# wangkenpu/rsrgan

Hardware: AMD Instinct MI355X
Metric: GAN train frames/sec (G+D step), 257-dim LPS->40-dim MFCC (higher is better)
Workload: dtype f32

## Files before the change

### rsrgan_amd/csrc/capi.cpp

```cpp
#include <cstring>
#include <exception>
#include <new>
#include <vector>

#include "model.h"
#include "segan.h"

using namespace rsr;

struct rsrgan_handle_s { Model m; };

#define CHECK_H(h)                                                    \
  if (!(h)) { set_error("null handle"); return RSRGAN_ERR_INVALID; }

#define REFUSE_INFER(h, what, rc)                                                                                   \
  if ((h)->m.infer()) { set_error("%s: the handle is inference-only (RSRGAN_FLAG_INFER)", what); return rc; }

template <class F>
static int guard(const char* what, F&& body) {
  try {
    return body();
  } catch (const std::bad_alloc&) {
    set_error("%s: out of host memory", what);
  } catch (const std::exception& e) {
// ... 372 lines not shown
  h->m.prof_on = true; h->m.prof_n = 0; h->m.prof_flops = 0.0; h->m.prof_gp_n = 0; h->m.prof_gp_flops = 0.0; h->m.prof_gb_n = 0; h->m.prof_gb_flops = 0.0; h->m.prof_fdt_n = 0;
  for (int& c : h->m.prof_cnt) c = 0;
  g_chain_launches = 0;
  return RSRGAN_OK;
}
int rsrgan_set_dropout(rsrgan_handle h, float keep_prob, uint64_t seed) {
  CHECK_H(h);
  REFUSE_INFER(h, "rsrgan_set_dropout", RSRGAN_ERR_STATE);
  if (!(keep_prob > 0.f && keep_prob <= 1.f)) { set_error("keep_prob=%g outside (0, 1]", (double)keep_prob); return RSRGAN_ERR_INVALID; }
  Model& m = h->m;
  if (keep_prob < 1.f && m.g_bnl()) { set_error("g_type bnlstm: DropoutWrapper (keep_prob < 1) is not built"); return RSRGAN_ERR_INVALID; }
  if (keep_prob < 1.f && !m.g_dnn()) {
    for (const LstmLayer& L : m.gl)
      if (!L.has_proj) { set_error("DropoutWrapper is built for generator layers with a projection (num_proj) only"); return RSRGAN_ERR_INVALID; }
  }
  if (hipDeviceSynchronize() != hipSuccess) { set_error("hipDeviceSynchronize failed"); return RSRGAN_ERR_HIP; }
  m.keep_prob = keep_prob; m.drop_seed = seed; m.drop_run = 0;
  if (m.drop_ctr && hipMemset(m.drop_ctr, 0, 16) != hipSuccess) { set_error("hipMemset failed"); return RSRGAN_ERR_HIP; }
  m.drop_graphs();
  m.g_fwd_valid = false;
  return RSRGAN_OK;
}

int rsrgan_device_status(rsrgan_handle h, int32_t* code) {
  CHECK_H(h);
  if (!code) { set_error("null output pointer"); return RSRGAN_ERR_INVALID; }
  Model& m = h->m;
  *code = 0;
  if (m.ev_last_set && hipEventSynchronize(m.ev_last) != hipSuccess) { set_error("hipEventSynchronize failed"); return RSRGAN_ERR_HIP; }
  for (hipStream_t q : {m.main_s, m.side})
    if (q && hipStreamSynchronize(q) != hipSuccess) { set_error("hipStreamSynchronize failed"); return RSRGAN_ERR_HIP; }
  if (!m.dp_ctl && !m.gp_ctl) return RSRGAN_OK;
  unsigned* blocks[3] = {m.dp_ctl, m.gp_ctl, m.dp_ctl2};
  for (int k_ = 0; k_ < 3; ++k_) {
    const int k = k_ == 2 ? 0 : k_;
    if (!blocks[k_]) continue;
    unsigned ctl[DP_CTL_WORDS];
    if (hipMemcpy(ctl, blocks[k_], sizeof(ctl), hipMemcpyDeviceToHost) != hipSuccess) { set_error("hipMemcpy failed"); return RSRGAN_ERR_HIP; }
    if (*code == 0 && ctl[DP_CTL_ERR] != 0) *code = (int32_t)(ctl[DP_CTL_ERR] + (k ? 0x10000u : 0u));
    if (ctl[DP_CTL_ERR] != 0 || ctl[DP_CTL_DONE] != 0) {
      const unsigned z[2] = {0u, 0u};
      if (hipMemcpy(blocks[k_] + DP_CTL_DONE, z, sizeof(z), hipMemcpyHostToDevice) != hipSuccess) { set_error("hipMemcpy failed"); return RSRGAN_ERR_HIP; }
      if (k == 1) m.gpersist_rearm();
      if (ctl[DP_CTL_ERR] != 0) m.persist_disable(k);
    }
  }
  return RSRGAN_OK;
}
int rsrgan_device_bytes(rsrgan_handle h, int64_t* bytes) {
  CHECK_H(h);
  if (!bytes) { set_error("null output pointer"); return RSRGAN_ERR_INVALID; }
  *bytes = (int64_t)h->m.alloc_bytes;
  return RSRGAN_OK;
}
int rsrgan_profile_launches(rsrgan_handle h, int64_t* n) {
  CHECK_H(h);
  if (!n) { set_error("null output pointer"); return RSRGAN_ERR_INVALID; }
  *n = g_chain_launches;
  return RSRGAN_OK;
}
int rsrgan_profile_read(rsrgan_handle h, int32_t* launches, double* total_us, double* alg_flops) {
  CHECK_H(h);
  Model& m = h->m;
  if (!launches || !total_us || !alg_flops) { set_error("null output pointer"); return RSRGAN_ERR_INVALID; }
  m.prof_on = false;
  double us = 0.0;
  for (int i = 0; i < m.prof_n; ++i) {
    if (hipEventSynchronize(m.prof_ev[2 * i + 1]) != hipSuccess) { set_error("hipEventSynchronize failed"); return RSRGAN_ERR_HIP; }
    float ms = 0.f;
    if (hipEventElapsedTime(&ms, m.prof_ev[2 * i], m.prof_ev[2 * i + 1]) != hipSuccess) { set_error("hipEventElapsedTime failed"); return RSRGAN_ERR_HIP; }
    us += 1e3 * ms;
  }
  *launches = m.prof_n; *total_us = us; *alg_flops = m.prof_flops;
  return RSRGAN_OK;
}
int rsrgan_profile_read_kind(rsrgan_handle h, int32_t kind, int32_t* launches, double* total_us, double* alg_flops) {
  CHECK_H(h);
  if (kind == 0) return rsrgan_profile_read(h, launches, total_us, alg_flops);
  Model& m = h->m;
  if (kind == 3 && launches && total_us && alg_flops) {
    *launches = m.prof_fdt_n; *total_us = 0.0; *alg_flops = 0.0;
    return RSRGAN_OK;
  }
  if (kind >= 4 && kind <= 8 && launches && total_us && alg_flops) {
    *launches = m.prof_cnt[kind]; *total_us = 0.0; *alg_flops = 0.0;
    return RSRGAN_OK;
  }
  if ((kind != 1 && kind != 2) || !launches || !total_us || !alg_flops) { set_error("profile_read_kind: bad argument"); return RSRGAN_ERR_INVALID; }
  std::vector<hipEvent_t>& ev = kind == 1 ? m.prof_gp_ev : m.prof_gb_ev;
  const int n = kind == 1 ? m.prof_gp_n : m.prof_gb_n;
  double us = 0.0;
  for (int i = 0; i < n; ++i) {
    if (hipEventSynchronize(ev[2 * i + 1]) != hipSuccess) { set_error("hipEventSynchronize failed"); return RSRGAN_ERR_HIP; }
    float ms = 0.f;
    if (hipEventElapsedTime(&ms, ev[2 * i], ev[2 * i + 1]) != hipSuccess) { set_error("hipEventElapsedTime failed"); return RSRGAN_ERR_HIP; }
    us += 1e3 * ms;
  }
  *launches = n; *total_us = us; *alg_flops = kind == 1 ? m.prof_gp_flops : m.prof_gb_flops;
  return RSRGAN_OK;
}

int rsrgan_op_launch_floor(int32_t n, int32_t mode, double* us_per_launch, void* stream) {
  if (n <= 0 || !us_per_launch) { set_error("op_launch_floor: bad argument"); return RSRGAN_ERR_INVALID; }
  static float* buf = nullptr;
  if (!buf && hipMalloc((void**)&buf, 2 * 65536 * 4 * sizeof(float)) != hipSuccess) { set_error("hipMalloc failed"); return RSRGAN_ERR_HIP; }
  hipStream_t s = nullptr;
  hipGraph_t g = nullptr; hipGraphExec_t ge = nullptr;
  hipEvent_t e0 = nullptr, e1 = nullptr;
  int rc = RSRGAN_ERR_HIP;
  do {
    if (hipStreamCreateWithFlags(&s, hipStreamNonBlocking) != hipSuccess) break;
    if (hipMemsetAsync(buf, 0, 2 * 65536 * 4 * sizeof(float), s) != hipSuccess) break;
    if (hipStreamBeginCapture(s, hipStreamCaptureModeThreadLocal) != hipSuccess) break;
    launch_floor_chain(buf, buf + 65536 * 4, n, mode, s);
    if (hipStreamEndCapture(s, &g) != hipSuccess) break;
    if (hipGraphInstantiate(&ge, g, nullptr, nullptr, 0) != hipSuccess) break;
    if (hipEventCreate(&e0) != hipSuccess || hipEventCreate(&e1) != hipSuccess) break;
    if (hipGraphLaunch(ge, s) != hipSuccess) break;
    if (hipEventRecord(e0, s) != hipSuccess || hipGraphLaunch(ge, s) != hipSuccess || hipEventRecord(e1, s) != hipSuccess) break;
    if (hipEventSynchronize(e1) != hipSuccess) break;
    float ms = 0.f;
    if (hipEventElapsedTime(&ms, e0, e1) != hipSuccess) break;
    *us_per_launch = 1e3 * ms / n;
    rc = RSRGAN_OK;
  } while (0);
  if (rc != RSRGAN_OK) set_error("op_launch_floor: HIP call failed");
  if (e0) (void)hipEventDestroy(e0);
  if (e1) (void)hipEventDestroy(e1);
  if (ge) (void)hipGraphExecDestroy(ge);
  if (g) (void)hipGraphDestroy(g);
  if (s) (void)hipStreamDestroy(s);
  (void)stream;
  return rc;
}

static const size_t g_op_ws_floats = (size_t)32 << 20;
static const size_t g_op_scratch_floats = (size_t)2 << 20;
static float* op_ws() {
  static float* ws = nullptr;
  if (!ws && hipMalloc((void**)&ws, g_op_ws_floats * sizeof(float)) != hipSuccess) ws = nullptr;
  return ws;
}
static float* op_scratch() {
  static float* sc = nullptr;
  if (!sc && hipMalloc((void**)&sc, g_op_scratch_floats * sizeof(float)) != hipSuccess) sc = nullptr;
  return sc;
}
#define OP_REFUSE(cond, ...) do { if (cond) { set_error(__VA_ARGS__); return RSRGAN_ERR_INVALID; } } while (0)
struct WorkersScope {
  int saved;
  explicit WorkersScope(int w) : saved(g_gemm_workers) { if (w > 0) g_gemm_workers = w; }
  ~WorkersScope() { g_gemm_workers = saved; }
};

int rsrgan_op_gemm(const float* A, int32_t lda, int32_t a_kc, const float* B, int32_t ldb, int32_t b_kc, float* C, int32_t ldc,
                   int32_t M, int32_t N, int32_t K, const float* bias, int32_t act, float alpha, int32_t accumulate, void* stream) {
  if (!A || !B || !C || (lda & 3) || (ldb & 3)) { set_error("op_gemm: null pointer or leading dimension not a multiple of 4"); return RSRGAN_ERR_INVALID; }
  float* ws = op_ws();
  launch_gemm(A, lda, a_kc != 0, B, ldb, b_kc != 0, C, ldc, M, N, K, bias, act, alpha, accumulate != 0, (hipStream_t)stream,
              ws, ws ? g_op_ws_floats : 0);
  if (hipGetLastError() != hipSuccess) { set_error("op_gemm launch failed"); return RSRGAN_ERR_HIP; }
  return RSRGAN_OK;
}

int rsrgan_op_gemm2(const float* A, int32_t lda, int32_t a_kc, const float* A2, int32_t lda2, int32_t M1, const float* B, int32_t ldb,
                    int32_t b_kc, float* C, int32_t ldc, int32_t M, int32_t N, int32_t K, const float* bias, int32_t act, float alpha,
                    int32_t accumulate, int32_t map_rows_per, int64_t map_outer, int64_t map_inner, int32_t workers, int32_t force_cfg,
// ... 900 lines not shown
```

### rsrgan_amd/csrc/dpersist.hip

```cpp
#include "kernels.h"

namespace rsr {

#include "dpersist_dev.h"

#ifdef DP_TRACE
__device__ unsigned g_dp_trace[64][128][12];
#define DPT(i) do { if (threadIdx.x == 0 && t < 128) dp_tr[t][i] = (unsigned)__builtin_amdgcn_s_memtime(); } while (0)
#define DPG(i) do { if (threadIdx.x == 256 && t < 128) dp_tr[t][8 + (i)] = (unsigned)__builtin_amdgcn_s_memtime(); } while (0)
#define DPT_DECL __shared__ unsigned dp_tr[128][12];
#define DPT_FLUSH() do { if (threadIdx.x == 0 && blockIdx.x < 64) for (int t_ = 0; t_ < 128; ++t_) for (int i_ = 0; i_ < 12; ++i_) g_dp_trace[blockIdx.x][t_][i_] = dp_tr[t_][i_]; } while (0)
#else
#define DPT(i) do { } while (0)
#define DPG(i) do { } while (0)
#define DPT_DECL
#define DPT_FLUSH() do { } while (0)
#endif

__device__ __forceinline__ void dp_fwd_body(const DPersistArgs& a, const unsigned gen) {
  __shared__ __attribute__((aligned(16))) float part_m[DP_NQ][DP_KB][64][4];
  __shared__ __attribute__((aligned(16))) float part_x[2][DP_NQ][DP_KB][64][4];
  __shared__ __attribute__((aligned(16))) float stage[6][16 * DP_HS];
  __shared__ __attribute__((aligned(16))) float kx_lds[4][4][DP_KB][64][4];
  __shared__ __attribute__((aligned(16))) float wp_lds[4][4][64][4];
  __shared__ int dead;
  DPT_DECL
  const int RTn = a.N >> 4, ncl = a.nl * RTn;
  const int cl = blockIdx.x % ncl, cq = blockIdx.x / ncl;
  const int l = cl / RTn, r = cl - l * RTn;
  const DPersistLayer L = a.L[l];
  const int tid = threadIdx.x, lane = tid & 63, lr = lane & 15, q = lane >> 4;
  const int w = __builtin_amdgcn_readfirstlane(tid >> 6);
  const int H = a.H, H4 = 4 * H, T = a.T, P = L.P, ldP = L.ldP, I = L.I;
  const int r0 = r * 16;
  const int Ns = a.Ns ? a.Ns : a.N, rb = a.row0 + r0;
  gu32* err = (gu32*)a.ctl + DP_CTL_ERR;
  if (tid == 0) dead = 0;
  const size_t slot_stride_t = (size_t)DP_NQ * DP_SLOT;
  __syncthreads();

  if (w >= 4) {
    __builtin_amdgcn_s_setprio(3);
    const int j = w - 4;
    const gu64* gm = (const gu64*)a.gran + ((size_t)(l * RTn + r) * T) * slot_stride_t + (size_t)j * DP_SLOT;
    const gu64* gx = (const gu64*)a.gran + ((size_t)(max(l - 1, 0) * RTn + r) * T) * slot_stride_t + (size_t)j * DP_SLOT;
    gu64* gout = (gu64*)a.gran + ((size_t)(l * RTn + r) * T) * slot_stride_t + (size_t)cq * DP_SLOT;
    float vm[DP_KB * 4], vx[DP_KB * 4];
    auto put = [&](float (*part)[DP_KB][64][4], const float (&v)[DP_KB * 4]) {
#pragma unroll
      for (int kb = 0; kb < DP_KB; ++kb)
        *reinterpret_cast<float4*>(&part[j][kb][lane][0]) = make_float4(v[kb * 4], v[kb * 4 + 1], v[kb * 4 + 2], v[kb * 4 + 3]);
    };
    auto fail = [&]() { if (lane == 0) { dead = 1; __hip_atomic_store(err, 1u + (unsigned)blockIdx.x, __ATOMIC_RELAXED, __HIP_MEMORY_SCOPE_AGENT); } };
    if (l > 0) {
      if (!dp_sweep2(nullptr, gen, vm, gx, gen, vx, lane, err)) fail();
      put(part_x[0], vx);
    }
    __syncthreads();
    if (dead) return;
    const int t_end = cq == 0 ? T + 1 : T;
    for (int t = 0; t < t_end; ++t) {
      const bool wm = t > 0, wx = l > 0 && t + 1 < T;
      DPG(0);
      if (wm || wx) {
        if (!dp_sweep2(wm ? gm + (size_t)(t - 1) * slot_stride_t : nullptr, gen, vm,
                       wx ? gx + (size_t)(t + 1) * slot_stride_t : nullptr, gen, vx, lane, err)) fail();
        if (wm) put(part_m, vm);
        if (wx) put(part_x[(t + 1) & 1], vx);
      }
      DPG(1);
      __syncthreads();
      if (dead) return;
      if (t < T) {
        __syncthreads();
        DPG(2);
        if (j < 3) {
          f32x4 pm = f32x4{0.f, 0.f, 0.f, 0.f};
#pragma unroll
          for (int kb = 0; kb < 4; ++kb) {
            const float4 af = *reinterpret_cast<const float4*>(&stage[5][lr * DP_HS + 16 * kb + 4 * q]);
            const float4 bf = *reinterpret_cast<const float4*>(&wp_lds[j][kb][lane][0]);
            pm = __builtin_amdgcn_mfma_f32_16x16x4f32(bf.x, af.x, pm, 0, 0, 0);
            pm = __builtin_amdgcn_mfma_f32_16x16x4f32(bf.y, af.y, pm, 0, 0, 0);
            pm = __builtin_amdgcn_mfma_f32_16x16x4f32(bf.z, af.z, pm, 0, 0, 0);
            pm = __builtin_amdgcn_mfma_f32_16x16x4f32(bf.w, af.w, pm, 0, 0, 0);
          }
          gu64* go_ = gout + (size_t)t * slot_stride_t + ((size_t)j * 64 + lane) * 4;
          dp_store2(go_, gen, pm[0], pm[1]);
          dp_store2(go_ + 2, gen, pm[2], pm[3]);
        }
        else {
          const int c4 = (lane & 15) * 4, rr = lane >> 4;
#pragma unroll
          for (int rg = 0; rg < 4; ++rg) {
            const int row = 4 * rg + rr;
            const size_t grow = (size_t)t * Ns + rb + row;
#pragma unroll
            for (int g = 0; g < 4; ++g)
              *reinterpret_cast<float4*>(L.gates + grow * H4 + g * H + cq * 64 + c4) = *reinterpret_cast<const float4*>(&stage[g][row * DP_HS + c4]);
            *reinterpret_cast<float4*>(L.c + (grow + Ns) * H + cq * 64 + c4) = *reinterpret_cast<const float4*>(&stage[4][row * DP_HS + c4]);
            *reinterpret_cast<float4*>(L.h + grow * L.ldH + cq * 64 + c4) = *reinterpret_cast<const float4*>(&stage[5][row * DP_HS + c4]);
          }
        }
        DPG(3);
      }
    }
    return;
  }

  const int cell = cq * 64 + 16 * w + lr;
  float4 kh[4][DP_KB];
#pragma unroll
  for (int g = 0; g < 4; ++g)
#pragma unroll
    for (int kb = 0; kb < DP_KB; ++kb) {
      float vh[4], vx[4];
#pragma unroll
      for (int u = 0; u < 4; ++u) {
        const int k = 16 * kb + 4 * q + u;
        vh[u] = L.K[(size_t)(I + min(k, P - 1)) * H4 + g * H + cell];
        vx[u] = L.K[(size_t)min(k, I - 1) * H4 + g * H + cell];
      }
      asm volatile("" : "+v"(vh[0]), "+v"(vh[1]), "+v"(vh[2]), "+v"(vh[3]), "+v"(vx[0]), "+v"(vx[1]), "+v"(vx[2]), "+v"(vx[3]));
#pragma unroll
      for (int u = 0; u < 4; ++u) {
        const int k = 16 * kb + 4 * q + u;
        vh[u] = k < P ? vh[u] : 0.f;
        vx[u] = k < I ? vx[u] : 0.f;
      }
      kh[g][kb] = make_float4(vh[0], vh[1], vh[2], vh[3]);
      *reinterpret_cast<float4*>(&kx_lds[w][g][kb][lane][0]) = make_float4(vx[0], vx[1], vx[2], vx[3]);
    }
  {
    const int col = 16 * w + lr;
#pragma unroll
    for (int kb = 0; kb < 4; ++kb) {
      float v[4];
#pragma unroll
      for (int u = 0; u < 4; ++u) v[u] = L.Wp[(size_t)(cq * 64 + 16 * kb + 4 * q + u) * ldP + min(col, P - 1)];
      asm volatile("" : "+v"(v[0]), "+v"(v[1]), "+v"(v[2]), "+v"(v[3]));
#pragma unroll
      for (int u = 0; u < 4; ++u) v[u] = col < P ? v[u] : 0.f;
      *reinterpret_cast<float4*>(&wp_lds[w][kb][lane][0]) = make_float4(v[0], v[1], v[2], v[3]);
    }
  }
  const int cb = cq * 64 + 16 * w + 4 * q;
  const float4 pwi = *reinterpret_cast<const float4*>(L.wi + cb), pwf = *reinterpret_cast<const float4*>(L.wf + cb);
  const float4 pwo = *reinterpret_cast<const float4*>(L.wo + cb);
  f32x4 bs[4];
#pragma unroll
  for (int g = 0; g < 4; ++g) bs[g] = *reinterpret_cast<const f32x4*>(L.bias + g * H + cb);
  const int lenF = a.len[r0 + lr];
  float cp[4] = {0.f, 0.f, 0.f, 0.f};
  float4 mf[DP_KB];
#pragma unroll
  for (int kb = 0; kb < DP_KB; ++kb) mf[kb] = make_float4(0.f, 0.f, 0.f, 0.f);
  *reinterpret_cast<float4*>(L.c + (size_t)(rb + lr) * H + cb) = make_float4(0.f, 0.f, 0.f, 0.f);
  if (cq == 0 && w == 0) {
#pragma unroll
    for (int kb = 0; kb < DP_KB; ++kb)
      if (16 * kb + 4 * q < P) *reinterpret_cast<float4*>(L.mst + (size_t)(rb + lr) * ldP + 16 * kb + 4 * q) = make_float4(0.f, 0.f, 0.f, 0.f);
  }

  f32x4 accn[4];
  float4 xn[DP_KB];
  auto load_x = [&](int t) {
    const float* xr = L.in + ((size_t)t * Ns + rb + lr) * L.ldI;
#pragma unroll
    for (int kb = 0; kb < DP_KB; ++kb) xn[kb] = *reinterpret_cast<const float4*>(xr + min(16 * kb + 4 * q, I - 4));
  };
  auto sum_parts = [&](float (*part)[DP_KB][64][4], int width, float4 (&s)[DP_KB]) {
#pragma unroll
    for (int kb = 0; kb < DP_KB; ++kb) {
      const float4 p0 = *reinterpret_cast<const float4*>(&part[0][kb][lane][0]), p1 = *reinterpret_cast<const float4*>(&part[1][kb][lane][0]);
      const float4 p2 = *reinterpret_cast<const float4*>(&part[2][kb][lane][0]), p3 = *reinterpret_cast<const float4*>(&part[3][kb][lane][0]);
      s[kb] = dp_sel(16 * kb + 4 * q < width,
                     make_float4(((p0.x + p1.x) + p2.x) + p3.x, ((p0.y + p1.y) + p2.y) + p3.y, ((p0.z + p1.z) + p2.z) + p3.z,
                                 ((p0.w + p1.w) + p2.w) + p3.w), make_float4(0.f, 0.f, 0.f, 0.f));
    }
  };
  auto mma_part = [&](f32x4 (&acc)[4], const float4 (&af)[DP_KB], const float4 (&bf)[4][DP_KB]) {
#pragma unroll
    for (int kb = 0; kb < DP_KB; ++kb) {
#pragma unroll
      for (int g = 0; g < 4; ++g) acc[g] = __builtin_amdgcn_mfma_f32_16x16x4f32(bf[g][kb].x, af[kb].x, acc[g], 0, 0, 0);
#pragma unroll
      for (int g = 0; g < 4; ++g) acc[g] = __builtin_amdgcn_mfma_f32_16x16x4f32(bf[g][kb].y, af[kb].y, acc[g], 0, 0, 0);
#pragma unroll
      for (int g = 0; g < 4; ++g) acc[g] = __builtin_amdgcn_mfma_f32_16x16x4f32(bf[g][kb].z, af[kb].z, acc[g], 0, 0, 0);
#pragma unroll
      for (int g = 0; g < 4; ++g) acc[g] = __builtin_amdgcn_mfma_f32_16x16x4f32(bf[g][kb].w, af[kb].w, acc[g], 0, 0, 0);
    }
  };
  auto next_x = [&](int t) {
#pragma unroll
    for (int g = 0; g < 4; ++g) accn[g] = bs[g];
    float4 xs[DP_KB];
    if (l > 0) {
      sum_parts(part_x[t & 1], I, xs);
      const bool live = t < lenF;
#pragma unroll
      for (int kb = 0; kb < DP_KB; ++kb) xs[kb] = dp_sel(live, xs[kb], make_float4(0.f, 0.f, 0.f, 0.f));
    } else {
#pragma unroll
      for (int kb = 0; kb < DP_KB; ++kb) xs[kb] = dp_sel(16 * kb + 4 * q < I, xn[kb], make_float4(0.f, 0.f, 0.f, 0.f));
    }
#pragma unroll
    for (int kb = 0; kb < DP_KB; ++kb) {
      float4 bf[4];
#pragma unroll
      for (int g = 0; g < 4; ++g) bf[g] = *reinterpret_cast<const float4*>(&kx_lds[w][g][kb][lane][0]);
#pragma unroll
      for (int g = 0; g < 4; ++g) accn[g] = __builtin_amdgcn_mfma_f32_16x16x4f32(bf[g].x, xs[kb].x, accn[g], 0, 0, 0);
#pragma unroll
      for (int g = 0; g < 4; ++g) accn[g] = __builtin_amdgcn_mfma_f32_16x16x4f32(bf[g].y, xs[kb].y, accn[g], 0, 0, 0);
#pragma unroll
      for (int g = 0; g < 4; ++g) accn[g] = __builtin_amdgcn_mfma_f32_16x16x4f32(bf[g].z, xs[kb].z, accn[g], 0, 0, 0);
#pragma unroll
      for (int g = 0; g < 4; ++g) accn[g] = __builtin_amdgcn_mfma_f32_16x16x4f32(bf[g].w, xs[kb].w, accn[g], 0, 0, 0);
    }
  };
  auto store_m = [&](int t, const float4 (&mnew)[DP_KB], bool live_prev) {
    if (cq != 0 || w != 0) return;
#pragma unroll
    for (int kb = 0; kb < DP_KB; ++kb)
      if (16 * kb + 4 * q < P) {
        *reinterpret_cast<float4*>(L.mst + ((size_t)t * Ns + rb + lr) * ldP + 16 * kb + 4 * q) = mf[kb];
        *reinterpret_cast<float4*>(L.out + ((size_t)(t - 1) * Ns + rb + lr) * ldP + 16 * kb + 4 * q) =
            dp_sel(live_prev, mnew[kb], make_float4(0.f, 0.f, 0.f, 0.f));
      }
  };

  if (l == 0) load_x(0);
  __syncthreads();
  if (dead) return;
  next_x(0);
  if (l == 0) load_x(min(1, T - 1));

  float hv[4] = {0.f, 0.f, 0.f, 0.f}, sg[4][4] = {};
  for (int t = 0; t < T; ++t) {
    f32x4 acc[4];
    DPT(0);
    __syncthreads();
    if (dead) return;
    DPT(1);
#pragma unroll
    for (int g = 0; g < 4; ++g) acc[g] = accn[g];
    if (t > 0) {
      float4 ms[DP_KB];
      sum_parts(part_m, P, ms);
      const bool live_prev = (t - 1) < lenF;
#pragma unroll
      for (int kb = 0; kb < DP_KB; ++kb) mf[kb] = dp_sel(live_prev, ms[kb], mf[kb]);
      store_m(t, ms, live_prev);
    }
    mma_part(acc, mf, kh);
    DPT(2);
    const bool live = t < lenF;
    const float pi_[4] = {pwi.x, pwi.y, pwi.z, pwi.w}, pf_[4] = {pwf.x, pwf.y, pwf.z, pwf.w}, po_[4] = {pwo.x, pwo.y, pwo.z, pwo.w};
#pragma unroll
    for (int i = 0; i < 4; ++i) {
      const float cpv = cp[i];
      const float gi = dp_sigmoid(acc[0][i] + pi_[i] * cpv);
      const float gf = dp_sigmoid(acc[2][i] + a.forget_bias + pf_[i] * cpv);
      const float gj = dp_tanh(acc[1][i]);
      const float cn = gf * cpv + gi * gj;
      const float go = dp_sigmoid(acc[3][i] + po_[i] * cn);
      const float hh = go * dp_tanh(cn);
      hv[i] = live ? hh : 0.f;
      sg[0][i] = live ? gi : 0.f; sg[1][i] = live ? gj : 0.f; sg[2][i] = live ? gf : 0.f; sg[3][i] = live ? go : 0.f;
      cp[i] = live ? cn : cpv;
    }
    {
      const int so = lr * DP_HS + 16 * w + 4 * q;
#pragma unroll
      for (int g = 0; g < 4; ++g) *reinterpret_cast<float4*>(&stage[g][so]) = make_float4(sg[g][0], sg[g][1], sg[g][2], sg[g][3]);
      *reinterpret_cast<float4*>(&stage[4][so]) = make_float4(cp[0], cp[1], cp[2], cp[3]);
      *reinterpret_cast<float4*>(&stage[5][so]) = make_float4(hv[0], hv[1], hv[2], hv[3]);
    }
    DPT(3);
    __syncthreads();
    DPT(4);
    DPT(7);
    __builtin_amdgcn_s_sleep(12);
    if (t + 1 < T) next_x(t + 1);
    if (l == 0) load_x(min(t + 2, T - 1));
    DPT(5);
    DPT(6);
  }
  DPT_FLUSH();
  if (cq == 0) {
    __syncthreads();
    if (dead) return;
    float4 ms[DP_KB];
    sum_parts(part_m, P, ms);
    const bool live_prev = (T - 1) < lenF;
#pragma unroll
    for (int kb = 0; kb < DP_KB; ++kb) mf[kb] = dp_sel(live_prev, ms[kb], mf[kb]);
    store_m(T, ms, live_prev);
  }
}

__global__ __launch_bounds__(512, 1) void k_dlstm_fwd(const DPersistArgs a) {
  gu32* ctl = (gu32*)a.ctl;
  const unsigned gen = __hip_atomic_load(ctl + DP_CTL_GEN, __ATOMIC_RELAXED, __HIP_MEMORY_SCOPE_AGENT);
  dp_fwd_body(a, gen);
  if (threadIdx.x == 0) persist_last_out(ctl, gen, [] { return gridDim.x; }, [&] { return a.L[a.nl - 1].out; }, 0u, [] {});
}

__device__ __forceinline__ void dp_bwd_body(const DPersistArgs& a, const unsigned gen) {
  __shared__ __attribute__((aligned(16))) float part_m[DP_NQ][DP_KB][64][4];
  __shared__ __attribute__((aligned(16))) float part_x[2][DP_NQ][DP_KB][64][4];
  __shared__ __attribute__((aligned(16))) float stage[4][16 * DP_HS];
  __shared__ __attribute__((aligned(16))) float psum[4][DP_KB][64][4];
  __shared__ __attribute__((aligned(16))) float psum_x[2][4][DP_KB][64][4];
  __shared__ __attribute__((aligned(16))) float kx_lds[4][DP_KB][4][64][4];
  __shared__ int dead;
  DPT_DECL
  const int RTn = a.N >> 4, ncl = a.nl * RTn;
  const int cl = blockIdx.x % ncl, cq = blockIdx.x / ncl;
  const int l = cl / RTn, r = cl - l * RTn;
  const DPersistLayer L = a.L[l];
  const int tid = threadIdx.x, lane = tid & 63, lr = lane & 15, q = lane >> 4;
  const int w = __builtin_amdgcn_readfirstlane(tid >> 6);
  const int H = a.H, H4 = 4 * H, T = a.T, N = a.N, P = L.P, ldP = L.ldP, I = L.I;
  const int r0 = r * 16;
  const bool top = l == a.nl - 1;
  gu32* err = (gu32*)a.ctl + DP_CTL_ERR;
  if (tid == 0) dead = 0;
  const size_t slot_stride_t = (size_t)DP_NQ * DP_SLOT;
  auto edge = [&](int layer, int e) -> gu64* {
    return (gu64*)a.gran + ((size_t)((layer * 2 + e) * RTn + r) * T) * slot_stride_t;
  };
  __syncthreads();

  if (w >= 4) {
    __builtin_amdgcn_s_setprio(3);
    const int j = w - 4;
    const gu64* gm = edge(l, 0) + (size_t)j * DP_SLOT;
    const gu64* gx = edge(min(l + 1, a.nl - 1), 1) + (size_t)j * DP_SLOT;
    gu64* gout_m = edge(l, 0) + (size_t)cq * DP_SLOT;
    gu64* gout_x = edge(l, 1) + (size_t)cq * DP_SLOT;
    gu32* dwf = a.dw_ws ? (gu32*)a.dw_flag + ((size_t)(l * RTn + r) * (T + 1)) * 4 + cq : nullptr;
    float vm[DP_KB * 4], vx[DP_KB * 4];
    auto put = [&](float (*part)[DP_KB][64][4], const float (&v)[DP_KB * 4]) {
#pragma unroll
      for (int kb = 0; kb < DP_KB; ++kb)
        *reinterpret_cast<float4*>(&part[j][kb][lane][0]) = make_float4(v[kb * 4], v[kb * 4 + 1], v[kb * 4 + 2], v[kb * 4 + 3]);
    };
    auto fail = [&]() { if (lane == 0) { dead = 1; __hip_atomic_store(err, 1u + (unsigned)blockIdx.x, __ATOMIC_RELAXED, __HIP_MEMORY_SCOPE_AGENT); } };
    auto publish = [&](float (*ps)[DP_KB][64][4], gu64* dst) {
      const float4 p0 = *reinterpret_cast<const float4*>(&ps[0][j][lane][0]), p1 = *reinterpret_cast<const float4*>(&ps[1][j][lane][0]);
      const float4 p2 = *reinterpret_cast<const float4*>(&ps[2][j][lane][0]), p3 = *reinterpret_cast<const float4*>(&ps[3][j][lane][0]);
      gu64* go_ = dst + ((size_t)j * 64 + lane) * 4;
      dp_store2(go_, gen, ((p0.x + p1.x) + p2.x) + p3.x, ((p0.y + p1.y) + p2.y) + p3.y);
      dp_store2(go_ + 2, gen, ((p0.z + p1.z) + p2.z) + p3.z, ((p0.w + p1.w) + p2.w) + p3.w);
    };
    if (!top) {
      if (!dp_sweep2(nullptr, gen, vm, gx + (size_t)(T - 1) * slot_stride_t, gen, vx, lane, err)) fail();
      put(part_x[(T - 1) & 1], vx);
    }
    __syncthreads();
    if (dead) return;
    for (int t = T - 1; t >= 0; --t) {
      const bool wm = t < T - 1, wx = !top && t > 0;
      DPG(0);
      if (wm || wx) {
        if (!dp_sweep2(wm ? gm + (size_t)(t + 1) * slot_stride_t : nullptr, gen, vm,
                       wx ? gx + (size_t)(t - 1) * slot_stride_t : nullptr, gen, vx, lane, err)) fail();
        if (wm) put(part_m, vm);
        if (wx) put(part_x[(t - 1) & 1], vx);
      }
      DPG(1);
      __syncthreads();
      if (dead) return;
      if (j < 3 && l > 0 && t < T - 1) publish(psum_x[(t + 1) & 1], gout_x + (size_t)(t + 1) * slot_stride_t);
      __syncthreads();
      DPG(2);
      if (j < 3) {
        publish(psum, gout_m + (size_t)t * slot_stride_t);
      } else {
        const int c4 = (lane & 15) * 4, rr = lane >> 4;
        if (dwf) {
          if (lane == 0) __hip_atomic_store(dwf + (size_t)t * 4, gen, __ATOMIC_RELAXED, __HIP_MEMORY_SCOPE_AGENT);
#pragma unroll
          for (int rg = 0; rg < 4; ++rg) {
            const int row = 4 * rg + rr;
            const size_t grow = (size_t)t * N + r0 + row;
#pragma unroll
            for (int g = 0; g < 4; ++g)
              dp_store4_wt(L.gates + grow * H4 + g * H + cq * 64 + c4, *reinterpret_cast<const float4*>(&stage[g][row * DP_HS + c4]));
          }
        } else {
#pragma unroll
          for (int rg = 0; rg < 4; ++rg) {
            const int row = 4 * rg + rr;
            const size_t grow = (size_t)t * N + r0 + row;
#pragma unroll
            for (int g = 0; g < 4; ++g)
              *reinterpret_cast<float4*>(L.gates + grow * H4 + g * H + cq * 64 + c4) = *reinterpret_cast<const float4*>(&stage[g][row * DP_HS + c4]);
          }
        }
      }
      DPG(3);
    }
    if (l > 0) {
      __syncthreads();
      if (j < 3) publish(psum_x[0], gout_x);
    }
    return;
  }

  const int cb = cq * 64 + 16 * w + 4 * q;
  float4 wpA[DP_KB], khA[DP_KB][4];
  {
    const float* wrow = L.Wp + (size_t)(cq * 64 + 16 * w + lr) * ldP;
#pragma unroll
    for (int kb = 0; kb < DP_KB; ++kb) {
      const int k = 16 * kb + 4 * q;
      const float4 v = *reinterpret_cast<const float4*>(wrow + min(k, P - 4));
      wpA[kb] = dp_sel(k < P, v, make_float4(0.f, 0.f, 0.f, 0.f));
    }
#pragma unroll
    for (int pt = 0; pt < DP_KB; ++pt) {
      const int p = 16 * pt + lr;
#pragma unroll
      for (int g = 0; g < 4; ++g) {
        const float4 vh = *reinterpret_cast<const float4*>(L.K + (size_t)(I + min(p, P - 1)) * H4 + g * H + cb);
        const float4 vx = *reinterpret_cast<const float4*>(L.K + (size_t)min(p, I - 1) * H4 + g * H + cb);
        khA[pt][g] = dp_sel(p < P, vh, make_float4(0.f, 0.f, 0.f, 0.f));
        *reinterpret_cast<float4*>(&kx_lds[w][pt][g][lane][0]) = dp_sel(l > 0 && p < I, vx, make_float4(0.f, 0.f, 0.f, 0.f));
      }
    }
  }
  const float4 pwi = *reinterpret_cast<const float4*>(L.wi + cb), pwf = *reinterpret_cast<const float4*>(L.wf + cb);
  const float4 pwo = *reinterpret_cast<const float4*>(L.wo + cb);
  const float pi_[4] = {pwi.x, pwi.y, pwi.z, pwi.w}, pf_[4] = {pwf.x, pwf.y, pwf.z, pwf.w}, po_[4] = {pwo.x, pwo.y, pwo.z, pwo.w};
  const int lenF = a.len[r0 + lr];

  float dc[4] = {0.f, 0.f, 0.f, 0.f};
  float4 mf[DP_KB];
#pragma unroll
  for (int kb = 0; kb < DP_KB; ++kb) mf[kb] = make_float4(0.f, 0.f, 0.f, 0.f);
  f32x4 gn[4], cpn;
  float4 don[DP_KB];
  f32x4 ccur;
  auto prefetch = [&](int t) {
    const size_t row = (size_t)t * N + r0 + lr;
#pragma unroll
    for (int g = 0; g < 4; ++g) gn[g] = *reinterpret_cast<const f32x4*>(L.gates + row * H4 + g * H + cb);
    cpn = *reinterpret_cast<const f32x4*>(L.c + row * H + cb);
    if (top) {
#pragma unroll
      for (int kb = 0; kb < DP_KB; ++kb)
        don[kb] = *reinterpret_cast<const float4*>(a.dout_top + row * a.ld_dout + min(16 * kb + 4 * q, P - 4));
    }
  };
  auto sum_parts = [&](float (*part)[DP_KB][64][4], int width, float4 (&s)[DP_KB]) {
#pragma unroll
    for (int kb = 0; kb < DP_KB; ++kb) {
      const float4 p0 = *reinterpret_cast<const float4*>(&part[0][kb][lane][0]), p1 = *reinterpret_cast<const float4*>(&part[1][kb][lane][0]);
      const float4 p2 = *reinterpret_cast<const float4*>(&part[2][kb][lane][0]), p3 = *reinterpret_cast<const float4*>(&part[3][kb][lane][0]);
      s[kb] = dp_sel(16 * kb + 4 * q < width,
                     make_float4(((p0.x + p1.x) + p2.x) + p3.x, ((p0.y + p1.y) + p2.y) + p3.y, ((p0.z + p1.z) + p2.z) + p3.z,
                                 ((p0.w + p1.w) + p2.w) + p3.w), make_float4(0.f, 0.f, 0.f, 0.f));
    }
  };
  ccur = *reinterpret_cast<const f32x4*>(L.c + ((size_t)T * N + r0 + lr) * H + cb);
  prefetch(T - 1);
  __syncthreads();
  if (dead) return;

  for (int t = T - 1; t >= 0; --t) {
    DPT(0);
    __syncthreads();
    if (dead) return;
    DPT(1);
    const bool live = t < lenF;
    f32x4 gt[4];
#pragma unroll
    for (int g = 0; g < 4; ++g) gt[g] = gn[g];
    const f32x4 cprev = cpn;
    float4 dout[DP_KB];
    if (top) {
#pragma unroll
      for (int kb = 0; kb < DP_KB; ++kb) dout[kb] = dp_sel(16 * kb + 4 * q < P, don[kb], make_float4(0.f, 0.f, 0.f, 0.f));
    } else {
      sum_parts(part_x[t & 1], P, dout);
    }
    prefetch(max(t - 1, 0));
    if (t < T - 1) {
      float4 ms[DP_KB];
      sum_parts(part_m, P, ms);
      const bool live_next = (t + 1) < lenF;
#pragma unroll
      for (int kb = 0; kb < DP_KB; ++kb) mf[kb] = dp_sel(live_next, ms[kb], mf[kb]);
    }
    float4 dm[DP_KB];
#pragma unroll
    for (int kb = 0; kb < DP_KB; ++kb)
      dm[kb] = dp_sel(live, make_float4(dout[kb].x + mf[kb].x, dout[kb].y + mf[kb].y, dout[kb].z + mf[kb].z, dout[kb].w + mf[kb].w),
                      make_float4(0.f, 0.f, 0.f, 0.f));
    if (cq == 0 && w == 0) {
      if (a.dw_ws) {
#pragma unroll
        for (int kb = 0; kb < DP_KB; ++kb)
          if (16 * kb + 4 * q < P) dp_store4_wt(L.dmt + ((size_t)t * N + r0 + lr) * ldP + 16 * kb + 4 * q, dm[kb]);
      } else {
#pragma unroll
        for (int kb = 0; kb < DP_KB; ++kb)
          if (16 * kb + 4 * q < P) *reinterpret_cast<float4*>(L.dmt + ((size_t)t * N + r0 + lr) * ldP + 16 * kb + 4 * q) = dm[kb];
      }
    }
    f32x4 dh = f32x4{0.f, 0.f, 0.f, 0.f};
#pragma unroll
    for (int kb = 0; kb < DP_KB; ++kb) {
      dh = __builtin_amdgcn_mfma_f32_16x16x4f32(wpA[kb].x, dm[kb].x, dh, 0, 0, 0);
      dh = __builtin_amdgcn_mfma_f32_16x16x4f32(wpA[kb].y, dm[kb].y, dh, 0, 0, 0);
      dh = __builtin_amdgcn_mfma_f32_16x16x4f32(wpA[kb].z, dm[kb].z, dh, 0, 0, 0);
      dh = __builtin_amdgcn_mfma_f32_16x16x4f32(wpA[kb].w, dm[kb].w, dh, 0, 0, 0);
    }
    DPT(2);
    float dz[4][4];
#pragma unroll
    for (int i = 0; i < 4; ++i) {
      const float gi = gt[0][i], gj = gt[1][i], gf = gt[2][i], go = gt[3][i];
      const float tc = dp_tanh(ccur[i]);
      const float dao = dh[i] * tc * go * (1.f - go);
      const float dcn = dc[i] + dh[i] * go * (1.f - tc * tc) + dao * po_[i];
      const float daf = dcn * cprev[i] * gf * (1.f - gf);
      const float dai = dcn * gj * gi * (1.f - gi);
      const float dj = dcn * gi * (1.f - gj * gj);
      dz[0][i] = live ? dai : 0.f; dz[1][i] = live ? dj : 0.f; dz[2][i] = live ? daf : 0.f; dz[3][i] = live ? dao : 0.f;
      dc[i] = live ? dcn * gf + dai * pi_[i] + daf * pf_[i] : dc[i];
    }
    ccur = cprev;
    {
      const int so = lr * DP_HS + 16 * w + 4 * q;
#pragma unroll
      for (int g = 0; g < 4; ++g) *reinterpret_cast<float4*>(&stage[g][so]) = make_float4(dz[g][0], dz[g][1], dz[g][2], dz[g][3]);
    }
    DPT(3);
    f32x4 pa[DP_KB];
#pragma unroll
    for (int pt = 0; pt < DP_KB; ++pt) pa[pt] = f32x4{0.f, 0.f, 0.f, 0.f};
#pragma unroll
    for (int g = 0; g < 4; ++g) {
#pragma unroll
      for (int pt = 0; pt < DP_KB; ++pt) pa[pt] = __builtin_amdgcn_mfma_f32_16x16x4f32(khA[pt][g].x, dz[g][0], pa[pt], 0, 0, 0);
#pragma unroll
      for (int pt = 0; pt < DP_KB; ++pt) pa[pt] = __builtin_amdgcn_mfma_f32_16x16x4f32(khA[pt][g].y, dz[g][1], pa[pt], 0, 0, 0);
#pragma unroll
      for (int pt = 0; pt < DP_KB; ++pt) pa[pt] = __builtin_amdgcn_mfma_f32_16x16x4f32(khA[pt][g].z, dz[g][2], pa[pt], 0, 0, 0);
#pragma unroll
      for (int pt = 0; pt < DP_KB; ++pt) pa[pt] = __builtin_amdgcn_mfma_f32_16x16x4f32(khA[pt][g].w, dz[g][3], pa[pt], 0, 0, 0);
    }
#pragma unroll
    for (int pt = 0; pt < DP_KB; ++pt) *reinterpret_cast<f32x4*>(&psum[w][pt][lane][0]) = pa[pt];
    DPT(4);
    __syncthreads();
    DPT(5);
    if (l > 0) {
      __builtin_amdgcn_s_sleep(8);
#pragma unroll
      for (int pt = 0; pt < DP_KB; ++pt) pa[pt] = f32x4{0.f, 0.f, 0.f, 0.f};
#pragma unroll
      for (int g = 0; g < 4; ++g) {
        float4 af[DP_KB];
#pragma unroll
        for (int pt = 0; pt < DP_KB; ++pt) af[pt] = *reinterpret_cast<const float4*>(&kx_lds[w][pt][g][lane][0]);
#pragma unroll
        for (int pt = 0; pt < DP_KB; ++pt) pa[pt] = __builtin_amdgcn_mfma_f32_16x16x4f32(af[pt].x, dz[g][0], pa[pt], 0, 0, 0);
#pragma unroll
        for (int pt = 0; pt < DP_KB; ++pt) pa[pt] = __builtin_amdgcn_mfma_f32_16x16x4f32(af[pt].y, dz[g][1], pa[pt], 0, 0, 0);
#pragma unroll
        for (int pt = 0; pt < DP_KB; ++pt) pa[pt] = __builtin_amdgcn_mfma_f32_16x16x4f32(af[pt].z, dz[g][2], pa[pt], 0, 0, 0);
#pragma unroll
        for (int pt = 0; pt < DP_KB; ++pt) pa[pt] = __builtin_amdgcn_mfma_f32_16x16x4f32(af[pt].w, dz[g][3], pa[pt], 0, 0, 0);
      }
#pragma unroll
      for (int pt = 0; pt < DP_KB; ++pt) *reinterpret_cast<f32x4*>(&psum_x[t & 1][w][pt][lane][0]) = pa[pt];
    }
    DPT(6);
  }
  DPT_FLUSH();
  if (l > 0) __syncthreads();
}

constexpr int DW_MT = 6;
__device__ __forceinline__ float dp_ld_sc1(const float* p) {
  return __uint_as_float(__hip_atomic_load((const unsigned*)p, __ATOMIC_RELAXED, __HIP_MEMORY_SCOPE_AGENT));
}
template <bool proj>
__device__ __forceinline__ void dp_dw_body(const DPersistArgs& a, const unsigned gen, const int bid) {
  const int RTn = a.N >> 4;
  const int g = bid & 3, cl = bid >> 2;
  const int l = cl / RTn, r = cl - l * RTn;
  const DPersistLayer L = a.L[l];
  const int lane = threadIdx.x & 63, lr = lane & 15, q = lane >> 4;
  const int w = __builtin_amdgcn_readfirstlane(threadIdx.x >> 6);
  const int H = a.H, H4 = 4 * H, T = a.T, N = a.N, I = L.I, P = L.P, ldP = L.ldP, ldI = L.ldI;
  const int r0 = r * 16;
  const int c0 = 32 * w, col0 = g * H + c0;
  gu32* err = (gu32*)a.ctl + DP_CTL_ERR;
  const gu32* flags = (const gu32*)a.dw_flag + ((size_t)(l * RTn + r) * (T + 1)) * 4;

  f32x4 acc[DW_MT][2];
#pragma unroll
  for (int mt = 0; mt < DW_MT; ++mt) { acc[mt][0] = f32x4{0.f, 0.f, 0.f, 0.f}; acc[mt][1] = f32x4{0.f, 0.f, 0.f, 0.f}; }
  f32x4 accp[2][DP_KB];
#pragma unroll
  for (int j = 0; j < 2; ++j)
#pragma unroll
    for (int nt = 0; nt < DP_KB; ++nt) accp[j][nt] = f32x4{0.f, 0.f, 0.f, 0.f};
  float pp[2] = {0.f, 0.f};
  const size_t coff = g == 3 ? (size_t)N * H : 0;

  struct Ops { float av[DW_MT][4], bv[2][4], ev[DP_KB][4], fv[2][4]; };
  bool ok = true;
  auto wait_for = [&](int t) {
    const gu32* fp = flags + (size_t)(t >= 2 ? t - 2 : T) * 4;
    const unsigned long long t0 = __builtin_amdgcn_s_memrealtime();
    for (unsigned spins = 0;; ++spins) {
      u32x4 v;
      asm volatile("global_load_dwordx4 %0, %1, off sc1\n\ts_waitcnt vmcnt(0)" : "=&v"(v) : "v"(fp) : "memory");
      if (v.x == gen && v.y == gen && v.z == gen && v.w == gen) return;
      __builtin_amdgcn_s_sleep(32);
      if ((spins & 63) == 63 && (__builtin_amdgcn_s_memrealtime() - t0 > 100000000ull ||
                                 __hip_atomic_load(err, __ATOMIC_RELAXED, __HIP_MEMORY_SCOPE_AGENT) != 0)) { ok = false; return; }
    }
  };
  unsigned off_x[3], off_m[3], off_d[DP_KB];
  float msk_x[3], msk_m[3], one_m[3];
#pragma unroll
  for (int k = 0; k < 3; ++k) {
    const int f = 16 * k + lr;
    off_x[k] = (unsigned)((r0 + q) * ldI + min(f, I - 1)); msk_x[k] = f < I ? 1.f : 0.f;
    off_m[k] = (unsigned)((r0 + q) * ldP + min(f, P - 1)); msk_m[k] = f < P ? 1.f : 0.f; one_m[k] = f == P ? 1.f : 0.f;
    off_d[k] = off_m[k];
  }
  const unsigned off_b = (unsigned)((r0 + q) * H4 + col0 + lr);
  const unsigned off_c = (unsigned)((r0 + q) * (proj ? L.ldH : H) + c0 + lr);
  auto load = [&](Ops& o, int t) {
#pragma unroll
    for (int s = 0; s < 4; ++s) {
      const size_t rw = (size_t)t * N + 4 * s;
      const float* gb = L.gates + rw * H4;
      o.bv[0][s] = dp_ld_sc1(gb + off_b);
      o.bv[1][s] = dp_ld_sc1(gb + off_b + 16);
    }
#pragma unroll
    for (int s = 0; s < 4; ++s) {
      const size_t rw = (size_t)t * N + 4 * s;
      const float* xb = L.in + rw * ldI;
      const float* mb = L.mst + rw * ldP;
#pragma unroll
      for (int k = 0; k < 3; ++k) { o.av[k][s] = xb[off_x[k]]; o.av[3 + k][s] = mb[off_m[k]]; }
    }
    if (proj) {
#pragma unroll
      for (int s = 0; s < 4; ++s) {
        const size_t rw = (size_t)t * N + 4 * s;
        const float* hb = L.h + rw * L.ldH;
        const float* db = L.dmt + rw * ldP;
        o.fv[0][s] = hb[off_c]; o.fv[1][s] = hb[off_c + 16];
#pragma unroll
        for (int nt = 0; nt < DP_KB; ++nt) o.ev[nt][s] = dp_ld_sc1(db + off_d[nt]);
      }
    } else {
#pragma unroll
      for (int s = 0; s < 4; ++s) {
        const float* cb = L.c + coff + ((size_t)t * N + 4 * s) * H;
        o.fv[0][s] = cb[off_c]; o.fv[1][s] = cb[off_c + 16];
      }
    }
    __builtin_amdgcn_sched_barrier(0);
#pragma unroll
    for (int s = 0; s < 4; ++s) {
#pragma unroll
      for (int k = 0; k < 3; ++k) { o.av[k][s] *= msk_x[k]; o.av[3 + k][s] = o.av[3 + k][s] * msk_m[k] + one_m[k]; }
      if (proj) {
#pragma unroll
        for (int nt = 0; nt < DP_KB; ++nt) o.ev[nt][s] *= msk_m[nt];
      }
    }
  };
  auto compute = [&](const Ops& o) {
#pragma unroll
    for (int s = 0; s < 4; ++s) {
#pragma unroll
      for (int mt = 0; mt < DW_MT; ++mt) {
        acc[mt][0] = __builtin_amdgcn_mfma_f32_16x16x4f32(o.av[mt][s], o.bv[0][s], acc[mt][0], 0, 0, 0);
        acc[mt][1] = __builtin_amdgcn_mfma_f32_16x16x4f32(o.av[mt][s], o.bv[1][s], acc[mt][1], 0, 0, 0);
      }
    }
    if (proj) {
#pragma unroll
      for (int s = 0; s < 4; ++s)
#pragma unroll
        for (int j = 0; j < 2; ++j)
#pragma unroll
          for (int nt = 0; nt < DP_KB; ++nt) accp[j][nt] = __builtin_amdgcn_mfma_f32_16x16x4f32(o.fv[j][s], o.ev[nt][s], accp[j][nt], 0, 0, 0);
    } else {
#pragma unroll
      for (int s = 0; s < 4; ++s) { pp[0] += o.bv[0][s] * o.fv[0][s]; pp[1] += o.bv[1][s] * o.fv[1][s]; }
    }
  };
  __shared__ int prog;
  if (threadIdx.x == 0) prog = T;
  __syncthreads();
  Ops o;
  if (w == 0) {
    wait_for(T - 1);
    if (lane == 0) __hip_atomic_store(&prog, ok ? T - 1 : -1, __ATOMIC_RELAXED, __HIP_MEMORY_SCOPE_WORKGROUP);
    for (int t = T - 1; t >= 0 && ok; --t) {
      u32x4 fl = {gen, gen, gen, gen};
      if (t >= 1) {
        const gu32* fp = flags + (size_t)(t >= 3 ? t - 3 : T) * 4;
        asm volatile("global_load_dwordx4 %0, %1, off sc1" : "=&v"(fl) : "v"(fp) : "memory");
      }
      load(o, t);
      compute(o);
      asm volatile("s_waitcnt vmcnt(0)" : "+v"(fl) : : "memory");
      if (t >= 1) {
        if (!(fl.x == gen && fl.y == gen && fl.z == gen && fl.w == gen)) { __builtin_amdgcn_s_sleep(32); wait_for(t - 1); }
        if (lane == 0) __hip_atomic_store(&prog, ok ? t - 1 : -1, __ATOMIC_RELAXED, __HIP_MEMORY_SCOPE_WORKGROUP);
      }
    }
  } else {
    for (int t = T - 1; t >= 0 && ok; --t) {
      for (;;) {
        const int p_ = __hip_atomic_load(&prog, __ATOMIC_RELAXED, __HIP_MEMORY_SCOPE_WORKGROUP);
        if (p_ < 0) { ok = false; break; }
        if (p_ <= t) break;
        __builtin_amdgcn_s_sleep(4);
      }
      if (!ok) break;
      load(o, t);
      compute(o);
    }
  }
  if (!ok) return;
  float* wsb = a.dw_ws + (size_t)(l * RTn + r) * a.dw_stride;
#pragma unroll
  for (int mt = 0; mt < DW_MT; ++mt)
#pragma unroll
    for (int nt = 0; nt < 2; ++nt)
#pragma unroll
      for (int i = 0; i < 4; ++i) {
        const int f = 16 * (mt % 3) + 4 * q + i;
        const bool on = mt < 3 ? f < I : f <= P;
        if (on) wsb[(size_t)(mt < 3 ? f : I + f) * H4 + col0 + 16 * nt + lr] = acc[mt][nt][i];
      }
  if (proj) {
    float* pw = wsb + (size_t)(I + P + 1) * H4 + 3 * H;
#pragma unroll
    for (int j = 0; j < 2; ++j)
#pragma unroll
      for (int nt = 0; nt < DP_KB; ++nt)
#pragma unroll
        for (int i = 0; i < 4; ++i)
          if (16 * nt + lr < P) pw[(size_t)(c0 + 16 * j + 4 * q + i) * ldP + 16 * nt + lr] = accp[j][nt][i];
  } else {
    float* pw = wsb + (size_t)(I + P + 1) * H4 + (g == 0 ? 0 : g == 2 ? 1 : 2) * H + c0;
#pragma unroll
    for (int nt = 0; nt < 2; ++nt) {
      float v = pp[nt];
      v += __shfl_xor(v, 16); v += __shfl_xor(v, 32);
      if (q == 0) pw[16 * nt + lr] = v;
    }
  }
}

__global__ __launch_bounds__(512, 1) void k_dlstm_bwd(const DPersistArgs a) {
  gu32* ctl = (gu32*)a.ctl;
  const unsigned gen = __hip_atomic_load(ctl + DP_CTL_GEN, __ATOMIC_RELAXED, __HIP_MEMORY_SCOPE_AGENT);
  const int nchain = a.nl * (a.N >> 4) * DP_NQ;
  if ((int)blockIdx.x >= nchain) {
    const int bid = (int)blockIdx.x - nchain;
    if ((bid & 3) == 1) dp_dw_body<true>(a, gen, bid); else dp_dw_body<false>(a, gen, bid);
  } else {
    dp_bwd_body(a, gen);
    if (a.dw_ws) {
      asm volatile("s_waitcnt vmcnt(0)" ::: "memory");
      __syncthreads();
      if (threadIdx.x == 0) {
        const int RTn = a.N >> 4, ncl = a.nl * RTn, cl = blockIdx.x % ncl, cq = blockIdx.x / ncl;
        __hip_atomic_store((gu32*)a.dw_flag + ((size_t)cl * (a.T + 1) + a.T) * 4 + cq, gen, __ATOMIC_RELAXED, __HIP_MEMORY_SCOPE_AGENT);
      }
    }
  }
  if (threadIdx.x == 0) persist_last_out(ctl, gen, [] { return gridDim.x; }, [&] { return a.L[0].gates; }, 0u, [] {});
}


size_t dpersist_granule_bytes(int nl, int N, int T) { return (size_t)2 * nl * (N / 16) * T * DP_NQ * DP_SLOT * sizeof(unsigned long long); }

int dpersist_grid(int nl, int N) { return nl * (N / 16) * DP_NQ; }
size_t dpersist_lds_bytes() {
  hipFuncAttributes f{}, b{};
  if (hipFuncGetAttributes(&f, (const void*)k_dlstm_fwd) != hipSuccess || hipFuncGetAttributes(&b, (const void*)k_dlstm_bwd) != hipSuccess) return 0;
  return f.sharedSizeBytes > b.sharedSizeBytes ? f.sharedSizeBytes : b.sharedSizeBytes;
}

bool dpersist_supported(const DPersistArgs& a) {
  if (a.nl < 1 || a.nl > DP_MAXL || a.N % 16 != 0 || a.H != 64 * DP_NQ || a.T < 1) return false;
  if (dpersist_grid(a.nl, a.N) > 128 || dpersist_grid(a.nl, a.N) > device_cu_count()) return false;
  for (int l = 0; l < a.nl; ++l) {
    const DPersistLayer& L = a.L[l];
    if (L.P > 16 * DP_KB || L.P % 4 != 0 || L.ldP % 4 != 0 || L.P < 4) return false;
    if (l > 0 && (L.I != a.L[l - 1].P)) return false;
    if (L.I > 16 * DP_KB || (l == 0 && (L.I < 4 || L.I % 4 != 0 || L.ldI % 4 != 0))) return false;
  }
  return true;
}

void launch_dlstm_bwd(const DPersistArgs& a, hipStream_t s) {
  const int blocks = dpersist_grid(a.nl, a.N) + (a.dw_ws ? dpersist_dw_grid(a.nl, a.N) : 0);
  hipLaunchKernelGGL(k_dlstm_bwd, dim3(blocks), dim3(512), 0, s, a);
  ++g_chain_launches;
}
int dpersist_dw_grid(int nl, int N) { return 4 * nl * (N / 16); }
size_t dpersist_dw_stride(const DPersistArgs& a) { return (size_t)(a.L[0].I + a.L[0].P + 1) * 4 * a.H + 3 * (size_t)a.H + (size_t)a.H * a.L[0].ldP; }
size_t dpersist_dw_flag_bytes(int nl, int N, int T) { return (size_t)nl * (N / 16) * (T + 1) * 4 * sizeof(unsigned); }
bool dpersist_dw_supported(const DPersistArgs& a) {
  for (int l = 0; l < a.nl; ++l) {
    const DPersistLayer& L = a.L[l];
    if (L.I > 48 || L.P > 47 || L.I < 1 || L.I != a.L[0].I || L.P != a.L[0].P || L.ldP != a.L[0].ldP || L.ldI < L.I) return false;
  }
  return a.H == 64 * DP_NQ;
}

__global__ __launch_bounds__(768, 3) void k_dlstm_fwd_t(const DPersistArgs a) {
  __shared__ __attribute__((aligned(16))) DpFwdTLds S;
  gu32* ctl = (gu32*)a.ctl;
  const unsigned gen = __hip_atomic_load(ctl + DP_CTL_GEN, __ATOMIC_RELAXED, __HIP_MEMORY_SCOPE_AGENT);
  if (threadIdx.x == 0) S.dead = 0;
  __syncthreads();
  dp_fwdt_body<false>(a, gen, S, (int)blockIdx.x, false);
  if (threadIdx.x == 0) persist_last_out(ctl, gen, [] { return gridDim.x; }, [&] { return a.L[a.nl - 1].out; }, 0u, [] {});
}
void launch_dlstm_fwd_t(const DPersistArgs& a, hipStream_t s) {
  hipLaunchKernelGGL(k_dlstm_fwd_t, dim3(a.nl * (a.N / 32) * DP_NQ), dim3(768), 0, s, a);
  ++g_chain_launches;
}

size_t dpersist_fwdt_lds_bytes() { return sizeof(DpFwdTLds); }
int dpersist_trail_grid(int nl, int N) { return nl * (N / 32) * DP_NQ + N / 16; }
size_t dpersist_trail_lds_bytes() { return sizeof(DpTrailLds); }
bool dpersist_trail_supported(const DPersistArgs& a) {
  if (!dpersist_supported(a) || a.N % 32 != 0 || !a.dy || !a.fc_w || !a.dtop) return false;
  if (a.ld_dy % 4 != 0 || a.ld_fcw % 4 != 0 || a.ld_dtop % 4 != 0 || a.fc_P < 1 || a.fc_P > a.ld_dtop || a.ld_dtop > 16 * 8 * DP_FCT) return false;
  return a.L[0].I % 4 == 0 && a.L[0].I >= 4 && a.L[0].I <= a.ld_dy && a.L[0].I <= a.ld_fcw;
}
void launch_dlstm_fwd(const DPersistArgs& a, hipStream_t s) {
  const int blocks = dpersist_grid(a.nl, a.N);
  hipLaunchKernelGGL(k_dlstm_fwd, dim3(blocks), dim3(512), 0, s, a);
  ++g_chain_launches;
}

}
```

### rsrgan_amd/csrc/kernels.h

```cpp
#pragma once
#include <hip/hip_runtime.h>
#include <stdint.h>

#include "switches.h"

namespace rsr {

constexpr int MAXJ = 8;

struct Place { int x0, nx, sb, se, nb, w; };
constexpr int JOBMAP_MAX = 768;
struct JobMap { int valid; unsigned char job[JOBMAP_MAX]; };
struct PlanItem { int ncol, nrow; double cost; int mult; };
int plan_places(int n, const PlanItem* items, Place* out);

enum { DYN_G_LR = 0, DYN_D_LR = 1, DYN_LAMBDA = 2, DYN_D_REAL = 3, DYN_D_FAKE = 4, DYN_L2 = 5, DYN_CLIP = 6,
       DYN_B1 = 7, DYN_B2 = 8, DYN_EPS = 9, DYN_EMA = 10, DYN_ADAM_LRT = 11, DYN_ADAM_LRT_D = 12, DYN_COUNT = 16 };

struct FwdGateJob {
  const float* x;
  const float* KxT;
  const float* m;
  const float* KhT;
  const float* Wsw;
// ... 34 lines not shown
  const float* noise;
  int ldh, ldm, ldo, P, t, N;
  int nblk_c;
  Place pl;
  DropSpec drop;
};
struct FwdProjJobs { int n; FwdProjJob j[MAXJ]; JobMap map; };

struct BwdAJob {
  const float* dout;
  const float* dmst;
  const float* Wp;
  const float* Wp_sw;
  float* dmt;
  float* gates;
  const float* c_prev;
  const float* c_cur;
  const float* wf; const float* wi; const float* wo;
  float* dc;
  const int* len;
  int ldm, P, t, N, H;
  int nblk_c;
  Place pl;
  DropSpec drop;
};
struct BwdAJobs { int n; BwdAJob j[MAXJ]; JobMap map; };

struct BwdBJob {
  const float* dz;
  const float* K;
  const float* Ksw;
  float* dx;
  float* dmst;
  const int* len;
  int I, n_begin, n_end, lddx, ldm, t, N, H4;
  int dx_accumulate;
  int nblk_c;
  Place pl;
  float* ws;
  int ldw, KG, kpg, ncg, nrg;
  Place plp, plr;
};
struct BwdBJobs { int n; BwdBJob j[MAXJ]; JobMap map, mapr; };

inline int job_blocks(int nblk_c, int N, int rows = 32) { return ((nblk_c + 7) & ~7) * ((N + rows - 1) / rows); }
int fwd_gates_rows();
void launch_fwd_gates(const FwdGateJobs& jobs, int total_blocks, int kb_max, hipStream_t s);
void launch_fwd_proj(const FwdProjJobs& jobs, int total_blocks, int kb_max, hipStream_t s);
int bwd_a_cells();
void launch_bwd_a(const BwdAJobs& jobs, int total_blocks, int kb_max, hipStream_t s);
void launch_bwd_b(const BwdBJobs& jobs, int total_blocks, int kb_max, hipStream_t s);
size_t bwd_b_plan(BwdBJobs& jobs, float* ws_base);
void launch_bwd_b_splitk(const BwdBJobs& jobs, hipStream_t s);
constexpr int DP_MAXL = 3;
constexpr int DP_CTL_GEN = 0, DP_CTL_DONE = 1, DP_CTL_ERR = 2, DP_CTL_WORDS = 4;
struct DPersistLayer {
  const float *K, *bias, *wi, *wf, *wo, *Wp;
  float *gates, *c, *h, *mst, *out;
  const float* in;
  float* dmt;
  int I, P, ldP, ldH, ldI;
};
struct DPersistArgs {
  DPersistLayer L[DP_MAXL];
  int nl, N, T, H;
  const int* len;
  unsigned long long* gran;
  unsigned* ctl;
  float forget_bias;
  const float* dout_top;
  int ld_dout;
  float* dy;
  const float* fc_w;
  float* dtop;
  int ld_dy, ld_fcw, ld_dtop, fc_P;
  const float* fc_b;
  const float* noise;
  int xd_Ns, xd_row0;
  int Ns, row0;
  int nrt;
  float* dw_ws;
  unsigned* dw_flag;
  size_t dw_stride;
};
int dpersist_dw_grid(int nl, int N);
size_t dpersist_dw_stride(const DPersistArgs& a);
size_t dpersist_dw_flag_bytes(int nl, int N, int T);
bool dpersist_dw_supported(const DPersistArgs& a);
size_t dpersist_granule_bytes(int nl, int N, int T);
int dpersist_trail_grid(int nl, int N);
size_t dpersist_trail_lds_bytes();
bool dpersist_trail_supported(const DPersistArgs& a);
bool dpersist_supported(const DPersistArgs& a);
int dpersist_grid(int nl, int N);
size_t dpersist_lds_bytes();
void launch_dlstm_fwd(const DPersistArgs& a, hipStream_t s);
void launch_dlstm_fwd_t(const DPersistArgs& a, hipStream_t s);
void launch_dlstm_bwd(const DPersistArgs& a, hipStream_t s);
constexpr int GP_MAXL = 4;
constexpr int GP_ROWS = 32;
constexpr int GP_THREADS = 768;
struct GPersistLayer {
  const float *KxT, *KhT;
  const float *bias, *wi, *wf, *wo, *Wp;
  float *gates, *c, *h, *mst, *out;
  const float* in;
  float* dmt;
  int I, P, ldI, ldP, ldH;
  float* res_out;
  const float *ca, *cb;
};
struct GPersistArgs {
  GPersistLayer L[GP_MAXL];
  int nl, N, T, H;
  int NT, NC;
  const int* len;
  unsigned long long *gran1, *gran2;
  unsigned* ctl;
  float forget_bias;
  unsigned long long* gran3;
  const float* dout_top;
  int ld_dout;
  float* din0;
  int ld_din0;
  int res;
  int tags;
  int dout_trail;
  int fwd_trail;
  int ngl, grp0;
  int nrt;
  int sched;
  int carry;
  int lean;
  int cnorm;
};
constexpr int GP_TMAX = 2046;
bool gpersist_plan(GPersistArgs& a);
void gpersist_arm_bytes(void* p, size_t bytes, hipStream_t s);
extern thread_local int g_gemm_workers;
int gpersist_grid(const GPersistArgs& a);
int gpersist_dt_grid(const GPersistArgs& a, const DPersistArgs& d);
void launch_glstm_fwd_dt(const GPersistArgs& a, const DPersistArgs& d, hipStream_t s);
size_t dpersist_fwdt_lds_bytes();
void launch_glstm_bwd_dt(const GPersistArgs& a, const DPersistArgs& d, hipStream_t s);
size_t gpersist_lds_bytes();
int device_cu_count();
bool resident_probe(int grid, int threads, size_t lds_bytes);
size_t gpersist_gran1_bytes(const GPersistArgs& a);
size_t gpersist_gran2_bytes(const GPersistArgs& a);
size_t gpersist_gran3_bytes(const GPersistArgs& a);
void gpersist_arm(const GPersistArgs& a, hipStream_t s);
void launch_glstm_fwd(const GPersistArgs& a, hipStream_t s);
bool gpersist_np_plan(GPersistArgs& a, int nt_force = 0);
size_t gpersist_np_gran2_bytes(const GPersistArgs& a);
size_t gpersist_np_lds_bytes();
void launch_glstm_np_fwd(const GPersistArgs& a, hipStream_t s);
size_t gpersist_np_gran1_bytes(const GPersistArgs& a);
size_t gpersist_np_gran3_bytes(const GPersistArgs& a);
void gpersist_np_arm(const GPersistArgs& a, hipStream_t s);
void launch_glstm_np_bwd(const GPersistArgs& a, hipStream_t s);
void launch_glstm_bwd(const GPersistArgs& a, hipStream_t s);
extern long long g_chain_launches;
void launch_floor_chain(float* a, float* b, int n, int mode, hipStream_t s);

struct GemmRowMap { int rows_per; long long outer; long long inner; };
enum { GEMM_CLS_NONE = 0, GEMM_CLS_GEMM16 = 1, GEMM_CLS_N32 = 2, GEMM_CLS_KGEMM = 3, GEMM_CLS_KGEMM_S = 4, GEMM_CLS_GEMM16_B = 5,
       GEMM_CLS_KGEMM_B = 6, GEMM_CLS_KGEMM_S_B = 7 };
struct GemmPlanRecord { int cls, bm, bn, W, n_dp, fixup, splits, Ur; };
extern thread_local GemmPlanRecord g_gemm_last_plan;
void launch_gemm_mapped(const float* A, int lda, const GemmRowMap& ma, const float* A2, int lda2, int M1, bool a_kc, const float* B, int ldb,
                        bool b_kc, float* C, int ldc, int M, int N, int K, const float* bias, int act, float alpha,
                        bool accumulate, hipStream_t s, float* ws, size_t ws_floats, int force_cfg = -1);
constexpr int GEMM16_MAXB = 4;
struct Gemm16Batch { const float* A[GEMM16_MAXB]; const float* A2[GEMM16_MAXB]; const float* B[GEMM16_MAXB]; float* C[GEMM16_MAXB]; int n; };
void launch_gemm16_batch(const Gemm16Batch& bt, int lda, int lda2, int M1, int ldb, int ldc, int M, int N, int K, bool accumulate,
                         hipStream_t s, float* ws, size_t ws_floats);
void launch_gemm2(const float* A, int lda, const float* A2, int lda2, int M1, bool a_kc, const float* B, int ldb, bool b_kc,
                  float* C, int ldc, int M, int N, int K, const float* bias, int act, float alpha, bool accumulate,
// ... 140 lines not shown
```

### rsrgan_amd/csrc/model.cpp

```cpp
#include "model.h"

#include <cmath>
#include <cstdarg>
#include <cstdio>
#include <cstdlib>
#include <cstring>

namespace rsr {

static thread_local char g_err[512] = "";
void set_error(const char* fmt, ...) {
  va_list ap;
  va_start(ap, fmt);
  vsnprintf(g_err, sizeof(g_err), fmt, ap);
  va_end(ap);
}
const char* get_error() { return g_err; }

static inline uint64_t seg_key(int seg, int T, unsigned bits) { return ((uint64_t)seg << 48) | ((uint64_t)(unsigned)T << 16) | (bits & 0xffffu); }
enum { SEG_D = 1, SEG_G_MAIN = 2, SEG_G_FCIN = 3, SEG_G_LAYER0 = 4 , SEG_G_L2 = 20, SEG_G_TAIL = 21, SEG_APPLY_D = 22, SEG_APPLY_G = 23, SEG_G_BATCH = 24, SEG_BNL = 25 };

template <class F>
void Model::run_seg(uint64_t key, hipStream_t s, F&& body) {
  if (!graphs_on() || s == nullptr) { body(); return; }
// ... 293 lines not shown
    flush_g();
    for (size_t c = 0; c < chains.size(); ++c) {
      Chain& ch = chains[c];
      const int off = offsets ? (*offsets)[c] : 0;
      for (int l = (int)ch.size() - 1; l >= 0; --l) {
        const int t = d - off - l;
        if (t < 0 || t >= T) continue;
        const LayerRun& R = ch[l];
        if (!R.L->has_proj) continue;
        if (pj.n == MAXJ) flush_p();
        FwdProjJob& p = pj.j[pj.n++]; fill_proj(p, R, t); pb += proj_blocks(R.L->P, R.N);
        pk = std::max(pk, kb16(R.L->ldH));
      }
    }
    if (fcs)
      for (auto& F : *fcs) {
        const int t = d - F.offset;
        if (t < 0 || t >= T) continue;
        if (pj.n == MAXJ) flush_p();
        FwdProjJob& p = pj.j[pj.n++]; fill_fc_fwd(p, F, t); pb += proj_blocks(F.D, F.N);
        pk = std::max(pk, kb16(F.ld_in));
      }
    flush_p();
  }
}

void Model::refresh_fold(hipStream_t s) {
  SwizzleList sl{};
  for (size_t l = 0; l < dl.size(); ++l) {
    const LstmLayer& L = dl[l]; const LstmLayer& F = dl_fold[l];
    const int H4 = 4 * L.H;
    const float* K = D.W(L.tK);
    float* Kf = dl_fold_K[l];
    if (l == 0) (void)hipMemcpyAsync(Kf, K, (size_t)L.I * H4 * sizeof(float), hipMemcpyDeviceToDevice, s);
    else gemm(D.W(dl[l - 1].tWp), dl[l - 1].ldP, true, K, H4, false, Kf, H4, dl[l - 1].H, H4, L.I, nullptr, 0, 0.f, false, s);
    gemm(D.W(L.tWp), L.ldP, true, K + (size_t)L.I * H4, H4, false, Kf + (size_t)F.I * H4, H4, L.H, H4, L.P, nullptr, 0, 0.f, false, s);
    const int ncb = (F.H + 15) / 16;
    sl.j[sl.n++] = SwizzleJob{Kf, F.Wg_full, H4, 4, F.H, 0, 0, 0, F.I, F.P, F.ldI, 4 * ncb, (F.ldI + F.ldP + 15) / 16, 0};
    sl.j[sl.n++] = SwizzleJob{Kf, F.Wg_h, H4, 4, F.H, 0, 0, 0, F.I, F.P, 0, 4 * ncb, (F.ldP + 15) / 16, 0};
  }
  launch_swizzle_many(sl, s);
}

bool Model::fold_forward(Chain& ch, int T, hipStream_t s) {
  if (dl_fold.empty() || !wavefront() || ch.size() != dl_fold.size()) return false;
  Chain fch;
  for (size_t l = 0; l < ch.size(); ++l) {
    const LayerRun& R = ch[l];
    if (R.L != &dl[l] || R.S != &d_st[l] || R.res_in || R.res_out || R.zx_batched || R.want_wgrads || R.row0 != 0 || R.Ns != R.N) return false;
    LayerRun Rf = R;
    Rf.L = &dl_fold[l]; Rf.S = &d_fold_st[l];
    if (l > 0) Rf.in = d_st[l - 1].h;
    fch.push_back(Rf);
  }
  refresh_fold(s);
  std::vector<Chain> chains{fch};
  const bool prof_was = prof_on;
  prof_on = false;
  rnn_forward(chains, T, s);
  prof_on = prof_was;
  for (size_t l = 0; l < ch.size(); ++l) {
    const LstmLayer& L = dl[l];
    gemm(d_st[l].h, L.ldH, true, D.W(L.tWp), L.ldP, false, d_st[l].out, L.ldP, T * ch[l].N, L.P, L.H, nullptr, 0, 0.f, false, s);
  }
  return true;
}

bool Model::persist_forward(Chain& ch, int T, hipStream_t s) {
  if (!dp_gran || !(dp_live & 1) || !wavefront() || ch.size() != dl.size()) return false;
  DPersistArgs a{};
  a.nl = (int)ch.size(); a.N = ch[0].N; a.T = T; a.H = dl[0].H; a.len = ch[0].len;
  a.gran = dp_gran; a.ctl = dp_ctl; a.forget_bias = cfg.forget_bias;
  for (size_t l = 0; l < ch.size(); ++l) {
    const LayerRun& R = ch[l]; const LstmLayer& L = dl[l]; const LstmStash& S = d_st[l];
    if (R.L != &L || R.S != &S || R.res_in || R.res_out || R.row0 != 0 || R.Ns != R.N || R.N != a.N || !L.has_proj || L.H != a.H) return false;
    if (l > 0 && R.in != d_st[l - 1].out) return false;
    DPersistLayer& D_ = a.L[l];
    D_.K = D.W(L.tK); D_.bias = D.W(L.tb); D_.wi = D.W(L.twi); D_.wf = D.W(L.twf); D_.wo = D.W(L.two); D_.Wp = D.W(L.tWp);
    D_.gates = S.gates; D_.c = S.c; D_.h = S.h; D_.mst = S.mst; D_.out = S.out;
    D_.I = L.I; D_.P = L.P; D_.ldP = L.ldP; D_.ldH = L.ldH; D_.ldI = L.ldI;
    D_.in = l == 0 ? R.in : nullptr;
  }
  if (!dpersist_supported(a) || dpersist_grid(a.nl, a.N) > dp_max_grid || dpersist_granule_bytes(a.nl, a.N, a.T) > dp_gran_bytes) return false;
  if (switches().dfwd_t && a.N % 32 == 0) launch_dlstm_fwd_t(a, s); else launch_dlstm_fwd(a, s);
  if (prof_on) ++prof_cnt[4];
  return true;
}

int Model::trail_nrt() const {
  const bool on = switches().dp_nrt && switches().gp_nrt;
  return on && B == 32 && Bt <= 16 && (gp_live & 3) == 3 && (dp_live & 3) == 3 ? 1 : 0;
}
bool Model::gpersist_shape(GPersistArgs& a, int T) const {
  const bool res = (cfg.g_type == RSRGAN_G_RES_LSTM_L || g_resi()) && switches().gp_res;
  if (!gp_live || gl.empty() || gl.size() > (size_t)GP_MAXL || (cfg.g_type != RSRGAN_G_LSTM && cfg.g_type != RSRGAN_G_RES_LSTM_BASE && !res && !bnl_infer())) return false;
  a = GPersistArgs{};
  a.nl = (int)gl.size(); a.N = B; a.T = T; a.H = gl[0].H; a.res = res ? (g_resi() ? 2 : 1) : 0;
  bool noproj = !gl[0].has_proj;
  a.tags = switches().gp_tags && !noproj ? 1 : 0;
  if (bnl_infer()) { if (!a.tags) return false; a.cnorm = 1; }
  for (size_t l = 0; l < gl.size(); ++l) {
    const LstmLayer& L = gl[l];
    if (L.has_proj == noproj || L.H != a.H) return false;
    GPersistLayer& G_ = a.L[l];
    G_.I = L.I; G_.P = L.P; G_.ldI = L.ldI; G_.ldP = L.ldP; G_.ldH = L.ldH;
  }
  if (noproj) return switches().gp_noproj && !res && (gp_live & 1) && gpersist_np_plan(a, gp_np_nt);
  if (!gpersist_plan(a)) return false;
  if (switches().gp_nrt && B == 32 && Bt <= 16 && (gp_live & 3) == 3) a.nrt = 1;
  const int sched_env = switches().gp_sched;
  a.sched = sched_env >= 0 ? sched_env : (B >= 64 ? 3 : 0);
  return true;
}
bool Model::gpersist_args(GPersistArgs& a, int T) const {
  if (!gpersist_shape(a, T)) return false;
  a.len = len_dev;
  a.gran1 = gp_gran1; a.gran2 = gp_gran2; a.gran3 = gp_gran3; a.ctl = gp_ctl; a.forget_bias = cfg.forget_bias;
  for (size_t l = 0; l < gl.size(); ++l) {
    const LstmLayer& L = gl[l]; const LstmStash& S = g_st[l];
    GPersistLayer& G_ = a.L[l];
    G_.KxT = L.KxT; G_.KhT = L.KhT; G_.bias = L.bias_f ? L.bias_f : G.W(L.tb); G_.ca = L.ca; G_.cb = L.cb; G_.wi = G.W(L.twi); G_.wf = G.W(L.twf); G_.wo = G.W(L.two); G_.Wp = L.has_proj ? G.W(L.tWp) : nullptr;
    G_.gates = S.gates; G_.c = S.c; G_.h = S.h; G_.mst = S.mst; G_.out = S.out; G_.dmt = S.dmt;
    G_.res_out = a.res ? g_res[l] : nullptr;
  }
  return true;
}

void Model::persist_disable(int which) {
  if (which == 1) gp_live = 0; else dp_live = 0;
  lazy_sw = false;
  trail_fits = false;
  dpipe = false;
  drop_graphs();
  refresh_swizzles(RSRGAN_NET_G, nullptr);
  refresh_swizzles(RSRGAN_NET_D, nullptr);
  (void)hipStreamSynchronize(nullptr);
}

void Model::gpersist_rearm() {
  GPersistArgs a{};
  if (!gp_gran1 || !gpersist_args(a, gp_Tcap)) return;
  if (gp_noproj) {
    if (gp_gran3) { gpersist_np_arm(a, 0); (void)hipDeviceSynchronize(); }
    return;
  }
  gpersist_arm(a, 0);
  (void)hipDeviceSynchronize();
}

static void glstm_fwd_groups(GPersistArgs a, const DPersistArgs* d, hipStream_t s) {
  const int ngr = a.N / GP_ROWS;
  if (!a.ngl) { if (d) launch_glstm_fwd_dt(a, *d, s); else launch_glstm_fwd(a, s); return; }
  for (int g = 0; g < ngr; ++g) {
    a.grp0 = g;
    if (d && g == ngr - 1) launch_glstm_fwd_dt(a, *d, s); else launch_glstm_fwd(a, s);
  }
}
static void glstm_bwd_groups(GPersistArgs a, const DPersistArgs* d, hipStream_t s) {
  const int ngr = a.N / GP_ROWS;
  if (!a.ngl) { if (d) launch_glstm_bwd_dt(a, *d, s); else launch_glstm_bwd(a, s); return; }
  for (int g = 0; g < ngr; ++g) {
    a.grp0 = g;
    if (d && g == 0) { a.dout_trail = 1; launch_glstm_bwd_dt(a, *d, s); } else { a.dout_trail = 0; launch_glstm_bwd(a, s); }
  }
}

bool Model::persist_forward_g(int T, hipStream_t s) {
  if (!gp_fwd_on() || !wavefront() || seq_drop_on()) return false;
  GPersistArgs a{};
  if (!gpersist_args(a, T) || (gp_noproj ? gpersist_np_gran2_bytes(a) : gpersist_gran2_bytes(a)) > gp_gran2_bytes) return false;
  a.L[0].in = g_ins[0];
  a.carry = g_carry ? 1 : 0;
  if (infer()) {
    a.lean = 1; a.len = len_win;
    a.L[0].in = g_ins[0] + (size_t)inf_t0 * B * gl[0].ldI;
    const size_t top = gl.size() - 1;
    for (size_t l = 0; l < gl.size(); ++l) {
      GPersistLayer& G_ = a.L[l];
      G_.gates = G_.h = G_.dmt = nullptr;
      const size_t o = (size_t)inf_t0 * B * gl[l].ldP;
      G_.out = l == top && !a.res ? g_st[l].out + o : nullptr;
      G_.res_out = l == top && a.res ? g_res[l] + o : nullptr;
    }
  }
  if (gp_noproj) {
    for (size_t l = 0; l < gl.size(); ++l) a.L[l].Wp = nullptr;
    launch_glstm_np_fwd(a, s);
    if (prof_on) ++prof_cnt[7];
    return true;
  }
  if (prof_on) {
    if ((size_t)(2 * prof_gp_n + 2) > prof_gp_ev.size()) {
      const size_t old = prof_gp_ev.size();
      prof_gp_ev.resize(old + 8, nullptr);
      for (size_t i = old; i < prof_gp_ev.size(); ++i) (void)hipEventCreate(&prof_gp_ev[i]);
    }
    for (size_t l = 0; l < gl.size(); ++l)
      prof_gp_flops += 2.0 * Bt * T * ((double)(gl[l].I + gl[l].P) * 4.0 * gl[l].H + (double)gl[l].H * gl[l].P);
    (void)hipEventRecord(prof_gp_ev[2 * prof_gp_n], s);
    glstm_fwd_groups(a, nullptr, s);
    (void)hipEventRecord(prof_gp_ev[2 * prof_gp_n + 1], s);
    ++prof_gp_n;
    return true;
  }
  glstm_fwd_groups(a, nullptr, s);
  return true;
}

// ... 63 lines not shown
      if (l > 0 && (R.din_accumulate || ch[l].din != ch[l - 1].dout)) return false;
    }
    if (ch[0].din) return false;
    a.dout_top = ch.back().dout; a.ld_dout = gl.back().ldP;
    if (!a.dout_top) return false;
    if (check_only) return true;
    launch_glstm_np_bwd(a, s);
    if (prof_on) ++prof_cnt[8];
    if (!defer_wgrads) chain_wgrads(ch, T, s, nullptr, pre, post);
    else { if (pre) pre(s); if (post) post(s); }
    return true;
  }
  const bool resi = a.res == 2;
  if (resi) { a.res = 0; if (gp_trail_next) return false; }
  for (size_t l = 0; l < ch.size(); ++l) {
    const LayerRun& R = ch[l];
    if (R.L != &gl[l] || R.S != &g_st[l] || R.row0 != 0 || R.Ns != R.N || R.N != a.N || R.len != a.len) return false;
    if (!a.res) {
      if (resi ? (R.res_in != g_ins[0] || R.res_out != g_res[l]) : (R.res_in || R.res_out)) return false;
      if (l > 0 && (R.din_accumulate || ch[l].din != ch[l - 1].dout)) return false;
    } else {
      if (R.res_in != g_ins[l] || R.res_out != g_res[l] || R.dout != ch.back().dout) return false;
      if (l > 0 ? (!R.din_accumulate || R.din != R.dout) : R.din != nullptr) return false;
    }
  }
  if (!a.res && ch[0].din && ch[0].din_accumulate) return false;
  a.dout_top = ch.back().dout; a.ld_dout = gl.back().ldP;
  if (!a.dout_top) return false;
  if (check_only) return true;
  const bool din_inside = ch[0].din && switches().gp_din0 && (gl[0].I + 15) / 16 <= (gl[0].P + 15) / 16 && gl[0].ldI % 4 == 0;
  if (din_inside) { a.din0 = ch[0].din; a.ld_din0 = gl[0].ldI; }
  a.dout_trail = gp_trail_next ? switch_now_trail_dbg() : 0;
  if (gp_phase == 2) {
  } else if (prof_on) {
    if ((size_t)(2 * prof_gb_n + 2) > prof_gb_ev.size()) {
      const size_t old = prof_gb_ev.size();
      prof_gb_ev.resize(old + 8, nullptr);
      for (size_t i = old; i < prof_gb_ev.size(); ++i) (void)hipEventCreate(&prof_gb_ev[i]);
    }
    for (size_t l = 0; l < gl.size(); ++l)
      prof_gb_flops += 2.0 * Bt * T * ((double)((l || din_inside ? gl[l].I : 0) + gl[l].P) * 4.0 * gl[l].H + (double)gl[l].H * gl[l].P);
    if (gp_trail_next) {
      for (size_t l = 0; l < dl.size(); ++l)
        prof_gb_flops += 2.0 * Bt * T * ((double)(dl[l].I + dl[l].P) * 4.0 * dl[l].H + (double)dl[l].H * dl[l].P);
      prof_gb_flops += 2.0 * Bt * T * (double)Dout * gR;
    }
    (void)hipEventRecord(prof_gb_ev[2 * prof_gb_n], s);
    glstm_bwd_groups(a, gp_trail_next ? &dt_args : nullptr, s);
    (void)hipEventRecord(prof_gb_ev[2 * prof_gb_n + 1], s);
    ++prof_gb_n;
  } else
    glstm_bwd_groups(a, gp_trail_next ? &dt_args : nullptr, s);
  if (gp_phase == 1) return true;
  auto din0 = [&](hipStream_t q) {
    if (ch[0].din && !din_inside) {
      const LayerRun& R = ch[0];
      const int H4 = 4 * R.L->H;
      gemm(R.S->gates, H4, true, R.ps->W(R.L->tK), H4, true, R.din, R.L->ldI, T * R.N, R.L->I, H4, nullptr, 0, 0.f, false, q);
    }
  };
  if (!defer_wgrads) chain_wgrads(ch, T, s, din0, pre, post);
  else { if (pre) pre(s); din0(s); if (post) post(s); }
  return true;
}

bool Model::persist_backward(Chain& ch, int T, hipStream_t s) {
  if (!dp_gran || !(dp_live & 2) || !wavefront() || ch.size() != dl.size() || ch[0].din) return false;
  DPersistArgs a{};
  a.nl = (int)ch.size(); a.N = ch[0].N; a.T = T; a.H = dl[0].H; a.len = ch[0].len;
  a.gran = dp_gran; a.ctl = dp_ctl; a.forget_bias = cfg.forget_bias;
  for (size_t l = 0; l < ch.size(); ++l) {
    const LayerRun& R = ch[l]; const LstmLayer& L = dl[l]; const LstmStash& S = d_st[l];
    if (R.L != &L || R.S != &S || R.res_in || R.res_out || R.row0 != 0 || R.Ns != R.N || R.N != a.N || !L.has_proj || L.H != a.H) return false;
    if (l > 0 && R.in != d_st[l - 1].out) return false;
    DPersistLayer& D_ = a.L[l];
    D_.K = D.W(L.tK); D_.bias = D.W(L.tb); D_.wi = D.W(L.twi); D_.wf = D.W(L.twf); D_.wo = D.W(L.two); D_.Wp = D.W(L.tWp);
    D_.gates = S.gates; D_.c = S.c; D_.h = S.h; D_.mst = S.mst; D_.out = S.out; D_.dmt = S.dmt;
    D_.I = L.I; D_.P = L.P; D_.ldP = L.ldP; D_.ldH = L.ldH; D_.ldI = L.ldI; D_.in = R.in;
  }
  a.dout_top = ch.back().dout; a.ld_dout = dl.back().ldP;
  if (!a.dout_top || !dpersist_supported(a) || dpersist_grid(a.nl, a.N) > dp_max_grid || dpersist_granule_bytes(a.nl, a.N, a.T) > dp_gran_bytes) return false;
  bool dw = dw_ws && !defer_wgrads && a.N == 2 * B && T <= Tmax;
  for (auto& R : ch) dw = dw && R.want_wgrads && R.in && R.ps == &D;
  if (dw) { a.dw_ws = dw_ws; a.dw_flag = dw_flag; a.dw_stride = dw_stride; }
  launch_dlstm_bwd(a, s);
  if (prof_on) { ++prof_cnt[5]; if (dw) ++prof_cnt[6]; }
  if (dw) {
    launch_dw_reduce(dw_ws, dw_stride, a.N / 16, dw_src, D.g, D.ct, D.partial, s);
    d_partial_fresh = true;
    return true;
  }
  if (!defer_wgrads) {
    bool dK_done = false;
    const bool rest = batch_wgrads(ch, T, s, true, &dK_done);
    for (auto& R : ch)
      if (R.want_wgrads) {
        if (!dK_done || !rest) layer_wgrads_gemms(R, 0, T, false, s, !dK_done, !rest);
        if (!rest) layer_wgrads_colsums(R, T, s, (side && s == side) ? scratch2 : scratch);
      }
  }
  return true;
}

bool Model::persist_backward_trail(Chain& ch, int T, hipStream_t s, float* dy, int ld_dy, float* dtop, int ld_dtop, bool check_only) {
  if (!trail_fits || !dp_gran || !(dp_live & 2) || !wavefront() || ch.size() != dl.size() || ch[0].din) return false;
  DPersistArgs a{};
  a.nl = (int)ch.size(); a.N = ch[0].N; a.T = T; a.H = dl[0].H; a.len = ch[0].len;
  a.gran = dp_gran; a.ctl = dp_ctl; a.forget_bias = cfg.forget_bias;
  for (size_t l = 0; l < ch.size(); ++l) {
    const LayerRun& R = ch[l]; const LstmLayer& L = dl[l]; const LstmStash& S = d_st[l];
    if (R.L != &L || R.S != &S || R.res_in || R.res_out || R.row0 != 0 || R.Ns != R.N || R.N != a.N || !L.has_proj || L.H != a.H || R.want_wgrads) return false;
    if (l > 0 && R.in != d_st[l - 1].out) return false;
    DPersistLayer& D_ = a.L[l];
    D_.K = D.W(L.tK); D_.bias = D.W(L.tb); D_.wi = D.W(L.twi); D_.wf = D.W(L.twf); D_.wo = D.W(L.two); D_.Wp = D.W(L.tWp);
    D_.gates = S.gates; D_.c = S.c; D_.h = S.h; D_.mst = S.mst; D_.out = S.out; D_.dmt = S.dmt;
    D_.I = L.I; D_.P = L.P; D_.ldP = L.ldP; D_.ldH = L.ldH; D_.ldI = L.ldI;
  }
  a.dout_top = ch.back().dout; a.ld_dout = dl.back().ldP;
  a.dy = dy; a.ld_dy = ld_dy; a.fc_w = G.W(g_fc_out_w); a.ld_fcw = ldDout; a.fc_P = gR; a.dtop = dtop; a.ld_dtop = ld_dtop;
  if (!a.dout_top || a.N != B || dl[0].I != Dout || !dpersist_trail_supported(a) || dpersist_granule_bytes(a.nl, a.N, a.T) > dp_gran_bytes) return false;
  if (check_only) return true;
  a.nrt = trail_nrt();
  dt_args = a;
  return true;
}

void Model::layer_wgrads_gemms(const LayerRun& R, int t0, int t1, bool accumulate, hipStream_t s, bool do_dK, bool do_dWp) {
  const LstmLayer& L = *R.L; const LstmStash& S = *R.S; const ParamSet& ps = *R.ps;
  const int H = L.H, H4 = 4 * H, Rws = (t1 - t0) * R.N;
  const size_t r0 = (size_t)t0 * R.N;
  float* dK = ps.Gd(L.tK);
  if (!do_dK) {
  } else if (L.I % 4 == 0) {
    launch_gemm2(R.in + r0 * L.ldI, L.ldI, S.mst + r0 * L.ldP, L.ldP, L.I, false, S.gates + r0 * H4, H4, false, dK, H4,
                 L.I + L.P, H4, Rws, nullptr, 0, 0.f, accumulate, s, (side && s == side) ? gemm_ws2 : gemm_ws, gemm_ws_floats);
  } else {
    gemm(R.in + r0 * L.ldI, L.ldI, false, S.gates + r0 * H4, H4, false, dK, H4, L.I, H4, Rws, nullptr, 0, 0.f, accumulate, s);
    gemm(S.mst + r0 * L.ldP, L.ldP, false, S.gates + r0 * H4, H4, false, dK + (size_t)L.I * H4, H4, L.P, H4, Rws, nullptr, 0, 0.f, accumulate, s);
  }
  if (L.has_proj && do_dWp)
    gemm(S.h + r0 * L.ldH, L.ldH, false, S.dmt + r0 * L.ldP, L.ldP, false, ps.Gd(L.tWp), L.ldP, H, L.P, Rws, nullptr, 0, 0.f, accumulate, s);
}

bool Model::batch_wgrads(Chain& ch, int T, hipStream_t s, bool dK_too, bool* dK_done, bool check_only) {
  *dK_done = false;
  std::vector<const LayerRun*> rs;
  for (auto& R : ch) if (R.want_wgrads) rs.push_back(&R);
  if (!switches().wgrad_batch || rs.size() < 2 || rs.size() > (size_t)GEMM16_MAXB) return false;
  const LstmLayer& L0 = *rs[0]->L;
  for (auto* R : rs) {
    const LstmLayer& L = *R->L;
    if (L.I != L0.I || L.P != L0.P || L.H != L0.H || L.ldI != L0.ldI || L.ldP != L0.ldP || L.ldH != L0.ldH || !L.has_proj ||
        R->N != rs[0]->N || R->Ns != R->N || R->row0 != 0)
      return false;
    if (L.I % 4 != 0 && (dK_too || !dk_tmp || R->ps != &G)) return false;
  }
  const int H = L0.H, H4 = 4 * H, Rws = T * rs[0]->N;
  if ((size_t)rs.size() * 64 * 7 * H > scratch_floats) return false;
  float* ws = (side && s == side) ? gemm_ws2 : gemm_ws;
  float* scr = (side && s == side) ? scratch2 : scratch;
  auto small = [&](int M, int N, int K) { const double outs = (double)M * N; return !(K >= 256 && outs >= 4.0e6) && !(K >= 2048 && outs >= 1.5e6); };
  if (check_only) { *dK_done = dK_too && small(L0.I + L0.P, H4, Rws); return small(H, L0.P, Rws); }
  if (dK_too && small(L0.I + L0.P, H4, Rws)) {
    Gemm16Batch bt{}; bt.n = (int)rs.size();
    for (int p = 0; p < bt.n; ++p) { bt.A[p] = rs[p]->in; bt.A2[p] = rs[p]->S->mst; bt.B[p] = rs[p]->S->gates; bt.C[p] = rs[p]->ps->Gd(rs[p]->L->tK); }
    launch_gemm16_batch(bt, L0.ldI, L0.ldP, L0.I, H4, H4, L0.I + L0.P, H4, Rws, false, s, ws, gemm_ws_floats);
    *dK_done = true;
  }
  if (!small(H, L0.P, Rws)) return false;
// ... 945 lines not shown
```

### rsrgan_amd/csrc/model.h

```cpp
#pragma once
#include <hip/hip_runtime.h>
#include <stdint.h>
#include <string>
#include <unordered_map>
#include <functional>
#include <vector>

#include "../../include/rsrgan.h"
#include "kernels.h"

namespace rsr {

inline int pad4(int x) { return (x + 3) & ~3; }

struct TensorDesc {
  std::string name;
  int rows, cols, ld;
  int64_t off;
  int64_t dense_off;
  bool l2;
  bool trainable = true;
  bool is_vector;
  int xavier_fan_out = 0;
  float bias_init = 0.f;
// ... 70 lines not shown
  DropSpec drop{};
};
typedef std::vector<LayerRun> Chain;

struct FcStage {
  int offset = 0;
  int N = 0, K = 0, D = 0;
  const float* in = nullptr; int ld_in = 0;
  const float* WT = nullptr;
  const float* bias = nullptr;
  const float* noise = nullptr;
  float* y = nullptr; int ldy = 0;
  float* out2 = nullptr; int ld2 = 0, Ns2 = 0, row02 = 0;
  bool accumulate = false;
};

struct BnlLayer {
  int B, H, P, ldP, ldH, nst;
  int train;
  float eps, fb;
  const int* len;
  const float *Whh, *Wp, *bias, *wf, *wi, *wo;
  const float *sc_in, *of_in, *sc_s, *of_s, *sc_c, *of_c;
  float *mm_in, *mv_in, *mm_s, *mv_s, *mm_c, *mv_c;
  float *xh_in, *yin, *xh_s, *act, *cnew, *chat, *ccar, *h, *mst, *out;
  float *mu, *var;
  const float* dout;
  float *dz, *dhh, *dyc, *dmn, *dcc, *dmc;
};
struct BnlCell {
  int tWx, tWh, tin[4], tst[4], tb, twf, twi, two, tce[4], tWp;
  float *zx = nullptr, *xh_in = nullptr, *yin = nullptr, *xh_s = nullptr, *act = nullptr, *cnew = nullptr, *chat = nullptr;
  float *ccar = nullptr, *h = nullptr, *mst = nullptr, *out = nullptr, *mu = nullptr, *var = nullptr;
  float *dz = nullptr, *dyc = nullptr, *dmn = nullptr, *dcc = nullptr, *dmc = nullptr;
};
bool bnl_supported(int B);
void launch_bnl_bn_in(const BnlLayer& a, const float* zx, int T, hipStream_t s);
void launch_bnl_cell_fwd(const BnlLayer& a, int t, hipStream_t s);
void launch_bnl_proj(const BnlLayer& a, int t, hipStream_t s);
void launch_bnl_ema(const BnlLayer& a, int T, float decay, hipStream_t s);
void launch_bnl_cell_bwd(const BnlLayer& a, int t, hipStream_t s);
void launch_bnl_dm(const BnlLayer& a, int t, hipStream_t s);
void launch_bnl_bn_in_bwd(const BnlLayer& a, float* dzx, int T, hipStream_t s);
struct BnlFold {
  const float *Wx, *Wh;
  const float* bn[12];
  const float* bias;
  int P, H, ldI, ldP;
  float eps;
  float *KxT, *KhT, *bias_f, *ca, *cb;
};
void launch_bnl_fold(const BnlFold& a, hipStream_t s);

struct Model {
  rsrgan_cfg cfg{};
  const HandleSwitches sw;
  int B = 0, Tmax = 0, Din = 0, Dout = 0, ldDin = 0, ldDout = 0;
  int Bt = 0;
  int pad_Bp() const { return Bt != B ? B : 0; }
  int gR = 0, dR = 0;
  ParamSet G, D;
  std::vector<LstmLayer> gl, dl;
  int g_fc_in_w = -1, g_fc_in_b = -1, g_fc_out_w = -1, g_fc_out_b = -1, d_fc_w = -1, d_fc_b = -1;

  float *x_tm = nullptr, *lab_tm = nullptr, *g_h0 = nullptr, *y_tm = nullptr;
  std::vector<float*> g_ins;
  std::vector<float*> g_res;
  std::vector<LstmStash> g_st;
  float *g_dA = nullptr, *g_dB = nullptr, *g_dC = nullptr;
  float *xd = nullptr, *logits = nullptr, *dlogits = nullptr;
  std::vector<LstmStash> d_st;
  float *d_dA = nullptr, *d_dB = nullptr, *last_dx0 = nullptr;
  int *len_dev = nullptr;
  float *zeros = nullptr;
  std::vector<LstmLayer> dl_fold;
  std::vector<float*> dl_fold_K;
  std::vector<LstmStash> d_fold_st;
  bool fold_forward(Chain& ch, int T, hipStream_t s);
  void refresh_fold(hipStream_t s);
  unsigned long long* dp_gran = nullptr;
  unsigned* dp_ctl = nullptr;
  size_t dp_gran_bytes = 0;
  int dp_live = sw.dpersist;
  bool persist_forward(Chain& ch, int T, hipStream_t s);
  bool persist_backward(Chain& ch, int T, hipStream_t s);
  bool persist_backward_trail(Chain& ch, int T, hipStream_t s, float* dy, int ld_dy, float* dtop, int ld_dtop, bool check_only = false);
  bool persist_forward_g_trail(Chain& ch, int T, hipStream_t s, const float* nf, bool check_only = false);
  bool dpipe = false;
  bool dfree_inside = false;
  bool dfree_current = false;
  int gp_phase = 0;
  hipEvent_t ev_dfree = nullptr, ev_real = nullptr;
  unsigned long long* dp_gran2 = nullptr;
  unsigned* dp_ctl2 = nullptr;
  bool persist_forward_real(int T, hipStream_t q, bool check_only = false);
  bool trail_fits = false;
  bool gp_trail_next = false;
  DPersistArgs dt_args{};
  unsigned long long *gp_gran1 = nullptr, *gp_gran2 = nullptr, *gp_gran3 = nullptr;
  unsigned* gp_ctl = nullptr;
  size_t gp_gran2_bytes = 0;
  int gp_live = sw.gpersist;
  int gp_Tcap = 0;
  float* dw_ws = nullptr; unsigned* dw_flag = nullptr; long long* dw_src = nullptr; size_t dw_stride = 0;
  bool d_partial_fresh = false;
  int dp_max_grid = 0;
  void persist_disable(int which);
  bool gp_fwd_on() const { return gp_gran1 && (gp_live & 1); }
  bool gpersist_shape(GPersistArgs& a, int T) const;
  int gp_np_nt = 0;
  bool gp_noproj = false;
  bool gpersist_args(GPersistArgs& a, int T) const;
  void gpersist_rearm();
  bool persist_forward_g(int T, hipStream_t s);
  float* g_state = nullptr;
  int g_state_sf = 0;
  bool g_carry = false;
  void gstate_xfer(int dir, int T, int rows, const int* mask, hipStream_t s);
  typedef std::function<void(hipStream_t)> StreamFn;
  bool persist_backward_g(Chain& ch, int T, hipStream_t s, bool check_only = false, const StreamFn& pre = nullptr, const StreamFn& post = nullptr);
  std::vector<FcLayer> gfc, dfc;
  std::vector<float*> g_act, d_act;
  float *fc_dA = nullptr, *fc_dB = nullptr, *joint = nullptr, *dy_buf = nullptr;
  int ldJ = 0;
  int *adam_t_dev_d = nullptr;
  bool g_dnn() const { return cfg.g_type == RSRGAN_G_DNN || cfg.g_type == RSRGAN_G_RCED; }
  bool g_rced() const { return cfg.g_type == RSRGAN_G_RCED; }
  bool g_resi() const { return cfg.g_type == RSRGAN_G_RES_LSTM_I; }
  std::vector<BnlCell> bnl;
  bool g_bnl() const { return cfg.g_type == RSRGAN_G_BNLSTM; }
  int bnl_check(const rsrgan_cfg& c) const;
  void bnl_params();
  void bnl_alloc();
  void bnl_init(std::vector<float>& host, uint64_t seed) const;
  BnlLayer bnl_args(int l, bool train) const;
  void bnl_forward(int T, bool train, hipStream_t s);
  void bnl_backward(int T, float* dy, hipStream_t s);
  int bnl_step(const float* x, const float* labels, const int32_t* lengths, int T, float* out_losses, bool want_grads, hipStream_t s);
  bool bnl_infer() const { return g_bnl() && infer(); }
  void bnl_infer_layers();
  void bnl_refresh_fold(hipStream_t s);
  std::vector<ConvLayer> gconv;
  FcLayer rc_fc{};
  std::vector<float*> rc_act;
  float *rc_col = nullptr, *rc_dcol = nullptr, *rc_dA = nullptr, *rc_dB = nullptr;
  std::vector<float*> rc_cols;
  std::vector<float*> rc_ft_fwd, rc_ft_bwd;
  std::vector<char> rc_wgrad_implicit;
  float* rc_wg_ws = nullptr;
  float* rc_x4 = nullptr;
  bool rc_keep_cols = false;
  size_t scratch_floats = 0;
  int rcS = 0, rcW = 0;
  void g_frame_forward(int rows, hipStream_t s);
  void g_frame_backward(int rows, float* dy, hipStream_t s);
  void rced_forward(int rows, hipStream_t s);
  void rced_backward(int rows, float* dy, hipStream_t s);
  bool d_dnn() const { return cfg.d_type == RSRGAN_D_DNN && !(cfg.flags & RSRGAN_FLAG_INFER); }
  bool d_adam() const { return g_dnn(); }
  void fc_forward(const ParamSet& ps, const std::vector<FcLayer>& L, const std::vector<float*>& act, int rows, hipStream_t s, int calls = 1,
                  int call0 = 0);
  float keep_prob = 1.f;
  uint64_t drop_seed = 0, drop_run = 0;
  bool drop_training() const {
    return g_dnn() && keep_prob < 1.f && !cfg.cross_validation && !bn_eval_call && scal[RSRGAN_L2_SCALE] > 0.0;
  }
// ... 35 lines not shown
  float *tmp3 = nullptr;
  float *scratch = nullptr;
  double scal[RSRGAN_SCALAR_COUNT_] = {0};
  bool g_fwd_valid = false;
  int cur_T = 0;
  bool d_grads_ready = false, g_grads_ready = false;
  std::vector<void*> allocs;
  size_t alloc_bytes = 0;

  int init(const rsrgan_cfg& c, uint64_t seed);
  int check_cfg() const;
  void build_tables();
  void plan_rows();
  int alloc_params();
  int alloc_generator();
  void alloc_rced();
  int alloc_discriminator();
  int alloc_shared();
  int plan_persistent();
  int plan_dpersist();
  int plan_gpersist();
  int init_values(uint64_t seed);
  size_t frame_rows() const { return (size_t)Tmax * B; }
  int g_ldP() const { return g_dnn() ? 4 : pad4(gR); }
  int d_ldP() const { return d_dnn() ? 4 : pad4(dR); }
  bool res_sums() const { return cfg.g_type == RSRGAN_G_RES_LSTM_L || cfg.g_type == RSRGAN_G_RES_LSTM_I; }
  bool ema_on() const { return cfg.ema_decay > 0.f && !infer(); }
  template <typename T> T* alloc(size_t n);
  template <typename T> T* alloc_opt(size_t n);
  void* alloc_raw(size_t bytes, bool required);
  int alloc_status(const char* stage) const;
  bool alloc_fail = false;
  size_t alloc_fail_bytes = 0;
  void destroy();

  int prepare_batch(const float* x, const float* labels, const int32_t* lengths, int T, hipStream_t s, const float** nr = nullptr,
                    const float** nf = nullptr, hipStream_t early = nullptr);
  void g_forward(int T, hipStream_t s, Chain* extra = nullptr);
  void g_forward_head(int T, hipStream_t s);
  void g_forward_tail(int T, hipStream_t s);
  void d_logits(int N, int T, hipStream_t s);
  void d_backward_pass(int N, int T, bool want_wgrads, bool need_dx0, const float* dlog, hipStream_t s, bool head_done = false);
  bool d_head(int N, int T, int n_real, const float* t_real, const float* t_fake, float* loss3, bool want_grads, bool want_wgrads, hipStream_t s);
  void g_backward_pass(int T, float* dy, hipStream_t s);
  int d_backward(const float* x, const float* labels, const int32_t* lengths, int T, const float* nr, const float* nf,
                 float* out_losses, bool want_grads, hipStream_t s);
  int g_backward(const float* x, const float* labels, const int32_t* lengths, int T, const float* nf,
                 float* out_losses, bool want_grads, bool reuse, hipStream_t s);
  int apply(int net, hipStream_t s);
  void apply_body(int net, hipStream_t s);
  int apply_inlined = 0;
  void refresh_transposes(int net, hipStream_t s);
  void refresh_swizzles(int net, hipStream_t s);
  bool lazy_sw = false;

  void rnn_forward(std::vector<Chain>& chains, int T, hipStream_t s, const std::vector<int>* offsets = nullptr,
                   const std::vector<FcStage>* fcs = nullptr);
  void rnn_backward(std::vector<Chain>& chains, int T, hipStream_t s, const std::vector<int>* offsets = nullptr,
                    const std::vector<FcStage>* fcs = nullptr);
  void layer_wgrads(const LayerRun& R, int T, hipStream_t s);
  void chain_wgrads(Chain& ch, int T, hipStream_t s, const StreamFn& between, const StreamFn& pre = nullptr, const StreamFn& post = nullptr);
  void layer_wgrads_gemms(const LayerRun& R, int t0, int t1, bool accumulate, hipStream_t s, bool do_dK = true, bool do_dWp = true);
  int trail_nrt() const;
  bool batch_wgrads(Chain& ch, int T, hipStream_t s, bool dK_too, bool* dK_done, bool check_only = false);
  void layer_wgrads_colsums(const LayerRun& R, int T, hipStream_t s, float* scr);
  hipStream_t side = nullptr;
  struct GradBucket { int64_t off = 0, count = 0; hipEvent_t ev = nullptr; bool marked = false; };
  std::vector<GradBucket> gbk[2];
  bool fused_apply = false;
  bool defer_wgrads = false;
  int build_buckets();
  void mark_bucket(int net, int i, hipStream_t s);
  void finish_buckets(int net, hipStream_t s);
  bool prof_on = false;
  std::vector<hipEvent_t> prof_ev;
  int prof_n = 0;
  double prof_flops = 0.0;
  std::vector<hipEvent_t> prof_gp_ev;
  int prof_gp_n = 0;
  double prof_gp_flops = 0.0;
  std::vector<hipEvent_t> prof_gb_ev;
  int prof_gb_n = 0;
  int prof_fdt_n = 0;
  int prof_cnt[9] = {};
  double prof_gb_flops = 0.0;
  void gates_launch(const FwdGateJobs& gj, int blocks, int kb, hipStream_t s);
  int gates_blocks(int H, int N) const;
  int proj_blocks(int P, int N) const;
  int bwd_a_blocks(int H, int N) const;
  void run_bwd_b_splitk(BwdBJobs& bj, hipStream_t s);
  hipEvent_t ev_pool[16] = {};
  int ev_next = 0;
  float* gemm_ws2 = nullptr;
  float* dk_tmp = nullptr;
  size_t dk_tmp_per = 0;
  float* scratch2 = nullptr;
  bool overlap() const { return side != nullptr && (cfg.flags & RSRGAN_FLAG_OVERLAP) != 0; }
  Chain g_chain(int T);
  Chain d_chain(int N, int Ns, int row0);
  void gemm(const float* A, int lda, bool a_kc, const float* B, int ldb, bool b_kc, float* C, int ldc, int M, int N,
            int K, const float* bias, int act, float alpha, bool accumulate, hipStream_t s);
  bool supervised() const { return (cfg.flags & RSRGAN_FLAG_SUPERVISED) != 0; }
  bool infer() const { return (cfg.flags & RSRGAN_FLAG_INFER) != 0; }
  static constexpr int INFER_WINDOW = 64;
  int inf_W = 0;
  int* len_win = nullptr;
  int inf_t0 = 0, inf_slot = 0;
  bool inf_failed = false;
  bool infer_fallback_stash();
  void infer_forward(int T, hipStream_t s);
  void infer_window_launches(int t0, int Tw, hipStream_t s);
  void infer_state_to_slot0(hipStream_t s);
  bool wavefront() const { return (cfg.flags & RSRGAN_FLAG_WAVEFRONT) != 0; }
  float* g_fc_out_wT = nullptr;
  float* bwdb_ws = nullptr;
  size_t bwdb_ws_floats = 0;
  bool bwd_b_splitk_ok(const BwdBJobs& jobs) const;
  float* gemm_ws = nullptr;
  size_t gemm_ws_floats = 0;

  struct GraphSlot { int uses = 0; hipGraphExec_t exec = nullptr; };
  std::unordered_map<uint64_t, GraphSlot> graphs;
  hipStream_t main_s = nullptr;
  hipEvent_t ev_in = nullptr, ev_out = nullptr;
  hipEvent_t ev_last = nullptr; bool ev_last_set = false;
  float *noise_r_buf = nullptr, *noise_f_buf = nullptr;
  bool graphs_on() const { return (cfg.flags & RSRGAN_FLAG_GRAPH) != 0 && wavefront() && !overlap() && !prof_on && !g_dnn() && sw.graphs; }
  template <class F> void run_seg(uint64_t key, hipStream_t s, F&& body);
  void drop_graphs();
  hipStream_t enter(hipStream_t caller);
  void leave(hipStream_t caller, hipStream_t work);
  const float* stage_noise(const float* src, float* buf, hipStream_t s);
};

void set_error(const char* fmt, ...);
const char* get_error();

#define HIPC(expr)                                                                   \
  do {                                                                               \
    hipError_t e_ = (expr);                                                          \
    if (e_ != hipSuccess) {                                                          \
      rsr::set_error("%s failed: %s (%s:%d)", #expr, hipGetErrorString(e_), __FILE__, __LINE__); \
      return RSRGAN_ERR_HIP;                                                         \
    }                                                                                \
  } while (0)

}
```

### rsrgan_amd/csrc/model_init.cpp

```cpp
#include "model.h"

#include <algorithm>
#include <cmath>
#include <random>

namespace rsr {

int ParamSet::add(const std::string& name, int rows, int cols, bool is_vector) {
  TensorDesc d;
  d.name = name;
  d.rows = rows; d.cols = cols; d.ld = pad4(cols);
  d.off = padded; d.dense_off = dense;
  d.l2 = name.find("bias") == std::string::npos;
  d.is_vector = is_vector;
  padded += ((int64_t)rows * d.ld + 63) / 64 * 64;
  dense += (int64_t)rows * cols;
  t.push_back(d);
  return (int)t.size() - 1;
}

void* Model::alloc_raw(size_t bytes, bool required) {
  void* p = nullptr;
  if (hipMalloc(&p, bytes) != hipSuccess) {
    if (required && !alloc_fail) { alloc_fail = true; alloc_fail_bytes = bytes; }
// ... 459 lines not shown
int Model::alloc_shared() {
  const rsrgan_cfg& c = cfg;
  const bool inf = infer();
  drop_ctr = (unsigned long long*)alloc<float>(4);
  len_dev = alloc<int>(2 * B);
  if (inf) len_win = alloc<int>(B);
  zeros = alloc<float>(64);
  if (!inf) { noise_r_buf = alloc<float>((size_t)B * Dout); noise_f_buf = alloc<float>((size_t)B * Dout); }
  if (hipStreamCreateWithFlags(&main_s, hipStreamNonBlocking) != hipSuccess) main_s = nullptr;
  if (main_s && (hipEventCreateWithFlags(&ev_in, hipEventDisableTiming) != hipSuccess ||
                 hipEventCreateWithFlags(&ev_out, hipEventDisableTiming) != hipSuccess)) { (void)hipStreamDestroy(main_s); main_s = nullptr; }
  dyn = alloc<float>(DYN_COUNT); adam_t_dev = alloc<int>(1);
  losses = alloc<float>(8); tmp3 = alloc<float>(4);
  size_t maxcols = 7 * (size_t)std::max(c.g_cells, c.d_cells);
  maxcols = std::max(maxcols, (size_t)Din + 4);
  maxcols = std::max(maxcols, (size_t)std::max(g_ldP(), ldDin));
  scratch_floats = std::max<size_t>(4 * 64 * maxcols, 16384);
  if (!inf) {
    scratch = alloc<float>(scratch_floats);
    scratch2 = alloc<float>(std::max<size_t>(4 * 64 * maxcols, 1024));
    g_fc_out_wT = g_dnn() ? nullptr : alloc<float>((size_t)Dout * g_ldP());
  }
  if (inf || hipStreamCreateWithFlags(&side, hipStreamNonBlocking) != hipSuccess) side = nullptr;
  if (hipEventCreateWithFlags(&ev_last, hipEventDisableTiming) != hipSuccess) ev_last = nullptr;
  if (side) {
    for (auto& e : ev_pool)
      if (hipEventCreateWithFlags(&e, hipEventDisableTiming) != hipSuccess) { side = nullptr; break; }
  }
  gemm_ws_floats = (size_t)32 << 20;
  gemm_ws = alloc_opt<float>(gemm_ws_floats);
  if (!gemm_ws) gemm_ws_floats = 0;
  bwdb_ws_floats = inf ? 0 : (size_t)8 << 20;
  if (!inf) {
    bwdb_ws = alloc_opt<float>(bwdb_ws_floats);
    gemm_ws2 = alloc_opt<float>(gemm_ws_floats ? gemm_ws_floats : 1);
  }
  if (!inf && switches().dk_pad && !gl.empty() && gl[0].has_proj && gl[0].I % 4 != 0 && gl[0].ldI % 4 == 0 && gl.size() <= (size_t)GEMM_MAXB) {
    dk_tmp_per = (size_t)(gl[0].ldI + gl[0].P) * 4 * gl[0].H;
    dk_tmp = alloc_opt<float>(dk_tmp_per * gl.size());
    if (!dk_tmp) dk_tmp_per = 0;
  }
  if (!gemm_ws2) side = nullptr;
  if (int rc = alloc_status("shared work space")) return rc;
  HIPC(hipMemset(drop_ctr, 0, 16));
  return RSRGAN_OK;
}

int Model::plan_persistent() {
  if (int rc = plan_dpersist()) return rc;
  if (int rc = plan_gpersist()) return rc;
  if (bnl_infer() && !gp_fwd_on()) {
    set_error("g_type bnlstm with RSRGAN_FLAG_INFER: no persistent forward plan for this configuration (batch_size=%d padded to %d rows, %d x %d / p%d; "
              "gpersist_plan's shapes, every workgroup of a row group resident at once, RSRGAN_GPERSIST / RSRGAN_PAD_ROWS not switched off), "
              "and a launch-per-phase forward of the folded cell is not built", Bt, B, cfg.g_layers, cfg.g_cells, cfg.g_proj);
    return RSRGAN_ERR_INVALID;
  }
  GPersistArgs ga{};
  if (sw.trail && dp_gran && (dp_live & 2) && gp_gran1 && gp_gran3 && !gp_noproj && (gp_live & 2) && B % 32 == 0 && gpersist_args(ga, gp_Tcap))
    trail_fits = resident_probe(gpersist_grid(ga) + ((dpersist_trail_grid((int)dl.size(), B) + 7) & ~7), GP_THREADS,
                                std::max(gpersist_lds_bytes(), dpersist_trail_lds_bytes()));
  lazy_sw = switches().lazy_swizzle && wavefront() && gp_gran1 && gp_gran3 && (gp_live & 3) == 3 && dp_gran && (dp_live & 3) == 3;
  if (sw.dpipe > 0 && trail_fits && side && !d_dnn() && dp_max_grid >= dpersist_grid((int)dl.size(), B)) {
    const size_t gb = dpersist_granule_bytes((int)dl.size(), B, Tmax) / 2;
    dp_gran2 = (unsigned long long*)alloc_opt<float>(gb / sizeof(float));
    dp_ctl2 = (unsigned*)alloc_opt<float>(16);
    if (dp_gran2 && dp_ctl2 && hipEventCreateWithFlags(&ev_dfree, hipEventDisableTiming) == hipSuccess &&
        hipEventCreateWithFlags(&ev_real, hipEventDisableTiming) == hipSuccess) {
      HIPC(ctl_reset(dp_ctl2));
      dpipe = true;
    }
  }
  return RSRGAN_OK;
}

int Model::plan_dpersist() {
  if (dp_live && !dl.empty() && dl.size() <= (size_t)DP_MAXL && B % 16 == 0) {
    const int nl_ = (int)dl.size();
    for (int rows : {2 * B, B}) {
      const int g_ = dpersist_grid(nl_, rows);
      if (g_ <= 128 && resident_probe(g_, 512, dpersist_lds_bytes())) { dp_max_grid = g_; break; }
    }
  }
  if (dp_max_grid <= 0) return RSRGAN_OK;
  dp_gran_bytes = dpersist_granule_bytes((int)dl.size(), 2 * B, Tmax);
  dp_gran = (unsigned long long*)alloc<float>(dp_gran_bytes / sizeof(float));
  dp_ctl = (unsigned*)alloc<float>(16);
  if (int rc = alloc_status("persistent discriminator rings")) return rc;
  HIPC(ctl_reset(dp_ctl));
  DPersistArgs pa{};
  pa.nl = (int)dl.size(); pa.N = 2 * B; pa.H = dl[0].H;
  for (size_t l = 0; l < dl.size(); ++l) { pa.L[l].I = dl[l].I; pa.L[l].P = dl[l].P; pa.L[l].ldP = dl[l].ldP; pa.L[l].ldI = dl[l].ldI; }
  bool shapes = switches().dw_inkernel && (dp_live & 2) && dpersist_dw_supported(pa) && !d_adam();
  for (auto& L : dl) shapes = shapes && L.has_proj && L.H == dl[0].H && L.ldH == dl[0].ldH;
  if (shapes && dpersist_grid(pa.nl, pa.N) == dp_max_grid) {
    const int nt = pa.N / 16;
    dw_stride = dpersist_dw_stride(pa);
    dw_ws = alloc_opt<float>((size_t)pa.nl * nt * dw_stride);
    dw_flag = (unsigned*)alloc_opt<float>(dpersist_dw_flag_bytes(pa.nl, pa.N, Tmax) / sizeof(float));
    std::vector<long long> src(D.t.size(), -1);
    const int IP = dl[0].I + dl[0].P, H4 = 4 * dl[0].H, H_ = dl[0].H;
    for (size_t l = 0; l < dl.size(); ++l) {
      const long long base = (long long)l * nt * (long long)dw_stride;
      src[dl[l].tK] = base; src[dl[l].tb] = base + (long long)IP * H4;
      const long long pp = base + (long long)(IP + 1) * H4;
      src[dl[l].twi] = pp; src[dl[l].twf] = pp + H_; src[dl[l].two] = pp + 2 * H_; src[dl[l].tWp] = pp + 3 * H_;
    }
    dw_src = (long long*)alloc_opt<float>(src.size() * 2);
    if (dw_ws && dw_flag && dw_src) HIPC(hipMemcpy(dw_src, src.data(), src.size() * sizeof(long long), hipMemcpyHostToDevice));
    else dw_ws = nullptr;
  }
  return RSRGAN_OK;
}

int Model::plan_gpersist() {
  const bool inf = infer();
  if (!gp_live || g_dnn() || (g_bnl() && !inf)) return RSRGAN_OK;
  auto ring = [&](size_t bytes) { return (unsigned long long*)alloc_opt<float>(bytes / sizeof(float)); };
  GPersistArgs ga{};
  gp_Tcap = std::min(Tmax, (int)GP_TMAX);
  gp_noproj = !gl.empty() && !gl[0].has_proj;
  if (gp_noproj) {
    bool fits = false;
    for (int nt : {2, 4}) {
      gp_np_nt = nt;
      if (gpersist_shape(ga, gp_Tcap) && resident_probe(gpersist_grid(ga), GP_THREADS, gpersist_np_lds_bytes())) { fits = true; break; }
    }
    if (!fits) { gp_np_nt = 0; return RSRGAN_OK; }
    gp_gran2_bytes = gpersist_np_gran2_bytes(ga);
    gp_gran2 = ring(gp_gran2_bytes);
    gp_ctl = (unsigned*)alloc_opt<float>(16);
    if (gp_np_nt == 2 && (gp_live & 2) && switches().gp_np_bwd && !inf) {
      gp_gran1 = ring(gpersist_np_gran1_bytes(ga));
      gp_gran3 = ring(gpersist_np_gran3_bytes(ga));
      if (!gp_gran1 || !gp_gran3) { gp_gran1 = gp_gran3 = nullptr; }
    }
    if (!gp_gran1) gp_gran1 = gp_gran2;
    if (gp_gran2 && gp_ctl) {
      HIPC(ctl_reset(gp_ctl));
      gpersist_rearm();
    } else { gp_gran1 = gp_gran2 = gp_gran3 = nullptr; gp_ctl = nullptr; }
  } else if (gpersist_args(ga, gp_Tcap) && resident_probe(gpersist_grid(ga), GP_THREADS, gpersist_lds_bytes())) {
    gp_gran1 = ring(gpersist_gran1_bytes(ga));
    gp_gran2_bytes = gpersist_gran2_bytes(ga);
    gp_gran2 = ring(gp_gran2_bytes);
    gp_ctl = (unsigned*)alloc_opt<float>(16);
    bool bwd_ok = (gp_live & 2) != 0 && !inf;
    for (auto& L : gl) bwd_ok = bwd_ok && L.P > 16;
    if (bwd_ok) gp_gran3 = ring(gpersist_gran3_bytes(ga));
    if (gp_gran1 && gp_gran2 && gp_ctl) {
      HIPC(ctl_reset(gp_ctl));
      gpersist_rearm();
    } else { gp_gran1 = gp_gran2 = nullptr; gp_ctl = nullptr; }
  }
  return RSRGAN_OK;
}

int Model::init_values(uint64_t seed) {
  const rsrgan_cfg& c = cfg;
  const bool inf = infer();
  std::mt19937_64 rng(seed);
  for (ParamSet* ps : {&G, &D}) {
    if (ps == &D && inf) continue;
    std::vector<float> host((size_t)ps->padded, 0.f);
    if (ps == &G && g_bnl()) bnl_init(host, seed);
    else for (auto& t : ps->t) {
      if (!t.l2 || t.const_init) {
        if (t.bias_init != 0.f)
          for (int cc = 0; cc < t.cols; ++cc) host[(size_t)t.off + cc] = t.bias_init;
        continue;
      }
      const double fan_in = t.is_vector ? t.cols : t.rows, fan_out = t.xavier_fan_out > 0 ? t.xavier_fan_out : t.cols;
      const double lim = std::sqrt(6.0 / (fan_in + fan_out));
      std::uniform_real_distribution<double> u(-lim, lim);
      for (int r = 0; r < t.rows; ++r)
        for (int cc = 0; cc < t.cols; ++cc) host[(size_t)t.off + (size_t)r * t.ld + cc] = (float)u(rng);
    }
    HIPC(hipMemcpy(ps->w, host.data(), host.size() * sizeof(float), hipMemcpyHostToDevice));
    if (ps->ema) HIPC(hipMemcpy(ps->ema, host.data(), host.size() * sizeof(float), hipMemcpyHostToDevice));
  }
  scal[RSRGAN_G_LEARNING_RATE] = 8e-5; scal[RSRGAN_D_LEARNING_RATE] = 1e-3; scal[RSRGAN_MSE_LAMBDA] = 10.0;
  scal[RSRGAN_D_REAL] = 1.0; scal[RSRGAN_D_FAKE] = 0.0; scal[RSRGAN_L2_SCALE] = c.l2_scale;
// ... 81 lines not shown
```

### rsrgan_amd/csrc/switches.h

```cpp
#pragma once
#include <cstdlib>

namespace rsr {

#define RSRGAN_SWITCHES(X) \
  X(GPERSIST,       gpersist,       INT,  3,    ANY,  handle,  "persistent generator recurrences (gpersist.hip): bit 0 the forward launch, bit 1 the BPTT; 0 = the launch-per-phase wavefront") \
  X(DPERSIST,       dpersist,       INT,  3,    ANY,  handle,  "persistent discriminator recurrences (dpersist.hip): bit 0 the forward launch, bit 1 the backward launch") \
  X(DFOLD,          dfold,          BOOL, 1,    ANY,  handle,  "folded small-cell recurrence of the discriminator (one launch per step); 0 = gates + projection") \
  X(TRAIL,          trail,          INT,  1,    ANY,  handle,  "the discriminator's BPTT trailing the generator's inside one launch (k_glstm_bwd_dt); 0 = two launches") \
  X(GRAPHS,         graphs,         BOOL, 1,    ANY,  handle,  "0 = RSRGAN_FLAG_GRAPH is ignored: every segment runs eagerly") \
  X(RCED_IMPLICIT,  rced_implicit,  BOOL, 1,    ANY,  handle,  "implicit-GEMM convolution for every R-CED layer it covers; 0 = patch-matrix GEMMs everywhere") \
  X(DPIPE,          dpipe,          INT,  0,    ANY,  handle,  "D(real) of the D-run ahead on the side stream: > 0 covers labels and lengths, >= 2 a noise_real tensor too (include/rsrgan.h)") \
  X(PAD_ROWS,       pad_rows,       BOOL, 1,    ANY,  process, "pad the batch to a multiple of 32 rows so that the persistent generator recurrences apply; 0 = the caller's row count") \
  X(DW_INKERNEL,    dw_inkernel,    BOOL, 1,    ANY,  process, "the discriminator's weight gradients inside its stand-alone BPTT launch; 0 = GEMM / column-sum launches behind it") \
  X(GP_NP_BWD,      gp_np_bwd,      BOOL, 1,    ANY,  process, "persistent BPTT of an unprojected generator (8 cells per workgroup); 0 = its BPTT takes the launch path") \
  X(GP_NP_NT,       gp_np_nt,       INT,  0,    ANY,  process, "gate tiles per workgroup of the unprojected generator's launches: 2 or 4; 0 = what the resident probe admits") \
  X(GP_NOPROJ,      gp_noproj,      BOOL, 1,    ANY,  process, "persistent forward recurrence for num_proj=None generators (the single-hop form); 0 = launch path") \
  X(GP_RES,         gp_res,         BOOL, 1,    ANY,  process, "res_lstm_l and res_lstm_i inside the persistent launches (the residual sums ride the hand-offs); 0 = launch path") \
  X(GP_TAGS,        gp_tags,        BOOL, 1,    ANY,  process, "ring slots tagged with the parity of the ring pass; 0 = slots re-armed with sentinels") \
  X(GP_NRT,         gp_nrt,         BOOL, 1,    ANY,  process, "a padded generator whose real rows fit one 16-row tile skips the padding tile; 0 = both tiles run") \
  X(DP_NRT,         dp_nrt,         BOOL, 1,    ANY,  process, "the same for the discriminator's halves of the fused launches (only together with GP_NRT); 0 = the padding tile runs") \
  X(GP_SCHED,       gp_sched,       INT,  -1,   ANY,  process, "GPersistArgs::sched 0..3: off-chain work of the forward launch behind the lane's publication; -1 = 3 from 64 rows on, else 0") \
  X(GP_DIN0,        gp_din0,        BOOL, 0,    ANY,  process, "layer 0's input gradient inside k_glstm_bwd (built, bit-stable, measured slower)") \
  X(TRAIL_FWD,      trail_fwd,      BOOL, 1,    ANY,  process, "D(G(x)) trailing the generator's forward recurrence in one launch (k_glstm_fwd_dt); 0 = separate launches") \
  X(DFWD_T,         dfwd_t,         BOOL, 0,    ANY,  process, "the discriminator's forward launch in its two-tile form (launch_dlstm_fwd_t) where rows % 32 == 0") \
  X(DHEAD,          dhead,          BOOL, 1,    ANY,  process, "fused discriminator head (logits, LSGAN loss and their gradients in k_dhead); 0 = d_logits + launch_lsgan + GEMMs") \
  X(WGRAD_BATCH,    wgrad_batch,    BOOL, 1,    ANY,  process, "the layers' weight-gradient products as batched launches; 0 = per layer") \
  X(WGRAD_STREAMS,  wgrad_streams,  INT,  2,    ANY,  process, "streams the weight gradients run on: >= 2 puts dWp and the column sums on the side stream (and allows FC_SIDE)") \
  X(FC_SIDE,        fc_side,        BOOL, 1,    ANY,  process, "the FCs' parameter gradients of the G-run on the side stream beside the dK GEMMs (needs WGRAD_STREAMS >= 2)") \
  X(DIN0_SIDE,      din0_side,      BOOL, 0,    ANY,  process, "layer 0's input gradient and what hangs on it on the side stream as well") \
  X(LAZY_SWIZZLE,   lazy_swizzle,   BOOL, 1,    ANY,  process, "fragment-tiled weight copies rebuilt where they are read, not after every update (when every recurrence runs persistent); 0 = after every update") \
  X(FUSED_SEG,      fused_seg,      BOOL, 1,    ANY,  process, "rsrgan_d_step / rsrgan_g_step: the update closes the backward pass's graph segment; 0 = a segment of its own") \
  X(DK_PAD,         dk_pad,         BOOL, 1,    ANY,  process, "kernel gradients of layers whose input width is no multiple of 4 as one stacked product into a padded temporary; 0 = separate products") \
  X(DPIPE_W,        dpipe_w,        INT,  224,  W8,   process, "GEMM workers of the G-run's weight-gradient launches under DPIPE (the rest of the CUs are left to D(real))") \
  X(XCD_GROUPS,     xcd_groups,     BOOL, 1,    ANY,  process, "heavy jobs of a step launch own a group of XCD slots; 0 = every job spans all 8 (the contiguous layout)") \
  X(BP_GROUPS,      bp_groups,      BOOL, 1,    ANY,  process, "the same for the backward step launches' K slices; 0 = no groups") \
  X(GEMM_SELF,      gemm_self,      BOOL, 1,    ANY,  process, "the 256 x 256 / 128 x 256 / 256 x 128 tiles of k_gemm_s among the plans; 0 = leaves them out") \
  X(GEMM_BATCH,     gemm_batch,     INT,  1,    ANY,  process, "batched GEMM launches: 0 = off (one by one), 1 = 192 x 256 tiles of k_gemm_s, 2 = the 128 x 128 form") \
  X(GEMM_BATCH_W,   gemm_batch_w,   INT,  0,    W8,   process, "workers of the 192 x 256 batched launch, leaving the other CUs to the side stream; 0 = all") \
  X(CONV4,          conv4,          INT,  1,    ANY,  process, "4x4x1-MFMA convolution kernels: 0 = never (both directions), 1 = widths that waste 16-wide columns, 2 = every multiple of 4") \
  X(CONV4_KS,       conv4_ks,       INT,  2,    ANY,  process, "their k' split for 512-position workgroups: 4 = two group sets x k' quarters (measured slower), else four x halves") \
  X(WGRAD4,         wgrad4,         INT,  -1,   ANY,  process, "4x4x1-MFMA weight gradient: 0 = never, 1 = widths that are no multiple of 16, 2 = all; -1 = from CONV4 (0 -> 0, else 2)") \
  X(CONV_ROWS,      conv_rows,      BOOL, 1,    ANY,  process, "row-aligned 64-column strips for wide frames, the remaining columns in a second launch; 0 = equal strips") \
  X(WGRAD_DH,       wgrad_dh,       INT,  6,    ANY,  process, "most filter rows per workgroup of k_conv_wgrad for multi-strip frames (3 = the earlier form)") \
  X(BN_NARROW,      bn_narrow,      INT,  4096, MIN0, process, "least row count that takes the narrow batch-norm form (0 = never)") \
  X(BN_SMALL_ROWS,  bn_small_rows,  INT,  384,  ANY,  process, "most rows that take the single-workgroup-per-column-block batch-norm path") \
  X(COLRED_VEC,     colred_vec,     INT,  11,   ANY,  process, "bit m: column-reduction mode m of segan.hip loads 16 bytes per lane (mode 2 stays scalar for parity)") \
  X(RESIDENT_PROBE, resident_probe, BOOL, 1,    ANY,  process, "ask the device whether a persistent launch is resident at once; 0 = trust the CU count") \
  X(RESIDENT_CAP,   resident_cap,   INT,  0,    ANY,  process, "n > 0: the probe's verdict of a device that can hold n workgroups (what a CU mask would make it find)") \
  X(GRAPH_DEBUG,    graph_debug,    BOOL, 0,    ANY,  call,    "report on stderr when the capture of a graph segment fails") \
  X(TRAIL_DBG,      trail_dbg,      INT,  1,    ANY,  call,    "GPersistArgs::dout_trail of a trailing BPTT launch (debugging the hand-off)")

enum SwKind { SW_BOOL, SW_INT };
enum SwClamp { SW_ANY, SW_MIN0, SW_W8 };

inline int switch_read(const char* name, SwKind kind, int def, SwClamp clamp) {
  const char* e = getenv(name);
  if (!e) return def;
  const int v = atoi(e);
  if (kind == SW_BOOL) return v != 0;
  if (clamp == SW_MIN0) return v > 0 ? v : 0;
  if (clamp == SW_W8) return v >= 64 && v <= 256 ? (v & ~7) : def;
  return v;
}

#define SW_READ(NAME, kind, def, clamp) switch_read("RSRGAN_" #NAME, SW_##kind, def, SW_##clamp)
#define SW_IN_handle_handle(x) x
#define SW_IN_handle_process(x)
#define SW_IN_handle_call(x)
#define SW_IN_process_handle(x)
#define SW_IN_process_process(x) x
#define SW_IN_process_call(x)
#define SW_IN_call_handle(x)
#define SW_IN_call_process(x)
#define SW_IN_call_call(x) x

#define X(NAME, field, kind, def, clamp, scope, doc) SW_IN_handle_##scope(const int field = SW_READ(NAME, kind, def, clamp);)
struct HandleSwitches { RSRGAN_SWITCHES(X) };
#undef X
#define X(NAME, field, kind, def, clamp, scope, doc) SW_IN_process_##scope(const int field = SW_READ(NAME, kind, def, clamp);)
struct ProcessSwitches { RSRGAN_SWITCHES(X) };
#undef X
inline const ProcessSwitches& switches() { static const ProcessSwitches s; return s; }
#define X(NAME, field, kind, def, clamp, scope, doc) SW_IN_call_##scope(inline int switch_now_##field() { return SW_READ(NAME, kind, def, clamp); })
RSRGAN_SWITCHES(X)
#undef X

}
```

Measured before the change: 1.330 million.

## Split discriminator persistent recurrence across eight workgroups per row tile

Templates the persistent discriminator forward and backward kernels on the number of workgroups per row tile (4 or 8). In the eighth form each workgroup owns fewer cells and gate tiles, so the per-step recurrence work spreads over more CUs. The default DPERSIST value is raised to 7, which turns the eight-way forward on, and a residency probe at init decides whether the larger grid fits. The cost is more cross-workgroup ring traffic and partial-sum reduction per step, plus an added s_sleep before the ring sweeps.

```diff
diff --git a/rsrgan_amd/csrc/capi.cpp b/rsrgan_amd/csrc/capi.cpp
--- a/rsrgan_amd/csrc/capi.cpp
+++ b/rsrgan_amd/csrc/capi.cpp
@@ -478,7 +478,7 @@
     *launches = m.prof_fdt_n; *total_us = 0.0; *alg_flops = 0.0;
     return RSRGAN_OK;
   }
-  if (kind >= 4 && kind <= 8 && launches && total_us && alg_flops) {
+  if (kind >= 4 && kind <= 10 && launches && total_us && alg_flops) {
     *launches = m.prof_cnt[kind]; *total_us = 0.0; *alg_flops = 0.0;
     return RSRGAN_OK;
   }
diff --git a/rsrgan_amd/csrc/dpersist.hip b/rsrgan_amd/csrc/dpersist.hip
--- a/rsrgan_amd/csrc/dpersist.hip
+++ b/rsrgan_amd/csrc/dpersist.hip
@@ -17,12 +17,54 @@
 #define DPT_FLUSH() do { } while (0)
 #endif
 
+template <int NQ>
+struct DpForm {
+  static_assert(NQ == 4 || NQ == 8, "cell quarters or eighths");
+  static constexpr int CW = 256 / NQ;
+  static constexpr int CPW = CW / 4;
+  static constexpr int CPL = CPW / 4;
+  static constexpr int NT = CPW / 4;
+  static constexpr int KBP = CW / 16;
+  static constexpr int THREADS = 64 * (4 + NQ);
+  __device__ static __forceinline__ int col(int tl, int m, int c0, int H) {
+    if constexpr (NQ == 4) return tl * H + c0 + m; else return (m & 3) * H + c0 + 2 * (m >> 2) + tl;
+  }
+};
+#ifndef DP_NQ8_WAIT
+#define DP_NQ8_WAIT 16
+#endif
+template <int N> struct DpVec;
+template <> struct DpVec<4> { typedef float4 type; };
+template <> struct DpVec<2> { typedef float2 type; };
+template <int N> __device__ __forceinline__ void dp_ldn(const float* p, float (&v)[N]) {
+  const typename DpVec<N>::type x = *reinterpret_cast<const typename DpVec<N>::type*>(p);
+  v[0] = x.x; v[1] = x.y;
+  if constexpr (N == 4) { v[2] = x.z; v[3] = x.w; }
+}
+template <int N> __device__ __forceinline__ void dp_stn(float* p, const float (&v)[N]) {
+  if constexpr (N == 4) *reinterpret_cast<float4*>(p) = make_float4(v[0], v[1], v[2], v[3]);
+  else *reinterpret_cast<float2*>(p) = make_float2(v[0], v[1]);
+}
+template <int NQ>
+__device__ __forceinline__ float4 dp_sum_nq(const float (*part)[DP_KB][64][4], int kb, int lane) {
+  float4 s = *reinterpret_cast<const float4*>(&part[0][kb][lane][0]);
+#pragma unroll
+  for (int e = 1; e < NQ; ++e) {
+    const float4 p = *reinterpret_cast<const float4*>(&part[e][kb][lane][0]);
+    s = make_float4(s.x + p.x, s.y + p.y, s.z + p.z, s.w + p.w);
+  }
+  return s;
+}
+
+template <int NQ>
 __device__ __forceinline__ void dp_fwd_body(const DPersistArgs& a, const unsigned gen) {
-  __shared__ __attribute__((aligned(16))) float part_m[DP_NQ][DP_KB][64][4];
-  __shared__ __attribute__((aligned(16))) float part_x[2][DP_NQ][DP_KB][64][4];
+  typedef DpForm<NQ> F;
+  constexpr int CW = F::CW, CPW = F::CPW, CPL = F::CPL, NT = F::NT, KBP = F::KBP;
+  __shared__ __attribute__((aligned(16))) float part_m[NQ][DP_KB][64][4];
+  __shared__ __attribute__((aligned(16))) float part_x[2][NQ][DP_KB][64][4];
   __shared__ __attribute__((aligned(16))) float stage[6][16 * DP_HS];
-  __shared__ __attribute__((aligned(16))) float kx_lds[4][4][DP_KB][64][4];
-  __shared__ __attribute__((aligned(16))) float wp_lds[4][4][64][4];
+  __shared__ __attribute__((aligned(16))) float kx_lds[4][NT][DP_KB][64][4];
+  __shared__ __attribute__((aligned(16))) float wp_lds[4][KBP][64][4];
   __shared__ int dead;
   DPT_DECL
   const int RTn = a.N >> 4, ncl = a.nl * RTn;
@@ -36,7 +78,7 @@
   const int Ns = a.Ns ? a.Ns : a.N, rb = a.row0 + r0;
   gu32* err = (gu32*)a.ctl + DP_CTL_ERR;
   if (tid == 0) dead = 0;
-  const size_t slot_stride_t = (size_t)DP_NQ * DP_SLOT;
+  const size_t slot_stride_t = (size_t)NQ * DP_SLOT;
   __syncthreads();
 
   if (w >= 4) {
@@ -63,6 +105,7 @@
       const bool wm = t > 0, wx = l > 0 && t + 1 < T;
       DPG(0);
       if (wm || wx) {
+        if constexpr (NQ == 8 && DP_NQ8_WAIT > 0) __builtin_amdgcn_s_sleep(DP_NQ8_WAIT);
         if (!dp_sweep2(wm ? gm + (size_t)(t - 1) * slot_stride_t : nullptr, gen, vm,
                        wx ? gx + (size_t)(t + 1) * slot_stride_t : nullptr, gen, vx, lane, err)) fail();
         if (wm) put(part_m, vm);
@@ -77,7 +120,7 @@
         if (j < 3) {
           f32x4 pm = f32x4{0.f, 0.f, 0.f, 0.f};
 #pragma unroll
-          for (int kb = 0; kb < 4; ++kb) {
+          for (int kb = 0; kb < KBP; ++kb) {
             const float4 af = *reinterpret_cast<const float4*>(&stage[5][lr * DP_HS + 16 * kb + 4 * q]);
             const float4 bf = *reinterpret_cast<const float4*>(&wp_lds[j][kb][lane][0]);
             pm = __builtin_amdgcn_mfma_f32_16x16x4f32(bf.x, af.x, pm, 0, 0, 0);
@@ -89,17 +132,18 @@
           dp_store2(go_, gen, pm[0], pm[1]);
           dp_store2(go_ + 2, gen, pm[2], pm[3]);
         }
-        else {
-          const int c4 = (lane & 15) * 4, rr = lane >> 4;
-#pragma unroll
-          for (int rg = 0; rg < 4; ++rg) {
-            const int row = 4 * rg + rr;
+        else if (NQ == 4 || j == 3) {
+          constexpr int LPR = CW / 4, RPP = 64 / LPR;
+          const int c4 = (lane % LPR) * 4, rr = lane / LPR;
+#pragma unroll
+          for (int rg = 0; rg < 16 / RPP; ++rg) {
+            const int row = RPP * rg + rr;
             const size_t grow = (size_t)t * Ns + rb + row;
 #pragma unroll
             for (int g = 0; g < 4; ++g)
-              *reinterpret_cast<float4*>(L.gates + grow * H4 + g * H + cq * 64 + c4) = *reinterpret_cast<const float4*>(&stage[g][row * DP_HS + c4]);
-            *reinterpret_cast<float4*>(L.c + (grow + Ns) * H + cq * 64 + c4) = *reinterpret_cast<const float4*>(&stage[4][row * DP_HS + c4]);
-            *reinterpret_cast<float4*>(L.h + grow * L.ldH + cq * 64 + c4) = *reinterpret_cast<const float4*>(&stage[5][row * DP_HS + c4]);
+              *reinterpret_cast<float4*>(L.gates + grow * H4 + g * H + cq * CW + c4) = *reinterpret_cast<const float4*>(&stage[g][row * DP_HS + c4]);
+            *reinterpret_cast<float4*>(L.c + (grow + Ns) * H + cq * CW + c4) = *reinterpret_cast<const float4*>(&stage[4][row * DP_HS + c4]);
+            *reinterpret_cast<float4*>(L.h + grow * L.ldH + cq * CW + c4) = *reinterpret_cast<const float4*>(&stage[5][row * DP_HS + c4]);
           }
         }
         DPG(3);
@@ -108,18 +152,18 @@
     return;
   }
 
-  const int cell = cq * 64 + 16 * w + lr;
-  float4 kh[4][DP_KB];
-#pragma unroll
-  for (int g = 0; g < 4; ++g)
+  float4 kh[NT][DP_KB];
+#pragma unroll
+  for (int g = 0; g < NT; ++g)
 #pragma unroll
     for (int kb = 0; kb < DP_KB; ++kb) {
+      const int gcol = F::col(g, lr, cq * CW + CPW * w, H);
       float vh[4], vx[4];
 #pragma unroll
       for (int u = 0; u < 4; ++u) {
         const int k = 16 * kb + 4 * q + u;
-        vh[u] = L.K[(size_t)(I + min(k, P - 1)) * H4 + g * H + cell];
-        vx[u] = L.K[(size_t)min(k, I - 1) * H4 + g * H + cell];
+        vh[u] = L.K[(size_t)(I + min(k, P - 1)) * H4 + gcol];
+        vx[u] = L.K[(size_t)min(k, I - 1) * H4 + gcol];
       }
       asm volatile("" : "+v"(vh[0]), "+v"(vh[1]), "+v"(vh[2]), "+v"(vh[3]), "+v"(vx[0]), "+v"(vx[1]), "+v"(vx[2]), "+v"(vx[3]));
 #pragma unroll
@@ -134,35 +178,43 @@
   {
     const int col = 16 * w + lr;
 #pragma unroll
-    for (int kb = 0; kb < 4; ++kb) {
+    for (int kb = 0; kb < KBP; ++kb) {
       float v[4];
 #pragma unroll
-      for (int u = 0; u < 4; ++u) v[u] = L.Wp[(size_t)(cq * 64 + 16 * kb + 4 * q + u) * ldP + min(col, P - 1)];
+      for (int u = 0; u < 4; ++u) v[u] = L.Wp[(size_t)(cq * CW + 16 * kb + 4 * q + u) * ldP + min(col, P - 1)];
       asm volatile("" : "+v"(v[0]), "+v"(v[1]), "+v"(v[2]), "+v"(v[3]));
 #pragma unroll
       for (int u = 0; u < 4; ++u) v[u] = col < P ? v[u] : 0.f;
       *reinterpret_cast<float4*>(&wp_lds[w][kb][lane][0]) = make_float4(v[0], v[1], v[2], v[3]);
     }
   }
-  const int cb = cq * 64 + 16 * w + 4 * q;
-  const float4 pwi = *reinterpret_cast<const float4*>(L.wi + cb), pwf = *reinterpret_cast<const float4*>(L.wf + cb);
-  const float4 pwo = *reinterpret_cast<const float4*>(L.wo + cb);
-  f32x4 bs[4];
-#pragma unroll
-  for (int g = 0; g < 4; ++g) bs[g] = *reinterpret_cast<const f32x4*>(L.bias + g * H + cb);
+  const int cb = cq * CW + CPW * w + CPL * q;
+  float pi_[CPL], pf_[CPL], po_[CPL];
+  dp_ldn<CPL>(L.wi + cb, pi_); dp_ldn<CPL>(L.wf + cb, pf_); dp_ldn<CPL>(L.wo + cb, po_);
+  f32x4 bs[NT];
+  if constexpr (NQ == 4) {
+#pragma unroll
+    for (int g = 0; g < 4; ++g) bs[g] = *reinterpret_cast<const f32x4*>(L.bias + g * H + cb);
+  } else {
+#pragma unroll
+    for (int g = 0; g < 4; ++g) {
+      const float2 b2 = *reinterpret_cast<const float2*>(L.bias + g * H + cb);
+      bs[0][g] = b2.x; bs[1][g] = b2.y;
+    }
+  }
   const int lenF = a.len[r0 + lr];
-  float cp[4] = {0.f, 0.f, 0.f, 0.f};
+  float cp[CPL] = {};
   float4 mf[DP_KB];
 #pragma unroll
   for (int kb = 0; kb < DP_KB; ++kb) mf[kb] = make_float4(0.f, 0.f, 0.f, 0.f);
-  *reinterpret_cast<float4*>(L.c + (size_t)(rb + lr) * H + cb) = make_float4(0.f, 0.f, 0.f, 0.f);
+  dp_stn<CPL>(L.c + (size_t)(rb + lr) * H + cb, cp);
   if (cq == 0 && w == 0) {
 #pragma unroll
     for (int kb = 0; kb < DP_KB; ++kb)
       if (16 * kb + 4 * q < P) *reinterpret_cast<float4*>(L.mst + (size_t)(rb + lr) * ldP + 16 * kb + 4 * q) = make_float4(0.f, 0.f, 0.f, 0.f);
   }
 
-  f32x4 accn[4];
+  f32x4 accn[NT];
   float4 xn[DP_KB];
   auto load_x = [&](int t) {
     const float* xr = L.in + ((size_t)t * Ns + rb + lr) * L.ldI;
@@ -172,29 +224,26 @@
   auto sum_parts = [&](float (*part)[DP_KB][64][4], int width, float4 (&s)[DP_KB]) {
 #pragma unroll
     for (int kb = 0; kb < DP_KB; ++kb) {
-      const float4 p0 = *reinterpret_cast<const float4*>(&part[0][kb][lane][0]), p1 = *reinterpret_cast<const float4*>(&part[1][kb][lane][0]);
-      const float4 p2 = *reinterpret_cast<const float4*>(&part[2][kb][lane][0]), p3 = *reinterpret_cast<const float4*>(&part[3][kb][lane][0]);
-      s[kb] = dp_sel(16 * kb + 4 * q < width,
-                     make_float4(((p0.x + p1.x) + p2.x) + p3.x, ((p0.y + p1.y) + p2.y) + p3.y, ((p0.z + p1.z) + p2.z) + p3.z,
-                                 ((p0.w + p1.w) + p2.w) + p3.w), make_float4(0.f, 0.f, 0.f, 0.f));
-    }
-  };
-  auto mma_part = [&](f32x4 (&acc)[4], const float4 (&af)[DP_KB], const float4 (&bf)[4][DP_KB]) {
+      s[kb] = dp_sel(16 * kb + 4 * q < width, dp_sum_nq<NQ>(part, kb, lane), make_float4(0.f, 0.f, 0.f, 0.f));
+      if constexpr (NQ == 8) __builtin_amdgcn_sched_barrier(0);
+    }
+  };
+  auto mma_part = [&](f32x4 (&acc)[NT], const float4 (&af)[DP_KB], const float4 (&bf)[NT][DP_KB]) {
 #pragma unroll
     for (int kb = 0; kb < DP_KB; ++kb) {
 #pragma unroll
-      for (int g = 0; g < 4; ++g) acc[g] = __builtin_amdgcn_mfma_f32_16x16x4f32(bf[g][kb].x, af[kb].x, acc[g], 0, 0, 0);
-#pragma unroll
-      for (int g = 0; g < 4; ++g) acc[g] = __builtin_amdgcn_mfma_f32_16x16x4f32(bf[g][kb].y, af[kb].y, acc[g], 0, 0, 0);
-#pragma unroll
-      for (int g = 0; g < 4; ++g) acc[g] = __builtin_amdgcn_mfma_f32_16x16x4f32(bf[g][kb].z, af[kb].z, acc[g], 0, 0, 0);
-#pragma unroll
-      for (int g = 0; g < 4; ++g) acc[g] = __builtin_amdgcn_mfma_f32_16x16x4f32(bf[g][kb].w, af[kb].w, acc[g], 0, 0, 0);
+      for (int g = 0; g < NT; ++g) acc[g] = __builtin_amdgcn_mfma_f32_16x16x4f32(bf[g][kb].x, af[kb].x, acc[g], 0, 0, 0);
+#pragma unroll
+      for (int g = 0; g < NT; ++g) acc[g] = __builtin_amdgcn_mfma_f32_16x16x4f32(bf[g][kb].y, af[kb].y, acc[g], 0, 0, 0);
+#pragma unroll
+      for (int g = 0; g < NT; ++g) acc[g] = __builtin_amdgcn_mfma_f32_16x16x4f32(bf[g][kb].z, af[kb].z, acc[g], 0, 0, 0);
+#pragma unroll
+      for (int g = 0; g < NT; ++g) acc[g] = __builtin_amdgcn_mfma_f32_16x16x4f32(bf[g][kb].w, af[kb].w, acc[g], 0, 0, 0);
     }
   };
   auto next_x = [&](int t) {
 #pragma unroll
-    for (int g = 0; g < 4; ++g) accn[g] = bs[g];
+    for (int g = 0; g < NT; ++g) accn[g] = bs[g];
     float4 xs[DP_KB];
     if (l > 0) {
       sum_parts(part_x[t & 1], I, xs);
@@ -207,17 +256,17 @@
     }
 #pragma unroll
     for (int kb = 0; kb < DP_KB; ++kb) {
-      float4 bf[4];
-#pragma unroll
-      for (int g = 0; g < 4; ++g) bf[g] = *reinterpret_cast<const float4*>(&kx_lds[w][g][kb][lane][0]);
-#pragma unroll
-      for (int g = 0; g < 4; ++g) accn[g] = __builtin_amdgcn_mfma_f32_16x16x4f32(bf[g].x, xs[kb].x, accn[g], 0, 0, 0);
-#pragma unroll
-      for (int g = 0; g < 4; ++g) accn[g] = __builtin_amdgcn_mfma_f32_16x16x4f32(bf[g].y, xs[kb].y, accn[g], 0, 0, 0);
-#pragma unroll
-      for (int g = 0; g < 4; ++g) accn[g] = __builtin_amdgcn_mfma_f32_16x16x4f32(bf[g].z, xs[kb].z, accn[g], 0, 0, 0);
-#pragma unroll
-      for (int g = 0; g < 4; ++g) accn[g] = __builtin_amdgcn_mfma_f32_16x16x4f32(bf[g].w, xs[kb].w, accn[g], 0, 0, 0);
+      float4 bf[NT];
+#pragma unroll
+      for (int g = 0; g < NT; ++g) bf[g] = *reinterpret_cast<const float4*>(&kx_lds[w][g][kb][lane][0]);
+#pragma unroll
+      for (int g = 0; g < NT; ++g) accn[g] = __builtin_amdgcn_mfma_f32_16x16x4f32(bf[g].x, xs[kb].x, accn[g], 0, 0, 0);
+#pragma unroll
+      for (int g = 0; g < NT; ++g) accn[g] = __builtin_amdgcn_mfma_f32_16x16x4f32(bf[g].y, xs[kb].y, accn[g], 0, 0, 0);
+#pragma unroll
+      for (int g = 0; g < NT; ++g) accn[g] = __builtin_amdgcn_mfma_f32_16x16x4f32(bf[g].z, xs[kb].z, accn[g], 0, 0, 0);
+#pragma unroll
+      for (int g = 0; g < NT; ++g) accn[g] = __builtin_amdgcn_mfma_f32_16x16x4f32(bf[g].w, xs[kb].w, accn[g], 0, 0, 0);
     }
   };
   auto store_m = [&](int t, const float4 (&mnew)[DP_KB], bool live_prev) {
@@ -237,15 +286,15 @@
   next_x(0);
   if (l == 0) load_x(min(1, T - 1));
 
-  float hv[4] = {0.f, 0.f, 0.f, 0.f}, sg[4][4] = {};
+  float hv[CPL] = {}, sg[4][CPL] = {};
   for (int t = 0; t < T; ++t) {
-    f32x4 acc[4];
+    f32x4 acc[NT];
     DPT(0);
     __syncthreads();
     if (dead) return;
     DPT(1);
 #pragma unroll
-    for (int g = 0; g < 4; ++g) acc[g] = accn[g];
+    for (int g = 0; g < NT; ++g) acc[g] = accn[g];
     if (t > 0) {
       float4 ms[DP_KB];
       sum_parts(part_m, P, ms);
@@ -257,26 +306,26 @@
     mma_part(acc, mf, kh);
     DPT(2);
     const bool live = t < lenF;
-    const float pi_[4] = {pwi.x, pwi.y, pwi.z, pwi.w}, pf_[4] = {pwf.x, pwf.y, pwf.z, pwf.w}, po_[4] = {pwo.x, pwo.y, pwo.z, pwo.w};
-#pragma unroll
-    for (int i = 0; i < 4; ++i) {
+    auto z = [&](int g, int i) { if constexpr (NQ == 4) return acc[g][i]; else return acc[i][g]; };
+#pragma unroll
+    for (int i = 0; i < CPL; ++i) {
       const float cpv = cp[i];
-      const float gi = dp_sigmoid(acc[0][i] + pi_[i] * cpv);
-      const float gf = dp_sigmoid(acc[2][i] + a.forget_bias + pf_[i] * cpv);
-      const float gj = dp_tanh(acc[1][i]);
+      const float gi = dp_sigmoid(z(0, i) + pi_[i] * cpv);
+      const float gf = dp_sigmoid(z(2, i) + a.forget_bias + pf_[i] * cpv);
+      const float gj = dp_tanh(z(1, i));
       const float cn = gf * cpv + gi * gj;
-      const float go = dp_sigmoid(acc[3][i] + po_[i] * cn);
+      const float go = dp_sigmoid(z(3, i) + po_[i] * cn);
       const float hh = go * dp_tanh(cn);
       hv[i] = live ? hh : 0.f;
       sg[0][i] = live ? gi : 0.f; sg[1][i] = live ? gj : 0.f; sg[2][i] = live ? gf : 0.f; sg[3][i] = live ? go : 0.f;
       cp[i] = live ? cn : cpv;
     }
     {
-      const int so = lr * DP_HS + 16 * w + 4 * q;
-#pragma unroll
-      for (int g = 0; g < 4; ++g) *reinterpret_cast<float4*>(&stage[g][so]) = make_float4(sg[g][0], sg[g][1], sg[g][2], sg[g][3]);
-      *reinterpret_cast<float4*>(&stage[4][so]) = make_float4(cp[0], cp[1], cp[2], cp[3]);
-      *reinterpret_cast<float4*>(&stage[5][so]) = make_float4(hv[0], hv[1], hv[2], hv[3]);
+      const int so = lr * DP_HS + CPW * w + CPL * q;
+#pragma unroll
+      for (int g = 0; g < 4; ++g) dp_stn<CPL>(&stage[g][so], sg[g]);
+      dp_stn<CPL>(&stage[4][so], cp);
+      dp_stn<CPL>(&stage[5][so], hv);
     }
     DPT(3);
     __syncthreads();
@@ -304,17 +353,27 @@
 __global__ __launch_bounds__(512, 1) void k_dlstm_fwd(const DPersistArgs a) {
   gu32* ctl = (gu32*)a.ctl;
   const unsigned gen = __hip_atomic_load(ctl + DP_CTL_GEN, __ATOMIC_RELAXED, __HIP_MEMORY_SCOPE_AGENT);
-  dp_fwd_body(a, gen);
+  dp_fwd_body<4>(a, gen);
   if (threadIdx.x == 0) persist_last_out(ctl, gen, [] { return gridDim.x; }, [&] { return a.L[a.nl - 1].out; }, 0u, [] {});
 }
-
+__global__ __launch_bounds__(768, 1) void k_dlstm_fwd8(const DPersistArgs a) {
+  gu32* ctl = (gu32*)a.ctl;
+  const unsigned gen = __hip_atomic_load(ctl + DP_CTL_GEN, __ATOMIC_RELAXED, __HIP_MEMORY_SCOPE_AGENT);
+  dp_fwd_body<8>(a, gen);
+  if (threadIdx.x == 0) persist_last_out(ctl, gen, [] { return gridDim.x; }, [&] { return a.L[a.nl - 1].out; }, 0u, [] {});
+}
+
+template <int NQ>
 __device__ __forceinline__ void dp_bwd_body(const DPersistArgs& a, const unsigned gen) {
-  __shared__ __attribute__((aligned(16))) float part_m[DP_NQ][DP_KB][64][4];
-  __shared__ __attribute__((aligned(16))) float part_x[2][DP_NQ][DP_KB][64][4];
+  typedef DpForm<NQ> F;
+  constexpr int CW = F::CW, CPW = F::CPW, CPL = F::CPL;
+  constexpr int NKB = CPW / 4;
+  __shared__ __attribute__((aligned(16))) float part_m[NQ][DP_KB][64][4];
+  __shared__ __attribute__((aligned(16))) float part_x[2][NQ][DP_KB][64][4];
   __shared__ __attribute__((aligned(16))) float stage[4][16 * DP_HS];
   __shared__ __attribute__((aligned(16))) float psum[4][DP_KB][64][4];
   __shared__ __attribute__((aligned(16))) float psum_x[2][4][DP_KB][64][4];
-  __shared__ __attribute__((aligned(16))) float kx_lds[4][DP_KB][4][64][4];
+  __shared__ __attribute__((aligned(16))) float kx_lds[4][DP_KB][NKB][64][4];
   __shared__ int dead;
   DPT_DECL
   const int RTn = a.N >> 4, ncl = a.nl * RTn;
@@ -328,7 +387,7 @@
   const bool top = l == a.nl - 1;
   gu32* err = (gu32*)a.ctl + DP_CTL_ERR;
   if (tid == 0) dead = 0;
-  const size_t slot_stride_t = (size_t)DP_NQ * DP_SLOT;
+  const size_t slot_stride_t = (size_t)NQ * DP_SLOT;
   auto edge = [&](int layer, int e) -> gu64* {
     return (gu64*)a.gran + ((size_t)((layer * 2 + e) * RTn + r) * T) * slot_stride_t;
   };
@@ -341,7 +400,7 @@
     const gu64* gx = edge(min(l + 1, a.nl - 1), 1) + (size_t)j * DP_SLOT;
     gu64* gout_m = edge(l, 0) + (size_t)cq * DP_SLOT;
     gu64* gout_x = edge(l, 1) + (size_t)cq * DP_SLOT;
-    gu32* dwf = a.dw_ws ? (gu32*)a.dw_flag + ((size_t)(l * RTn + r) * (T + 1)) * 4 + cq : nullptr;
+    gu32* dwf = a.dw_ws ? (gu32*)a.dw_flag + ((size_t)(l * RTn + r) * (T + 1)) * NQ + cq : nullptr;
     float vm[DP_KB * 4], vx[DP_KB * 4];
     auto put = [&](float (*part)[DP_KB][64][4], const float (&v)[DP_KB * 4]) {
 #pragma unroll
@@ -366,6 +425,7 @@
       const bool wm = t < T - 1, wx = !top && t > 0;
       DPG(0);
       if (wm || wx) {
+        if constexpr (NQ == 8 && DP_NQ8_WAIT > 0) __builtin_amdgcn_s_sleep(DP_NQ8_WAIT);
         if (!dp_sweep2(wm ? gm + (size_t)(t + 1) * slot_stride_t : nullptr, gen, vm,
                        wx ? gx + (size_t)(t - 1) * slot_stride_t : nullptr, gen, vx, lane, err)) fail();
         if (wm) put(part_m, vm);
@@ -379,26 +439,27 @@
       DPG(2);
       if (j < 3) {
         publish(psum, gout_m + (size_t)t * slot_stride_t);
-      } else {
-        const int c4 = (lane & 15) * 4, rr = lane >> 4;
+      } else if (NQ == 4 || j == 3) {
+        constexpr int LPR = CW / 4, RPP = 64 / LPR;
+        const int c4 = (lane % LPR) * 4, rr = lane / LPR;
         if (dwf) {
-          if (lane == 0) __hip_atomic_store(dwf + (size_t)t * 4, gen, __ATOMIC_RELAXED, __HIP_MEMORY_SCOPE_AGENT);
-#pragma unroll
-          for (int rg = 0; rg < 4; ++rg) {
-            const int row = 4 * rg + rr;
+          if (lane == 0) __hip_atomic_store(dwf + (size_t)t * NQ, gen, __ATOMIC_RELAXED, __HIP_MEMORY_SCOPE_AGENT);
+#pragma unroll
+          for (int rg = 0; rg < 16 / RPP; ++rg) {
+            const int row = RPP * rg + rr;
             const size_t grow = (size_t)t * N + r0 + row;
 #pragma unroll
             for (int g = 0; g < 4; ++g)
-              dp_store4_wt(L.gates + grow * H4 + g * H + cq * 64 + c4, *reinterpret_cast<const float4*>(&stage[g][row * DP_HS + c4]));
+              dp_store4_wt(L.gates + grow * H4 + g * H + cq * CW + c4, *reinterpret_cast<const float4*>(&stage[g][row * DP_HS + c4]));
           }
         } else {
 #pragma unroll
-          for (int rg = 0; rg < 4; ++rg) {
-            const int row = 4 * rg + rr;
+          for (int rg = 0; rg < 16 / RPP; ++rg) {
+            const int row = RPP * rg + rr;
             const size_t grow = (size_t)t * N + r0 + row;
 #pragma unroll
             for (int g = 0; g < 4; ++g)
-              *reinterpret_cast<float4*>(L.gates + grow * H4 + g * H + cq * 64 + c4) = *reinterpret_cast<const float4*>(&stage[g][row * DP_HS + c4]);
+              *reinterpret_cast<float4*>(L.gates + grow * H4 + g * H + cq * CW + c4) = *reinterpret_cast<const float4*>(&stage[g][row * DP_HS + c4]);
           }
         }
       }
@@ -411,10 +472,10 @@
     return;
   }
 
-  const int cb = cq * 64 + 16 * w + 4 * q;
-  float4 wpA[DP_KB], khA[DP_KB][4];
+  const int cb = cq * CW + CPW * w + CPL * q;
+  float4 wpA[DP_KB], khA[DP_KB][NKB];
   {
-    const float* wrow = L.Wp + (size_t)(cq * 64 + 16 * w + lr) * ldP;
+    const float* wrow = L.Wp + (size_t)(cq * CW + CPW * w + (NQ == 4 ? lr : 2 * (lr >> 2) + (lr & 1))) * ldP;
 #pragma unroll
     for (int kb = 0; kb < DP_KB; ++kb) {
       const int k = 16 * kb + 4 * q;
@@ -425,31 +486,38 @@
     for (int pt = 0; pt < DP_KB; ++pt) {
       const int p = 16 * pt + lr;
 #pragma unroll
-      for (int g = 0; g < 4; ++g) {
-        const float4 vh = *reinterpret_cast<const float4*>(L.K + (size_t)(I + min(p, P - 1)) * H4 + g * H + cb);
-        const float4 vx = *reinterpret_cast<const float4*>(L.K + (size_t)min(p, I - 1) * H4 + g * H + cb);
+      for (int g = 0; g < NKB; ++g) {
+        float4 vh, vx;
+        if constexpr (NQ == 4) {
+          vh = *reinterpret_cast<const float4*>(L.K + (size_t)(I + min(p, P - 1)) * H4 + g * H + cb);
+          vx = *reinterpret_cast<const float4*>(L.K + (size_t)min(p, I - 1) * H4 + g * H + cb);
+        } else {
+          const float* kh_ = L.K + (size_t)(I + min(p, P - 1)) * H4 + cb + g;
+          const float* kx_ = L.K + (size_t)min(p, I - 1) * H4 + cb + g;
+          vh = make_float4(kh_[0], kh_[H], kh_[2 * H], kh_[3 * H]);
+          vx = make_float4(kx_[0], kx_[H], kx_[2 * H], kx_[3 * H]);
+        }
         khA[pt][g] = dp_sel(p < P, vh, make_float4(0.f, 0.f, 0.f, 0.f));
         *reinterpret_cast<float4*>(&kx_lds[w][pt][g][lane][0]) = dp_sel(l > 0 && p < I, vx, make_float4(0.f, 0.f, 0.f, 0.f));
       }
     }
   }
-  const float4 pwi = *reinterpret_cast<const float4*>(L.wi + cb), pwf = *reinterpret_cast<const float4*>(L.wf + cb);
-  const float4 pwo = *reinterpret_cast<const float4*>(L.wo + cb);
-  const float pi_[4] = {pwi.x, pwi.y, pwi.z, pwi.w}, pf_[4] = {pwf.x, pwf.y, pwf.z, pwf.w}, po_[4] = {pwo.x, pwo.y, pwo.z, pwo.w};
+  float pi_[CPL], pf_[CPL], po_[CPL];
+  dp_ldn<CPL>(L.wi + cb, pi_); dp_ldn<CPL>(L.wf + cb, pf_); dp_ldn<CPL>(L.wo + cb, po_);
   const int lenF = a.len[r0 + lr];
 
-  float dc[4] = {0.f, 0.f, 0.f, 0.f};
+  float dc[CPL] = {};
   float4 mf[DP_KB];
 #pragma unroll
   for (int kb = 0; kb < DP_KB; ++kb) mf[kb] = make_float4(0.f, 0.f, 0.f, 0.f);
-  f32x4 gn[4], cpn;
+  float gn[4][CPL], cpn[CPL];
   float4 don[DP_KB];
-  f32x4 ccur;
+  float ccur[CPL];
   auto prefetch = [&](int t) {
     const size_t row = (size_t)t * N + r0 + lr;
 #pragma unroll
-    for (int g = 0; g < 4; ++g) gn[g] = *reinterpret_cast<const f32x4*>(L.gates + row * H4 + g * H + cb);
-    cpn = *reinterpret_cast<const f32x4*>(L.c + row * H + cb);
+    for (int g = 0; g < 4; ++g) dp_ldn<CPL>(L.gates + row * H4 + g * H + cb, gn[g]);
+    dp_ldn<CPL>(L.c + row * H + cb, cpn);
     if (top) {
 #pragma unroll
       for (int kb = 0; kb < DP_KB; ++kb)
@@ -459,14 +527,11 @@
   auto sum_parts = [&](float (*part)[DP_KB][64][4], int width, float4 (&s)[DP_KB]) {
 #pragma unroll
     for (int kb = 0; kb < DP_KB; ++kb) {
-      const float4 p0 = *reinterpret_cast<const float4*>(&part[0][kb][lane][0]), p1 = *reinterpret_cast<const float4*>(&part[1][kb][lane][0]);
-      const float4 p2 = *reinterpret_cast<const float4*>(&part[2][kb][lane][0]), p3 = *reinterpret_cast<const float4*>(&part[3][kb][lane][0]);
-      s[kb] = dp_sel(16 * kb + 4 * q < width,
-                     make_float4(((p0.x + p1.x) + p2.x) + p3.x, ((p0.y + p1.y) + p2.y) + p3.y, ((p0.z + p1.z) + p2.z) + p3.z,
-                                 ((p0.w + p1.w) + p2.w) + p3.w), make_float4(0.f, 0.f, 0.f, 0.f));
-    }
-  };
-  ccur = *reinterpret_cast<const f32x4*>(L.c + ((size_t)T * N + r0 + lr) * H + cb);
+      s[kb] = dp_sel(16 * kb + 4 * q < width, dp_sum_nq<NQ>(part, kb, lane), make_float4(0.f, 0.f, 0.f, 0.f));
+      if constexpr (NQ == 8) __builtin_amdgcn_sched_barrier(0);
+    }
+  };
+  dp_ldn<CPL>(L.c + ((size_t)T * N + r0 + lr) * H + cb, ccur);
   prefetch(T - 1);
   __syncthreads();
   if (dead) return;
@@ -477,10 +542,13 @@
     if (dead) return;
     DPT(1);
     const bool live = t < lenF;
-    f32x4 gt[4];
-#pragma unroll
-    for (int g = 0; g < 4; ++g) gt[g] = gn[g];
-    const f32x4 cprev = cpn;
+    float gt[4][CPL], cprev[CPL];
+#pragma unroll
+    for (int i = 0; i < CPL; ++i) {
+#pragma unroll
+      for (int g = 0; g < 4; ++g) gt[g][i] = gn[g][i];
+      cprev[i] = cpn[i];
+    }
     float4 dout[DP_KB];
     if (top) {
 #pragma unroll
@@ -521,9 +589,9 @@
       dh = __builtin_amdgcn_mfma_f32_16x16x4f32(wpA[kb].w, dm[kb].w, dh, 0, 0, 0);
     }
     DPT(2);
-    float dz[4][4];
-#pragma unroll
-    for (int i = 0; i < 4; ++i) {
+    float dz[4][CPL];
+#pragma unroll
+    for (int i = 0; i < CPL; ++i) {
       const float gi = gt[0][i], gj = gt[1][i], gf = gt[2][i], go = gt[3][i];
       const float tc = dp_tanh(ccur[i]);
       const float dao = dh[i] * tc * go * (1.f - go);
@@ -534,26 +602,28 @@
       dz[0][i] = live ? dai : 0.f; dz[1][i] = live ? dj : 0.f; dz[2][i] = live ? daf : 0.f; dz[3][i] = live ? dao : 0.f;
       dc[i] = live ? dcn * gf + dai * pi_[i] + daf * pf_[i] : dc[i];
     }
-    ccur = cprev;
+#pragma unroll
+    for (int i = 0; i < CPL; ++i) ccur[i] = cprev[i];
     {
-      const int so = lr * DP_HS + 16 * w + 4 * q;
-#pragma unroll
-      for (int g = 0; g < 4; ++g) *reinterpret_cast<float4*>(&stage[g][so]) = make_float4(dz[g][0], dz[g][1], dz[g][2], dz[g][3]);
+      const int so = lr * DP_HS + CPW * w + CPL * q;
+#pragma unroll
+      for (int g = 0; g < 4; ++g) dp_stn<CPL>(&stage[g][so], dz[g]);
     }
     DPT(3);
     f32x4 pa[DP_KB];
 #pragma unroll
     for (int pt = 0; pt < DP_KB; ++pt) pa[pt] = f32x4{0.f, 0.f, 0.f, 0.f};
-#pragma unroll
-    for (int g = 0; g < 4; ++g) {
-#pragma unroll
-      for (int pt = 0; pt < DP_KB; ++pt) pa[pt] = __builtin_amdgcn_mfma_f32_16x16x4f32(khA[pt][g].x, dz[g][0], pa[pt], 0, 0, 0);
-#pragma unroll
-      for (int pt = 0; pt < DP_KB; ++pt) pa[pt] = __builtin_amdgcn_mfma_f32_16x16x4f32(khA[pt][g].y, dz[g][1], pa[pt], 0, 0, 0);
-#pragma unroll
-      for (int pt = 0; pt < DP_KB; ++pt) pa[pt] = __builtin_amdgcn_mfma_f32_16x16x4f32(khA[pt][g].z, dz[g][2], pa[pt], 0, 0, 0);
-#pragma unroll
-      for (int pt = 0; pt < DP_KB; ++pt) pa[pt] = __builtin_amdgcn_mfma_f32_16x16x4f32(khA[pt][g].w, dz[g][3], pa[pt], 0, 0, 0);
+    auto zb = [&](int g, int u) { if constexpr (NQ == 4) return dz[g][u]; else return dz[u][g]; };
+#pragma unroll
+    for (int g = 0; g < NKB; ++g) {
+#pragma unroll
+      for (int pt = 0; pt < DP_KB; ++pt) pa[pt] = __builtin_amdgcn_mfma_f32_16x16x4f32(khA[pt][g].x, zb(g, 0), pa[pt], 0, 0, 0);
+#pragma unroll
+      for (int pt = 0; pt < DP_KB; ++pt) pa[pt] = __builtin_amdgcn_mfma_f32_16x16x4f32(khA[pt][g].y, zb(g, 1), pa[pt], 0, 0, 0);
+#pragma unroll
+      for (int pt = 0; pt < DP_KB; ++pt) pa[pt] = __builtin_amdgcn_mfma_f32_16x16x4f32(khA[pt][g].z, zb(g, 2), pa[pt], 0, 0, 0);
+#pragma unroll
+      for (int pt = 0; pt < DP_KB; ++pt) pa[pt] = __builtin_amdgcn_mfma_f32_16x16x4f32(khA[pt][g].w, zb(g, 3), pa[pt], 0, 0, 0);
     }
 #pragma unroll
     for (int pt = 0; pt < DP_KB; ++pt) *reinterpret_cast<f32x4*>(&psum[w][pt][lane][0]) = pa[pt];
@@ -565,18 +635,18 @@
 #pragma unroll
       for (int pt = 0; pt < DP_KB; ++pt) pa[pt] = f32x4{0.f, 0.f, 0.f, 0.f};
 #pragma unroll
-      for (int g = 0; g < 4; ++g) {
+      for (int g = 0; g < NKB; ++g) {
         float4 af[DP_KB];
 #pragma unroll
         for (int pt = 0; pt < DP_KB; ++pt) af[pt] = *reinterpret_cast<const float4*>(&kx_lds[w][pt][g][lane][0]);
 #pragma unroll
-        for (int pt = 0; pt < DP_KB; ++pt) pa[pt] = __builtin_amdgcn_mfma_f32_16x16x4f32(af[pt].x, dz[g][0], pa[pt], 0, 0, 0);
-#pragma unroll
-        for (int pt = 0; pt < DP_KB; ++pt) pa[pt] = __builtin_amdgcn_mfma_f32_16x16x4f32(af[pt].y, dz[g][1], pa[pt], 0, 0, 0);
-#pragma unroll
-        for (int pt = 0; pt < DP_KB; ++pt) pa[pt] = __builtin_amdgcn_mfma_f32_16x16x4f32(af[pt].z, dz[g][2], pa[pt], 0, 0, 0);
-#pragma unroll
-        for (int pt = 0; pt < DP_KB; ++pt) pa[pt] = __builtin_amdgcn_mfma_f32_16x16x4f32(af[pt].w, dz[g][3], pa[pt], 0, 0, 0);
+        for (int pt = 0; pt < DP_KB; ++pt) pa[pt] = __builtin_amdgcn_mfma_f32_16x16x4f32(af[pt].x, zb(g, 0), pa[pt], 0, 0, 0);
+#pragma unroll
+        for (int pt = 0; pt < DP_KB; ++pt) pa[pt] = __builtin_amdgcn_mfma_f32_16x16x4f32(af[pt].y, zb(g, 1), pa[pt], 0, 0, 0);
+#pragma unroll
+        for (int pt = 0; pt < DP_KB; ++pt) pa[pt] = __builtin_amdgcn_mfma_f32_16x16x4f32(af[pt].z, zb(g, 2), pa[pt], 0, 0, 0);
+#pragma unroll
+        for (int pt = 0; pt < DP_KB; ++pt) pa[pt] = __builtin_amdgcn_mfma_f32_16x16x4f32(af[pt].w, zb(g, 3), pa[pt], 0, 0, 0);
       }
 #pragma unroll
       for (int pt = 0; pt < DP_KB; ++pt) *reinterpret_cast<f32x4*>(&psum_x[t & 1][w][pt][lane][0]) = pa[pt];
@@ -591,7 +661,7 @@
 __device__ __forceinline__ float dp_ld_sc1(const float* p) {
   return __uint_as_float(__hip_atomic_load((const unsigned*)p, __ATOMIC_RELAXED, __HIP_MEMORY_SCOPE_AGENT));
 }
-template <bool proj>
+template <bool proj, int NQ>
 __device__ __forceinline__ void dp_dw_body(const DPersistArgs& a, const unsigned gen, const int bid) {
   const int RTn = a.N >> 4;
   const int g = bid & 3, cl = bid >> 2;
@@ -603,7 +673,16 @@
   const int r0 = r * 16;
   const int c0 = 32 * w, col0 = g * H + c0;
   gu32* err = (gu32*)a.ctl + DP_CTL_ERR;
-  const gu32* flags = (const gu32*)a.dw_flag + ((size_t)(l * RTn + r) * (T + 1)) * 4;
+  const gu32* flags = (const gu32*)a.dw_flag + ((size_t)(l * RTn + r) * (T + 1)) * NQ;
+  auto words_req = [&](const gu32* fp, u32x4& v0, u32x4& v1) {
+    if constexpr (NQ == 4) asm volatile("global_load_dwordx4 %0, %1, off sc1" : "=&v"(v0) : "v"(fp) : "memory");
+    else asm volatile("global_load_dwordx4 %0, %2, off sc1\n\tglobal_load_dwordx4 %1, %2, off offset:16 sc1" : "=&v"(v0), "=&v"(v1) : "v"(fp) : "memory");
+  };
+  auto words_ok = [&](const u32x4& v0, const u32x4& v1) {
+    bool k = v0.x == gen && v0.y == gen && v0.z == gen && v0.w == gen;
+    if constexpr (NQ == 8) k = k && v1.x == gen && v1.y == gen && v1.z == gen && v1.w == gen;
+    return k;
+  };
 
   f32x4 acc[DW_MT][2];
 #pragma unroll
@@ -619,12 +698,13 @@
   struct Ops { float av[DW_MT][4], bv[2][4], ev[DP_KB][4], fv[2][4]; };
   bool ok = true;
   auto wait_for = [&](int t) {
-    const gu32* fp = flags + (size_t)(t >= 2 ? t - 2 : T) * 4;
+    const gu32* fp = flags + (size_t)(t >= 2 ? t - 2 : T) * NQ;
     const unsigned long long t0 = __builtin_amdgcn_s_memrealtime();
     for (unsigned spins = 0;; ++spins) {
-      u32x4 v;
-      asm volatile("global_load_dwordx4 %0, %1, off sc1\n\ts_waitcnt vmcnt(0)" : "=&v"(v) : "v"(fp) : "memory");
-      if (v.x == gen && v.y == gen && v.z == gen && v.w == gen) return;
+      u32x4 v, v1 = {gen, gen, gen, gen};
+      if constexpr (NQ == 4) asm volatile("global_load_dwordx4 %0, %1, off sc1\n\ts_waitcnt vmcnt(0)" : "=&v"(v) : "v"(fp) : "memory");
+      else { words_req(fp, v, v1); asm volatile("s_waitcnt vmcnt(0)" : "+v"(v), "+v"(v1) : : "memory"); }
+      if (words_ok(v, v1)) return;
       __builtin_amdgcn_s_sleep(32);
       if ((spins & 63) == 63 && (__builtin_amdgcn_s_memrealtime() - t0 > 100000000ull ||
                                  __hip_atomic_load(err, __ATOMIC_RELAXED, __HIP_MEMORY_SCOPE_AGENT) != 0)) { ok = false; return; }
@@ -709,21 +789,23 @@
   __shared__ int prog;
   if (threadIdx.x == 0) prog = T;
   __syncthreads();
+  if constexpr (NQ == 8) { if (w >= 8) return; }
   Ops o;
   if (w == 0) {
     wait_for(T - 1);
     if (lane == 0) __hip_atomic_store(&prog, ok ? T - 1 : -1, __ATOMIC_RELAXED, __HIP_MEMORY_SCOPE_WORKGROUP);
     for (int t = T - 1; t >= 0 && ok; --t) {
-      u32x4 fl = {gen, gen, gen, gen};
+      u32x4 fl = {gen, gen, gen, gen}, fl1 = {gen, gen, gen, gen};
       if (t >= 1) {
-        const gu32* fp = flags + (size_t)(t >= 3 ? t - 3 : T) * 4;
-        asm volatile("global_load_dwordx4 %0, %1, off sc1" : "=&v"(fl) : "v"(fp) : "memory");
+        const gu32* fp = flags + (size_t)(t >= 3 ? t - 3 : T) * NQ;
+        words_req(fp, fl, fl1);
       }
       load(o, t);
       compute(o);
-      asm volatile("s_waitcnt vmcnt(0)" : "+v"(fl) : : "memory");
+      if constexpr (NQ == 4) asm volatile("s_waitcnt vmcnt(0)" : "+v"(fl) : : "memory");
+      else asm volatile("s_waitcnt vmcnt(0)" : "+v"(fl), "+v"(fl1) : : "memory");
       if (t >= 1) {
-        if (!(fl.x == gen && fl.y == gen && fl.z == gen && fl.w == gen)) { __builtin_amdgcn_s_sleep(32); wait_for(t - 1); }
+        if (!words_ok(fl, fl1)) { __builtin_amdgcn_s_sleep(32); wait_for(t - 1); }
         if (lane == 0) __hip_atomic_store(&prog, ok ? t - 1 : -1, __ATOMIC_RELAXED, __HIP_MEMORY_SCOPE_WORKGROUP);
       }
     }
@@ -772,40 +854,47 @@
   }
 }
 
-__global__ __launch_bounds__(512, 1) void k_dlstm_bwd(const DPersistArgs a) {
+template <int NQ>
+__device__ __forceinline__ void dp_bwd_launch(const DPersistArgs& a) {
   gu32* ctl = (gu32*)a.ctl;
   const unsigned gen = __hip_atomic_load(ctl + DP_CTL_GEN, __ATOMIC_RELAXED, __HIP_MEMORY_SCOPE_AGENT);
-  const int nchain = a.nl * (a.N >> 4) * DP_NQ;
+  const int nchain = a.nl * (a.N >> 4) * NQ;
   if ((int)blockIdx.x >= nchain) {
     const int bid = (int)blockIdx.x - nchain;
-    if ((bid & 3) == 1) dp_dw_body<true>(a, gen, bid); else dp_dw_body<false>(a, gen, bid);
+    if ((bid & 3) == 1) dp_dw_body<true, NQ>(a, gen, bid); else dp_dw_body<false, NQ>(a, gen, bid);
   } else {
-    dp_bwd_body(a, gen);
+    dp_bwd_body<NQ>(a, gen);
     if (a.dw_ws) {
       asm volatile("s_waitcnt vmcnt(0)" ::: "memory");
       __syncthreads();
       if (threadIdx.x == 0) {
         const int RTn = a.N >> 4, ncl = a.nl * RTn, cl = blockIdx.x % ncl, cq = blockIdx.x / ncl;
-        __hip_atomic_store((gu32*)a.dw_flag + ((size_t)cl * (a.T + 1) + a.T) * 4 + cq, gen, __ATOMIC_RELAXED, __HIP_MEMORY_SCOPE_AGENT);
+        __hip_atomic_store((gu32*)a.dw_flag + ((size_t)cl * (a.T + 1) + a.T) * NQ + cq, gen, __ATOMIC_RELAXED, __HIP_MEMORY_SCOPE_AGENT);
       }
     }
   }
   if (threadIdx.x == 0) persist_last_out(ctl, gen, [] { return gridDim.x; }, [&] { return a.L[0].gates; }, 0u, [] {});
 }
-
-
-size_t dpersist_granule_bytes(int nl, int N, int T) { return (size_t)2 * nl * (N / 16) * T * DP_NQ * DP_SLOT * sizeof(unsigned long long); }
-
-int dpersist_grid(int nl, int N) { return nl * (N / 16) * DP_NQ; }
-size_t dpersist_lds_bytes() {
+__global__ __launch_bounds__(512, 1) void k_dlstm_bwd(const DPersistArgs a) { dp_bwd_launch<4>(a); }
+__global__ __launch_bounds__(768, 1) void k_dlstm_bwd8(const DPersistArgs a) { dp_bwd_launch<8>(a); }
+
+
+size_t dpersist_granule_bytes(int nl, int N, int T, int nq) { return (size_t)2 * nl * (N / 16) * T * nq * DP_SLOT * sizeof(unsigned long long); }
+
+int dpersist_grid(int nl, int N, int nq) { return nl * (N / 16) * nq; }
+int dpersist_threads(int nq) { return nq == 8 ? DpForm<8>::THREADS : DpForm<4>::THREADS; }
+size_t dpersist_lds_bytes(int nq) {
   hipFuncAttributes f{}, b{};
-  if (hipFuncGetAttributes(&f, (const void*)k_dlstm_fwd) != hipSuccess || hipFuncGetAttributes(&b, (const void*)k_dlstm_bwd) != hipSuccess) return 0;
+  if (hipFuncGetAttributes(&f, nq == 8 ? (const void*)k_dlstm_fwd8 : (const void*)k_dlstm_fwd) != hipSuccess ||
+      hipFuncGetAttributes(&b, nq == 8 ? (const void*)k_dlstm_bwd8 : (const void*)k_dlstm_bwd) != hipSuccess) return 0;
   return f.sharedSizeBytes > b.sharedSizeBytes ? f.sharedSizeBytes : b.sharedSizeBytes;
 }
 
-bool dpersist_supported(const DPersistArgs& a) {
-  if (a.nl < 1 || a.nl > DP_MAXL || a.N % 16 != 0 || a.H != 64 * DP_NQ || a.T < 1) return false;
-  if (dpersist_grid(a.nl, a.N) > 128 || dpersist_grid(a.nl, a.N) > device_cu_count()) return false;
+bool dpersist_shapes_fit(const DPersistArgs& a) {
+  const int nq = a.nq ? a.nq : DP_NQ;
+  if (nq != 4 && nq != 8) return false;
+  if (a.nl < 1 || a.nl > DP_MAXL || a.N % 16 != 0 || a.H != 64 * DP_NQ || a.H != DpForm<8>::CW * 8 || a.T < 1) return false;
+  if (dpersist_grid(a.nl, a.N, nq) > 128) return false;
   for (int l = 0; l < a.nl; ++l) {
     const DPersistLayer& L = a.L[l];
     if (L.P > 16 * DP_KB || L.P % 4 != 0 || L.ldP % 4 != 0 || L.P < 4) return false;
@@ -814,15 +903,21 @@
   }
   return true;
 }
+bool dpersist_supported(const DPersistArgs& a) {
+  const int nq = a.nq ? a.nq : DP_NQ;
+  return dpersist_shapes_fit(a) && dpersist_grid(a.nl, a.N, nq) + (a.dw_ws ? dpersist_dw_grid(a.nl, a.N) : 0) <= device_cu_count();
+}
 
 void launch_dlstm_bwd(const DPersistArgs& a, hipStream_t s) {
-  const int blocks = dpersist_grid(a.nl, a.N) + (a.dw_ws ? dpersist_dw_grid(a.nl, a.N) : 0);
-  hipLaunchKernelGGL(k_dlstm_bwd, dim3(blocks), dim3(512), 0, s, a);
+  const int nq = a.nq ? a.nq : DP_NQ;
+  const int blocks = dpersist_grid(a.nl, a.N, nq) + (a.dw_ws ? dpersist_dw_grid(a.nl, a.N) : 0);
+  if (nq == 8) hipLaunchKernelGGL(k_dlstm_bwd8, dim3(blocks), dim3(DpForm<8>::THREADS), 0, s, a);
+  else hipLaunchKernelGGL(k_dlstm_bwd, dim3(blocks), dim3(512), 0, s, a);
   ++g_chain_launches;
 }
 int dpersist_dw_grid(int nl, int N) { return 4 * nl * (N / 16); }
 size_t dpersist_dw_stride(const DPersistArgs& a) { return (size_t)(a.L[0].I + a.L[0].P + 1) * 4 * a.H + 3 * (size_t)a.H + (size_t)a.H * a.L[0].ldP; }
-size_t dpersist_dw_flag_bytes(int nl, int N, int T) { return (size_t)nl * (N / 16) * (T + 1) * 4 * sizeof(unsigned); }
+size_t dpersist_dw_flag_bytes(int nl, int N, int T, int nq) { return (size_t)nl * (N / 16) * (T + 1) * nq * sizeof(unsigned); }
 bool dpersist_dw_supported(const DPersistArgs& a) {
   for (int l = 0; l < a.nl; ++l) {
     const DPersistLayer& L = a.L[l];
@@ -854,8 +949,10 @@
   return a.L[0].I % 4 == 0 && a.L[0].I >= 4 && a.L[0].I <= a.ld_dy && a.L[0].I <= a.ld_fcw;
 }
 void launch_dlstm_fwd(const DPersistArgs& a, hipStream_t s) {
-  const int blocks = dpersist_grid(a.nl, a.N);
-  hipLaunchKernelGGL(k_dlstm_fwd, dim3(blocks), dim3(512), 0, s, a);
+  const int nq = a.nq ? a.nq : DP_NQ;
+  const int blocks = dpersist_grid(a.nl, a.N, nq);
+  if (nq == 8) hipLaunchKernelGGL(k_dlstm_fwd8, dim3(blocks), dim3(DpForm<8>::THREADS), 0, s, a);
+  else hipLaunchKernelGGL(k_dlstm_fwd, dim3(blocks), dim3(512), 0, s, a);
   ++g_chain_launches;
 }
 
diff --git a/rsrgan_amd/csrc/kernels.h b/rsrgan_amd/csrc/kernels.h
--- a/rsrgan_amd/csrc/kernels.h
+++ b/rsrgan_amd/csrc/kernels.h
@@ -140,18 +140,21 @@
   float* dw_ws;
   unsigned* dw_flag;
   size_t dw_stride;
+  int nq;
 };
 int dpersist_dw_grid(int nl, int N);
 size_t dpersist_dw_stride(const DPersistArgs& a);
-size_t dpersist_dw_flag_bytes(int nl, int N, int T);
+size_t dpersist_dw_flag_bytes(int nl, int N, int T, int nq = 4);
 bool dpersist_dw_supported(const DPersistArgs& a);
-size_t dpersist_granule_bytes(int nl, int N, int T);
+size_t dpersist_granule_bytes(int nl, int N, int T, int nq = 4);
 int dpersist_trail_grid(int nl, int N);
 size_t dpersist_trail_lds_bytes();
 bool dpersist_trail_supported(const DPersistArgs& a);
 bool dpersist_supported(const DPersistArgs& a);
-int dpersist_grid(int nl, int N);
-size_t dpersist_lds_bytes();
+bool dpersist_shapes_fit(const DPersistArgs& a);
+int dpersist_grid(int nl, int N, int nq = 4);
+int dpersist_threads(int nq);
+size_t dpersist_lds_bytes(int nq = 4);
 void launch_dlstm_fwd(const DPersistArgs& a, hipStream_t s);
 void launch_dlstm_fwd_t(const DPersistArgs& a, hipStream_t s);
 void launch_dlstm_bwd(const DPersistArgs& a, hipStream_t s);
diff --git a/rsrgan_amd/csrc/model.cpp b/rsrgan_amd/csrc/model.cpp
--- a/rsrgan_amd/csrc/model.cpp
+++ b/rsrgan_amd/csrc/model.cpp
@@ -399,8 +399,11 @@
     D_.in = l == 0 ? R.in : nullptr;
   }
   if (!dpersist_supported(a) || dpersist_grid(a.nl, a.N) > dp_max_grid || dpersist_granule_bytes(a.nl, a.N, a.T) > dp_gran_bytes) return false;
-  if (switches().dfwd_t && a.N % 32 == 0) launch_dlstm_fwd_t(a, s); else launch_dlstm_fwd(a, s);
-  if (prof_on) ++prof_cnt[4];
+  const bool two_tile = switches().dfwd_t && a.N % 32 == 0;
+  if (!two_tile) a.nq = dp_pick_nq(4, a.nl, a.N, a.T, true);
+  if (a.nq == 8 && !dpersist_supported(a)) a.nq = 4;
+  if (two_tile) launch_dlstm_fwd_t(a, s); else launch_dlstm_fwd(a, s);
+  if (prof_on) { ++prof_cnt[4]; if (a.nq == 8) ++prof_cnt[9]; }
   return true;
 }
 
@@ -441,6 +444,11 @@
     G_.res_out = a.res ? g_res[l] : nullptr;
   }
   return true;
+}
+
+int Model::dp_pick_nq(int bit, int nl, int N, int T, bool one_edge) const {
+  if (!(dp_live & bit) || dp_max_grid8 <= 0 || dpersist_grid(nl, N, 8) > dp_max_grid8) return 4;
+  return dpersist_granule_bytes(nl, N, T, 8) / (one_edge ? 2 : 1) <= dp_gran_bytes ? 8 : 4;
 }
 
 void Model::persist_disable(int which) {
@@ -670,9 +678,12 @@
   if (!a.dout_top || !dpersist_supported(a) || dpersist_grid(a.nl, a.N) > dp_max_grid || dpersist_granule_bytes(a.nl, a.N, a.T) > dp_gran_bytes) return false;
   bool dw = dw_ws && !defer_wgrads && a.N == 2 * B && T <= Tmax;
   for (auto& R : ch) dw = dw && R.want_wgrads && R.in && R.ps == &D;
+  a.nq = dp_pick_nq(8, a.nl, a.N, a.T, false);
+  if (dw && a.nq != dp_dw_nq) a.nq = 4;
   if (dw) { a.dw_ws = dw_ws; a.dw_flag = dw_flag; a.dw_stride = dw_stride; }
+  if (a.nq == 8 && !dpersist_supported(a)) a.nq = 4;
   launch_dlstm_bwd(a, s);
-  if (prof_on) { ++prof_cnt[5]; if (dw) ++prof_cnt[6]; }
+  if (prof_on) { ++prof_cnt[5]; if (dw) ++prof_cnt[6]; if (a.nq == 8) ++prof_cnt[10]; }
   if (dw) {
     launch_dw_reduce(dw_ws, dw_stride, a.N / 16, dw_src, D.g, D.ct, D.partial, s);
     d_partial_fresh = true;
diff --git a/rsrgan_amd/csrc/model.h b/rsrgan_amd/csrc/model.h
--- a/rsrgan_amd/csrc/model.h
+++ b/rsrgan_amd/csrc/model.h
@@ -176,6 +176,9 @@
   unsigned* dp_ctl = nullptr;
   size_t dp_gran_bytes = 0;
   int dp_live = sw.dpersist;
+  int dp_max_grid8 = 0;
+  int dp_dw_nq = 4;
+  int dp_pick_nq(int bit, int nl, int N, int T, bool one_edge) const;
   bool persist_forward(Chain& ch, int T, hipStream_t s);
   bool persist_backward(Chain& ch, int T, hipStream_t s);
   bool persist_backward_trail(Chain& ch, int T, hipStream_t s, float* dy, int ld_dy, float* dtop, int ld_dtop, bool check_only = false);
@@ -377,7 +380,7 @@
   std::vector<hipEvent_t> prof_gb_ev;
   int prof_gb_n = 0;
   int prof_fdt_n = 0;
-  int prof_cnt[9] = {};
+  int prof_cnt[11] = {};
   double prof_gb_flops = 0.0;
   void gates_launch(const FwdGateJobs& gj, int blocks, int kb, hipStream_t s);
   int gates_blocks(int H, int N) const;
diff --git a/rsrgan_amd/csrc/model_init.cpp b/rsrgan_amd/csrc/model_init.cpp
--- a/rsrgan_amd/csrc/model_init.cpp
+++ b/rsrgan_amd/csrc/model_init.cpp
@@ -565,21 +565,35 @@
     }
   }
   if (dp_max_grid <= 0) return RSRGAN_OK;
-  dp_gran_bytes = dpersist_granule_bytes((int)dl.size(), 2 * B, Tmax);
+  DPersistArgs pa{};
+  pa.nl = (int)dl.size(); pa.N = 2 * B; pa.H = dl[0].H; pa.T = 1;
+  for (size_t l = 0; l < dl.size(); ++l) { pa.L[l].I = dl[l].I; pa.L[l].P = dl[l].P; pa.L[l].ldP = dl[l].ldP; pa.L[l].ldI = dl[l].ldI; }
+  bool dw_shapes = switches().dw_inkernel && (dp_live & 2) && dpersist_dw_supported(pa) && !d_adam();
+  for (auto& L : dl) dw_shapes = dw_shapes && L.has_proj && L.H == dl[0].H && L.ldH == dl[0].ldH;
+  if (dp_live & 12) {
+    for (int rows : {2 * B, B}) {
+      DPersistArgs p8 = pa;
+      p8.N = rows; p8.nq = 8;
+      if (dpersist_grid(pa.nl, rows) > dp_max_grid) continue;
+      if (!dpersist_shapes_fit(p8)) continue;
+      const int g8 = dpersist_grid(p8.nl, rows, 8);
+      const int ride = rows == 2 * B && dw_shapes && (dp_live & 8) ? dpersist_dw_grid(p8.nl, rows) : 0;
+      if (g8 + ride <= device_cu_count() && resident_probe(g8 + ride, dpersist_threads(8), dpersist_lds_bytes(8))) { dp_max_grid8 = g8; break; }
+    }
+  }
+  const bool bwd8 = (dp_live & 8) && dp_max_grid8 >= dpersist_grid(pa.nl, 2 * B, 8);
+  dp_gran_bytes = dpersist_granule_bytes((int)dl.size(), 2 * B, Tmax, bwd8 ? 8 : 4);
   dp_gran = (unsigned long long*)alloc<float>(dp_gran_bytes / sizeof(float));
   dp_ctl = (unsigned*)alloc<float>(16);
   if (int rc = alloc_status("persistent discriminator rings")) return rc;
   HIPC(ctl_reset(dp_ctl));
-  DPersistArgs pa{};
-  pa.nl = (int)dl.size(); pa.N = 2 * B; pa.H = dl[0].H;
-  for (size_t l = 0; l < dl.size(); ++l) { pa.L[l].I = dl[l].I; pa.L[l].P = dl[l].P; pa.L[l].ldP = dl[l].ldP; pa.L[l].ldI = dl[l].ldI; }
-  bool shapes = switches().dw_inkernel && (dp_live & 2) && dpersist_dw_supported(pa) && !d_adam();
-  for (auto& L : dl) shapes = shapes && L.has_proj && L.H == dl[0].H && L.ldH == dl[0].ldH;
+  const bool shapes = dw_shapes;
   if (shapes && dpersist_grid(pa.nl, pa.N) == dp_max_grid) {
     const int nt = pa.N / 16;
     dw_stride = dpersist_dw_stride(pa);
     dw_ws = alloc_opt<float>((size_t)pa.nl * nt * dw_stride);
-    dw_flag = (unsigned*)alloc_opt<float>(dpersist_dw_flag_bytes(pa.nl, pa.N, Tmax) / sizeof(float));
+    dp_dw_nq = bwd8 ? 8 : 4;
+    dw_flag = (unsigned*)alloc_opt<float>(dpersist_dw_flag_bytes(pa.nl, pa.N, Tmax, dp_dw_nq) / sizeof(float));
     std::vector<long long> src(D.t.size(), -1);
     const int IP = dl[0].I + dl[0].P, H4 = 4 * dl[0].H, H_ = dl[0].H;
     for (size_t l = 0; l < dl.size(); ++l) {
diff --git a/rsrgan_amd/csrc/switches.h b/rsrgan_amd/csrc/switches.h
--- a/rsrgan_amd/csrc/switches.h
+++ b/rsrgan_amd/csrc/switches.h
@@ -5,7 +5,7 @@
 
 #define RSRGAN_SWITCHES(X) \
   X(GPERSIST,       gpersist,       INT,  3,    ANY,  handle,  "persistent generator recurrences (gpersist.hip): bit 0 the forward launch, bit 1 the BPTT; 0 = the launch-per-phase wavefront") \
-  X(DPERSIST,       dpersist,       INT,  3,    ANY,  handle,  "persistent discriminator recurrences (dpersist.hip): bit 0 the forward launch, bit 1 the backward launch") \
+  X(DPERSIST,       dpersist,       INT,  7,    ANY,  handle,  "persistent discriminator recurrences (dpersist.hip): bit 0 the forward launch, bit 1 the backward launch; bits 2 / 3: that launch with eight workgroups per row tile where shapes and device allow") \
   X(DFOLD,          dfold,          BOOL, 1,    ANY,  handle,  "folded small-cell recurrence of the discriminator (one launch per step); 0 = gates + projection") \
   X(TRAIL,          trail,          INT,  1,    ANY,  handle,  "the discriminator's BPTT trailing the generator's inside one launch (k_glstm_bwd_dt); 0 = two launches") \
   X(GRAPHS,         graphs,         BOOL, 1,    ANY,  handle,  "0 = RSRGAN_FLAG_GRAPH is ignored: every segment runs eagerly") \
```

Result: no change. 1.331 million, median of 2 (+0.1%).
